# asmuth-archive/libsmatrix

Hardware: AMD Instinct MI355X
Metric: mixed incr+get ops/s (higher is better)
Workload: dtype u32; 1 GPU; config-2: 1xMI355X, 100M-nnz / 1M-row Zipf(1.1) stream (scrambled ids, seed 12345), batched incr+get, 2^24 ops per batch, step = incr batch + get batch; ids_per_axis=1000000, batch_ops=16777216, parallelism=single GPU

## Files before the change

include/smatrix_batch.h:

```cpp
#ifndef SMATRIX_BATCH_H
#define SMATRIX_BATCH_H

#include "smatrix.h"

#ifdef __cplusplus
extern "C" {
#endif

enum { SMATRIX_OP_GET = 0, SMATRIX_OP_SET = 1, SMATRIX_OP_INCR = 2, SMATRIX_OP_DECR = 3 };

int smatrix_apply_batch(smatrix_t* self, int op, size_t n, const uint32_t* x,
                        const uint32_t* y, const uint32_t* v, uint32_t* out);
int smatrix_get_batch(smatrix_t* self, size_t n, const uint32_t* x, const uint32_t* y, uint32_t* out);
int smatrix_set_batch(smatrix_t* self, size_t n, const uint32_t* x, const uint32_t* y,
                      const uint32_t* v, uint32_t* out);
int smatrix_incr_batch(smatrix_t* self, size_t n, const uint32_t* x, const uint32_t* y,
                       const uint32_t* v, uint32_t* out);
int smatrix_decr_batch(smatrix_t* self, size_t n, const uint32_t* x, const uint32_t* y,
                       const uint32_t* v, uint32_t* out);
int smatrix_rowlen_batch(smatrix_t* self, size_t n, const uint32_t* x, uint32_t* out);
int smatrix_getrow_batch(smatrix_t* self, size_t n, const uint32_t* x, const uint64_t* offsets,
                         uint32_t* ret, uint32_t* counts);

int smatrix_apply_batch_dev(smatrix_t* self, int op, size_t n, const uint32_t* d_x,
                            const uint32_t* d_y, const uint32_t* d_v, uint32_t* d_out,
                            void* hip_stream);

int smatrix_apply_packed_dev(smatrix_t* self, int op, size_t n, const uint32_t* d_records, uint32_t width,
                             uint32_t* d_out, void* hip_stream);
int smatrix_rowlen_batch_dev(smatrix_t* self, size_t n, const uint32_t* d_x, uint32_t* d_out,
                             void* hip_stream);
int smatrix_getrow_batch_dev(smatrix_t* self, size_t n, const uint32_t* d_x,
                             const uint64_t* d_offsets, uint32_t* d_ret, uint32_t* d_counts,
                             void* hip_stream);

int smatrix_cf_neighbors_batch(smatrix_t* self, size_t n, const uint32_t* items, const uint64_t* offsets,
                               uint32_t* ids, double* scores, uint32_t* counts);
int smatrix_cf_neighbors_batch_dev(smatrix_t* self, size_t n, const uint32_t* d_items,
                                   const uint64_t* d_offsets, uint32_t* d_ids, double* d_scores,
                                   uint32_t* d_counts, void* hip_stream);

int smatrix_cf_topk_batch(smatrix_t* self, size_t n, const uint32_t* items, uint32_t k, uint32_t* ids, double* scores,
                          uint32_t* counts);
int smatrix_cf_topk_batch_dev(smatrix_t* self, size_t n, const uint32_t* d_items, uint32_t k, uint32_t* d_ids,
                              double* d_scores, uint32_t* d_counts, void* hip_stream);

int smatrix_cf_recommend_batch(smatrix_t* self, size_t n_sessions, const uint64_t* offsets, const uint32_t* items,
                               uint32_t k, uint32_t* ids, double* scores, uint32_t* counts);
int smatrix_cf_recommend_batch_dev(smatrix_t* self, size_t n_sessions, const uint64_t* d_offsets, const uint32_t* d_items,
                                   uint32_t k, uint32_t* d_ids, double* d_scores, uint32_t* d_counts, void* hip_stream);

int smatrix_cf_import_sessions(smatrix_t* self, size_t n_sessions, const uint64_t* offsets, const uint32_t* ids);
int smatrix_cf_import_sessions_dev(smatrix_t* self, size_t n_sessions, const uint64_t* d_offsets, const uint32_t* d_ids,
                                   const uint64_t* d_op_offsets, uint64_t total_ops, void* hip_stream);

enum { SMATRIX_EXPORT_TABLE = 0, SMATRIX_EXPORT_SORTED = 1 };

int smatrix_export(smatrix_t* self, int order, uint64_t cap_rows, uint64_t cap_nnz,
                   uint32_t* rows, uint64_t* row_ptr, uint32_t* pairs, uint64_t* n_rows, uint64_t* nnz);
int smatrix_export_dev(smatrix_t* self, int order, uint64_t cap_rows, uint64_t cap_nnz,
                       uint32_t* d_rows, uint64_t* d_row_ptr, uint32_t* d_pairs,
                       uint64_t* n_rows, uint64_t* nnz, void* hip_stream);

int smatrix_merge(smatrix_t* dst, smatrix_t* src, int op, uint64_t max_batch, uint64_t* n_ops);

int smatrix_merge_scaled(smatrix_t* dst, smatrix_t* src, int op, uint32_t num, uint32_t den, uint32_t min_value,
                         uint64_t max_batch, uint64_t* n_ops, uint64_t* n_dropped);

int smatrix_merge_topk(smatrix_t* dst, smatrix_t* src, int op, uint32_t m, uint32_t min_value, uint64_t max_batch,
                       uint64_t* n_ops, uint64_t* n_dropped);
int smatrix_import_csr(smatrix_t* self, int op, uint64_t n_rows, const uint32_t* rows, const uint64_t* row_ptr,
                       const uint32_t* pairs, uint64_t max_batch, uint64_t* n_ops);
int smatrix_import_csr_dev(smatrix_t* self, int op, uint64_t n_rows, const uint32_t* d_rows,
                           const uint64_t* d_row_ptr, const uint32_t* d_pairs, uint64_t max_batch,
                           uint64_t* n_ops, void* hip_stream);

int smatrix_reserve(smatrix_t* self, uint64_t bytes);

void smatrix_release_cached_memory(void);

typedef struct {
  uint64_t rows;
  uint64_t dir_slots;
  uint64_t arena_units;
  uint64_t arena_mapped;
  uint64_t arena_free_units;
  uint64_t batches;
  uint64_t rounds;
  uint64_t deferred_ops;
  uint64_t rows_grown;
  uint64_t dir_grown;
  uint64_t rows_rebalanced;
  uint64_t long_probe_rounds;
  uint64_t scalar_cache_hits;
  uint64_t scalar_cache_flushes;
  uint64_t scalar_cache_flushed_cells;
  uint64_t bulk_rounds;
  uint64_t bulk_ops;
  uint64_t file_flushes;
  uint64_t file_rows_written;
  uint64_t file_leaked_bytes;
  uint64_t file_compactions;
  uint64_t spec_chains;
  uint64_t spec_refused;
  uint64_t file_bg_flushes;
  uint64_t cold_starts;
  uint64_t cold_keys;
  uint64_t clustered_mode;
  uint64_t set_located_by_fold;
  uint64_t flush_snapshots_refused;
  double   kernel_ms[4];
  uint64_t kernel_launches[4];
  uint64_t kernel_ops[4];
  double   write_call_ms, write_wait_ms, write_alloc_ms;
  double   last_write_call_ms, last_write_wait_ms, last_write_alloc_ms;
} smatrix_stats_t;

void smatrix_stats(smatrix_t* self, smatrix_stats_t* out);
void smatrix_stats_sz(smatrix_t* self, smatrix_stats_t* out, size_t size);
int smatrix_flush(smatrix_t* self);
#ifdef SMATRIX_EXPERIMENTAL
int smatrix_compact(smatrix_t* self);
#endif
void smatrix_profile(smatrix_t* self, int on);
int smatrix_row_info(smatrix_t* self, uint32_t x, uint32_t* size, uint32_t* used);
uint32_t smatrix_row_slots(smatrix_t* self, uint32_t x, uint32_t* kv, uint32_t cap_slots);
int smatrix_device_available(void);

#ifdef __cplusplus
}
#endif
#endif
```

libsmatrix_amd/_lib.py:

```python
import ctypes as C
import os

HERE = os.path.dirname(os.path.abspath(__file__))
LIB_PATH = os.path.join(HERE, "lib", "smatrix.so")
CSRC = os.path.join(HERE, "csrc")

u32p = C.POINTER(C.c_uint32)
u64p = C.POINTER(C.c_uint64)


class Stats(C.Structure):
    _fields_ = [(n, C.c_uint64) for n in (
        "rows", "dir_slots", "arena_units", "arena_mapped", "arena_free_units", "batches", "rounds",
        "deferred_ops", "rows_grown", "dir_grown", "rows_rebalanced", "long_probe_rounds", "scalar_cache_hits", "scalar_cache_flushes",
        "scalar_cache_flushed_cells", "bulk_rounds", "bulk_ops", "file_flushes", "file_rows_written", "file_leaked_bytes",
        "file_compactions", "spec_chains", "spec_refused", "file_bg_flushes", "cold_starts", "cold_keys", "clustered_mode", "set_located_by_fold", "flush_snapshots_refused")] + [
        ("kernel_ms", C.c_double * 4), ("kernel_launches", C.c_uint64 * 4), ("kernel_ops", C.c_uint64 * 4)] + [
        (n, C.c_double) for n in ("write_call_ms", "write_wait_ms", "write_alloc_ms", "last_write_call_ms", "last_write_wait_ms", "last_write_alloc_ms")]


class Handle(C.Structure):
    _fields_ = [("fd", C.c_int), ("shutdown", C.c_int), ("fpos", C.c_uint64),
                ("mem", C.c_uint64), ("impl", C.c_void_p)]


_lib = None


def load():
    global _lib
    if _lib is not None:
        return _lib
    if not os.path.exists(LIB_PATH):
        raise ImportError(
            "libsmatrix_amd: %s is missing -- build it with `make -C %s` "
            "(or python -c 'import __graft_entry__ as g; g.build()').  "
            "This package has no CPU fallback." % (LIB_PATH, CSRC))
    lib = C.CDLL(LIB_PATH)
    H = C.POINTER(Handle)
    V = C.c_void_p
    sig = {
        "smatrix_open": (H, [C.c_char_p]),
        "smatrix_close": (None, [H]),
        "smatrix_get": (C.c_uint32, [H, C.c_uint32, C.c_uint32]),
        "smatrix_set": (C.c_uint32, [H, C.c_uint32, C.c_uint32, C.c_uint32]),
        "smatrix_incr": (C.c_uint32, [H, C.c_uint32, C.c_uint32, C.c_uint32]),
        "smatrix_decr": (C.c_uint32, [H, C.c_uint32, C.c_uint32, C.c_uint32]),
        "smatrix_rowlen": (C.c_uint32, [H, C.c_uint32]),
        "smatrix_getrow": (C.c_uint32, [H, C.c_uint32, u32p, C.c_size_t]),
        "smatrix_apply_batch": (C.c_int, [H, C.c_int, C.c_size_t, u32p, u32p, u32p, u32p]),
        "smatrix_get_batch": (C.c_int, [H, C.c_size_t, u32p, u32p, u32p]),
        "smatrix_set_batch": (C.c_int, [H, C.c_size_t, u32p, u32p, u32p, u32p]),
        "smatrix_incr_batch": (C.c_int, [H, C.c_size_t, u32p, u32p, u32p, u32p]),
        "smatrix_decr_batch": (C.c_int, [H, C.c_size_t, u32p, u32p, u32p, u32p]),
        "smatrix_rowlen_batch": (C.c_int, [H, C.c_size_t, u32p, u32p]),
        "smatrix_getrow_batch": (C.c_int, [H, C.c_size_t, u32p, u64p, u32p, u32p]),
        "smatrix_apply_batch_dev": (C.c_int, [H, C.c_int, C.c_size_t, V, V, V, V, V]),
        "smatrix_apply_packed_dev": (C.c_int, [V, C.c_int, C.c_size_t, V, C.c_uint32, V, V]),
        "smatrix_rowlen_batch_dev": (C.c_int, [H, C.c_size_t, V, V, V]),
        "smatrix_getrow_batch_dev": (C.c_int, [H, C.c_size_t, V, V, V, V, V]),
        "smatrix_cf_neighbors_batch": (C.c_int, [H, C.c_size_t, u32p, u64p, u32p, C.POINTER(C.c_double), u32p]),
        "smatrix_cf_neighbors_batch_dev": (C.c_int, [H, C.c_size_t, V, V, V, V, V, V]),
        "smatrix_release_cached_memory": (None, []),
        "smatrix_reserve": (C.c_int, [H, C.c_uint64]),
        "smatrix_cf_topk_batch": (C.c_int, [H, C.c_size_t, u32p, C.c_uint32, u32p, C.POINTER(C.c_double), u32p]),
        "smatrix_cf_topk_batch_dev": (C.c_int, [H, C.c_size_t, V, C.c_uint32, V, V, V, V]),
        "smatrix_cf_recommend_batch": (C.c_int, [H, C.c_size_t, u64p, u32p, C.c_uint32, u32p, C.POINTER(C.c_double), u32p]),
        "smatrix_cf_recommend_batch_dev": (C.c_int, [H, C.c_size_t, V, V, C.c_uint32, V, V, V, V]),
        "smatrix_cf_import_sessions": (C.c_int, [H, C.c_size_t, u64p, u32p]),
        "smatrix_cf_import_sessions_dev": (C.c_int, [H, C.c_size_t, V, V, V, C.c_uint64, V]),
        "smatrix_export": (C.c_int, [H, C.c_int, C.c_uint64, C.c_uint64, u32p, u64p, u32p, u64p, u64p]),
        "smatrix_export_dev": (C.c_int, [H, C.c_int, C.c_uint64, C.c_uint64, V, V, V, u64p, u64p, V]),
        "smatrix_merge": (C.c_int, [H, H, C.c_int, C.c_uint64, u64p]),
        "smatrix_merge_scaled": (C.c_int, [H, H, C.c_int, C.c_uint32, C.c_uint32, C.c_uint32, C.c_uint64, u64p, u64p]),
        "smatrix_merge_topk": (C.c_int, [H, H, C.c_int, C.c_uint32, C.c_uint32, C.c_uint64, u64p, u64p]),
        "smatrix_import_csr": (C.c_int, [H, C.c_int, C.c_uint64, u32p, u64p, u32p, C.c_uint64, u64p]),
        "smatrix_import_csr_dev": (C.c_int, [H, C.c_int, C.c_uint64, V, V, V, C.c_uint64, u64p, V]),
        "smatrix_stats": (None, [H, C.POINTER(Stats)]),
        "smatrix_stats_sz": (None, [H, C.POINTER(Stats), C.c_size_t]),
        "smatrix_profile": (None, [H, C.c_int]),
        "smatrix_flush": (C.c_int, [H]),
        "smatrix_compact": (C.c_int, [H]),
        "smatrix_row_info": (C.c_int, [H, C.c_uint32, u32p, u32p]),
        "smatrix_row_slots": (C.c_uint32, [H, C.c_uint32, u32p, C.c_uint32]),
        "smatrix_device_available": (C.c_int, []),
        "smatrix_shard_of": (C.c_uint32, [C.c_uint32, C.c_uint32]),
        "smatrix_partition_dev": (C.c_int, [C.c_size_t, V, V, V, C.c_uint32, u64p, V, V, V, V, V, V, C.c_uint32, V, V]),
        "smatrix_partition_packed_dev": (C.c_int, [C.c_size_t, V, V, V, C.c_uint32, u64p, V, V, V, V, C.c_uint32, V, V]),
        "smatrix_shard_mix": (C.c_uint32, [C.c_uint32]),
        "smatrix_place_slot": (C.c_uint32, [C.c_uint32, C.c_uint32]),
        "smatrix_displaced_rows": (C.c_size_t, [V, C.c_uint32, C.c_uint32, V, C.c_size_t]),
        "smatrix_unpack_dev": (C.c_int, [C.c_size_t, C.c_uint32, V, V, V, V, V]),
        "smatrix_gather_dev": (C.c_int, [C.c_size_t, V, V, V, V]),
        "smatrix_shard_unique_id": (C.c_int, [V]),
        "smatrix_shard_open": (V, [C.c_char_p, C.c_int, C.c_int, V]),
        "smatrix_shard_close": (None, [V]),
        "smatrix_shard_local": (H, [V]),
        "smatrix_shard_rank": (C.c_int, [V]),
        "smatrix_shard_nranks": (C.c_int, [V]),
        "smatrix_shard_ops_applied": (C.c_uint64, [V]),
        "smatrix_shard_set_placement": (C.c_int, [V, V, V, C.c_uint32]),
        "smatrix_shard_apply_dev": (C.c_int, [V, C.c_int, C.c_size_t, V, V, V, V, V]),
        "smatrix_shard_apply_then_get_dev": (C.c_int, [V, C.c_int, C.c_size_t, V, V, V, V, V, V]),
        "smatrix_shard_transport": (C.c_char_p, [V]),
        "smatrix_shard_plan_json": (C.c_int, [V, V, C.c_size_t, C.c_uint64, C.c_int, C.c_int, V, C.c_size_t]),
        "smatrix_shard_get_placement": (C.c_int, [V, V, V, V, C.c_uint32, V]),
        "smatrix_shard_route_dev": (V, [V, C.c_int, C.c_size_t, V, V, V, C.c_int, V]),
        "smatrix_shard_apply_routed": (C.c_int, [V, V, C.c_int, V]),
        "smatrix_shard_finish": (C.c_int, [V, V, V, V]),
        "smatrix_shard_wait": (C.c_int, [V, V, V]),
        "smatrix_shard_rowlen_dev": (C.c_int, [V, C.c_size_t, V, V, V]),
        "smatrix_shard_getrow_dev": (C.c_int, [V, C.c_size_t, V, V, V, V, V]),
        "smx_probe_random_dev": (C.c_int, [V, C.c_size_t, C.c_size_t, C.c_int, C.c_uint64, V, V]),
        "smx_stream_new": (V, [C.c_int, C.c_uint64, C.c_uint32, C.c_double, C.c_int]),
        "smx_stream_free": (None, [V]),
        "smx_stream_fill": (None, [V, C.c_uint64, C.c_size_t, u32p, u32p]),
        "smx_stream_fill_device": (C.c_int, [V, C.c_uint64, C.c_size_t, V, V, V]),
        "smx_splitmix64_at": (C.c_uint64, [C.c_uint64, C.c_uint64]),
        "smx_fmix32": (C.c_uint32, [C.c_uint32]),
        "smx_stream_cdf": (C.POINTER(C.c_double), [V, u32p]),
    }
    for name, (res, args) in sig.items():
        fn = getattr(lib, name)
        fn.restype, fn.argtypes = res, args
    _lib = lib
    return lib
```

libsmatrix_amd/csrc/kernels/growth.hpp:

```cpp


constexpr uint32_t CHUNK_NONE = 0xFFFFFFFFu;
__device__ __forceinline__ void grow_plan_body(VGrid g, Ctl* ctl, GrowTask* tasks, uint64_t arena_cap_units, FreeLists fl,
                                               uint32_t task_budget, uint32_t chunk_cap, uint32_t* pend_ctl = nullptr, uint32_t pend_cap_keys = 0,
                                               uint32_t* task_of = nullptr) {
  __shared__ uint32_t l_pend, l_pend0, l_pend_ok;
  __shared__ uint32_t l_want[N_CLASSES], l_got[N_CLASSES];
  __shared__ int32_t l_top[N_CLASSES];
  __shared__ uint32_t l_chunks, l_chunk0, l_chunk_ok;
  __shared__ unsigned long long l_units, l_unit0;
  __shared__ uint32_t l_unit_ok;
  const uint32_t n = aload(&ctl->n_tasks);
  for (uint32_t t0 = g.bid * blockDim.x; t0 < n; t0 += g.nb * blockDim.x) {
    if (threadIdx.x < N_CLASSES) l_want[threadIdx.x] = 0;
    if (threadIdx.x == 0) { l_chunks = 0; l_units = 0; l_chunk_ok = 1; l_unit_ok = 1; l_pend = 0; l_pend_ok = 0; }
    __syncthreads();
    const uint32_t t = t0 + threadIdx.x;
    const bool live = t < n;
    uint32_t cls = 0, rank = 0;
    bool refused = live && t >= task_budget;
    const bool chunked = live && !refused && grow_kind(tasks[t].old_lg) == GROW_CHUNKED;
    uint32_t my_chunk = 0;
    if (chunked) my_chunk = atomicAdd(&l_chunks, 1u << (tasks[t].old_lg - 6));
    __syncthreads();
// ... 1055 lines not shown
  if (k.old_lg + 1 >= HOME_LG) {
    unsigned long long* hb = row_home(arena, k.new_base, k.old_lg + 1);
    for (uint32_t w = 0; w <= (nmask >> 6); w++) {
      unsigned long long m = 0;
      for (uint32_t b = 0; b < 64; b++) {
        const uint64_t c = T[w * 64 + b];
        if (c != 0 && cell_key(c) != 0 && (cell_key(c) & nmask) == w * 64 + b) m |= 1ull << b;
      }
      hb[w] = m;
    }
  }
  if (k.old_lg >= HOME_LG)
    for (uint32_t w = 0; w < (old_size >> 6); w++) row_home(arena, k.old_base, k.old_lg)[w] = 0;
}

__device__ __forceinline__ void grow_zero_body(VGrid g, const Ctl* ctl, const GrowTask* tasks,
                                               const uint32_t* map_old, uint8_t* arena) {
  uint32_t nchunks = aload(&ctl->n_chunks);
  uint32_t wave = (g.bid * blockDim.x + threadIdx.x) >> 6;
  uint32_t lane = threadIdx.x & 63;
  uint32_t nwaves = (g.nb * blockDim.x) >> 6;
  for (uint32_t ch = wave; ch < nchunks; ch += nwaves) {
    const GrowTask k = tasks[map_old[ch]];
    if (k.dup || k.new_base == 0) continue;
    const uint32_t p = (ch - k.chunk0) * 64 + lane;
    if (p < (1u << k.old_lg)) row_cells(arena, k.old_base)[p] = 0;
    if (lane == 0) row_home(arena, k.old_base, k.old_lg)[ch - k.chunk0] = 0;
  }
}
__global__ __launch_bounds__(256) void k_grow_zero(const Ctl* ctl, const GrowTask* tasks,
                                                   const uint32_t* map_old, uint8_t* arena) {
  grow_zero_body(SMX_VG, ctl, tasks, map_old, arena);
}

__device__ __forceinline__ void grow_commit_body(VGrid g, Ctl* ctl, GrowTask* tasks, DirSlot* dir, uint8_t* arena,
                                                 FreeLists fl, uint32_t* big_list = nullptr, uint32_t big_cap = 0) {
  __shared__ uint32_t l_want[N_CLASSES], l_at[N_CLASSES];
  const uint32_t n = aload(&ctl->n_tasks);
  for (uint32_t t0 = g.bid * blockDim.x; t0 < n; t0 += g.nb * blockDim.x) {
    if (threadIdx.x < N_CLASSES) l_want[threadIdx.x] = 0;
    __syncthreads();
    const uint32_t t = t0 + threadIdx.x;
    bool live = t < n;
    GrowTask k = {};
    uint32_t cls = 0, rank = 0;
    if (live && tasks[t].new_base == 0) {
      atomicAnd(&dir[tasks[t].dslot].meta, ~META_GROW);
      live = false;
    }
    if (live) {
      if (tasks[t].dup) grow_fixdup_one(tasks[t], arena);
      k = tasks[t];
      DirSlot& d = dir[k.dslot];
      const uint32_t lg = k.old_lg + 1;
      uint32_t count = k.count;
      if (lg >= BIG_LG && !k.dup) {
        const SubCtr* sc = row_subs(arena, k.new_base, lg);
        for (uint32_t i = 0; i < SUBS; i++) count += sc[i].cnt;
      }
      d.meta = META_USED | META_DIRTY | (lg << META_LG_SHIFT);
      d.base = k.new_base;
      d.used = count;
      if (big_list && lg == FAR_ROW_LG) {
        const uint32_t at = atomicAdd(&big_list[0], 1u);
        if (at < big_cap) big_list[1u + at] = k.dslot;
      }
      if (lg >= BIG_LG) {
        const uint32_t cap = (1u << lg) / 2u + 1u;
        subs_init(row_subs(arena, k.new_base, lg), cap > count ? cap - count : 0u);
      }
      if (k.old_lg >= BIG_LG) {
        uint64_t* z = reinterpret_cast<uint64_t*>(row_subs(arena, k.old_base, k.old_lg));
        for (uint32_t i = 0; i < SUBS * 8; i++) z[i] = 0;
      }
      cls = k.old_lg - ROW_FIRST_LG;
      rank = atomicAdd(&l_want[cls], 1u);
    }
    __syncthreads();
    if (threadIdx.x < N_CLASSES && l_want[threadIdx.x])
      l_at[threadIdx.x] = (uint32_t)atomicAdd(&ctl->free_cnt[threadIdx.x], (int32_t)l_want[threadIdx.x]);
    __syncthreads();
    if (live) {
      fl.list[cls][l_at[cls] + rank] = k.old_base;
    }
    __syncthreads();
  }
}
__global__ __launch_bounds__(256) void k_grow_commit(Ctl* ctl, GrowTask* tasks, DirSlot* dir, uint8_t* arena,
                                                     FreeLists fl, uint32_t* big_list, uint32_t big_cap) {
  grow_commit_body(SMX_VG, ctl, tasks, dir, arena, fl, big_list, big_cap);
}

__global__ __launch_bounds__(256) void k_home_list(const DirSlot* dir, uint32_t dir_size, uint32_t* list, uint32_t* n_list, uint32_t cap) {
  for (uint32_t h = blockIdx.x * blockDim.x + threadIdx.x; h < dir_size; h += gridDim.x * blockDim.x) {
    const DirSlot d = dir[h];
    if ((d.meta & META_USED) && d.base != 0 && meta_lg(d.meta) >= HOME_LG) {
      const uint32_t at = atomicAdd(n_list, 1u);
      if (at < cap) list[at] = h;
    }
  }
}
__global__ __launch_bounds__(256) void k_home_rebuild(const DirSlot* dir, const uint32_t* list, uint32_t first, uint8_t* arena) {
  const DirSlot d = dir[list[first + blockIdx.y]];
  const uint32_t lg = meta_lg(d.meta), nwords = 1u << (lg - 6), mask = (1u << lg) - 1u;
  const uint64_t* cells = row_cells(arena, d.base);
  unsigned long long* hb = row_home(arena, d.base, lg);
  const uint32_t lane = threadIdx.x & 63u;
  for (uint32_t w = blockIdx.x * 4u + (threadIdx.x >> 6); w < nwords; w += gridDim.x * 4u) {
    const uint32_t p = w * 64u + lane;
    const uint64_t c = cells[p];
    const uint64_t m = __ballot(c != 0 && cell_key(c) != 0 && (cell_key(c) & mask) == p);
    if (lane == 0) hb[w] = m;
  }
}

__device__ __forceinline__ void rebal_body(VGrid g, const Ctl* ctl, const uint32_t* rebal, DirSlot* dir, uint8_t* arena) {
  uint32_t n = aload(&ctl->n_rebal);
  for (uint32_t t = g.bid * blockDim.x + threadIdx.x; t < n; t += g.nb * blockDim.x) {
    DirSlot& d = dir[rebal[t]];
    const uint32_t lg = meta_lg(d.meta);
    SubCtr* sc = row_subs(arena, d.base, lg);
    uint32_t used = d.used;
    for (uint32_t k = 0; k < SUBS; k++) used += sc[k].cnt;
    const uint32_t cap = (1u << lg) / 2u + 1u;
    d.used = used;
    d.meta &= ~META_REBAL;
    subs_init(sc, cap > used ? cap - used : 0u);
  }
}
__global__ void k_rebal(const Ctl* ctl, const uint32_t* rebal, DirSlot* dir, uint8_t* arena) {
  rebal_body(SMX_VG, ctl, rebal, dir, arena);
}

__global__ void k_round_advance(Ctl* ctl, const uint32_t* rebal, DirSlot* dir, uint8_t* arena) {
  rebal_body(VGrid{0, 1}, ctl, rebal, dir, arena);
  __syncthreads();
  if (threadIdx.x != 0 || blockIdx.x != 0) return;
  ctl->n_prev = ctl->n_defer;
  ctl->spec_nd0 = ctl->n_defer;
  ctl->spec_nt0 = ctl->n_tasks;
  ctl->spec_gu0 = ctl->grow_units;
  ctl->spec_nrebal0 = ctl->n_rebal;
  ctl->spec_dirfull0 = ctl->dir_full;
  for (int k = 0; k < 4; k++) ctl->spec_nkind0[k] = ctl->n_kind[k];
  const uint32_t keep_long = ctl->n_long, keep_oom = ctl->arena_oom, keep_long_ops = ctl->n_long_ops, n_absent = ctl->n_absent;
  uint64_t* z = reinterpret_cast<uint64_t*>(ctl);
  for (uint32_t i = 0; i < CTL_ROUND_BYTES / 8; i++) z[i] = 0;
  ctl->n_defer = n_absent;
  ctl->n_long = keep_long;
  ctl->n_long_ops = keep_long_ops;
  ctl->arena_oom = keep_oom;
}

__global__ __launch_bounds__(256) void k_dir_rehash(const DirSlot* old, uint32_t old_size,
                                                    DirSlot* dir, uint32_t dmask) {
  uint32_t p = blockIdx.x * blockDim.x + threadIdx.x;
  if (p >= old_size) return;
  DirSlot s = old[p];
  if (!(s.meta & META_USED)) return;
  uint32_t h = fmix32(s.x) & dmask;
  uint64_t want = (uint64_t)s.meta | ((uint64_t)s.x << 32);
  for (;;) {
    uint64_t prev = atomicCAS(reinterpret_cast<unsigned long long*>(&dir[h]), 0ull,
                              (unsigned long long)want);
    if (prev == 0) break;
    h = (h + 1) & dmask;
  }
  dir[h].base = s.base;
  dir[h].used = s.used;
}
```

libsmatrix_amd/csrc/kernels/layout.hpp:

```cpp


struct DirSlot {
  uint32_t meta;
  uint32_t x;
  uint32_t base;
  uint32_t used;
};
static_assert(sizeof(DirSlot) == 16, "DirSlot must be 16 bytes");

constexpr uint32_t META_USED = 1u;
constexpr uint32_t META_GROW = 1u << 16;
constexpr uint32_t META_DIRTY = 1u << 18;
constexpr uint32_t META_LG_SHIFT = 8;
constexpr uint32_t ROW_FIRST_LG = 4;
constexpr uint32_t UNIT_BYTES = 128;

__host__ __device__ inline uint32_t meta_lg(uint32_t meta) { return (meta >> META_LG_SHIFT) & 63u; }
__host__ __device__ inline uint64_t units_of_lg(uint32_t lg) { return 1ull << (lg - ROW_FIRST_LG); }

constexpr uint32_t META_REBAL = 1u << 17;
#ifndef SMX_BIG_LG
#define SMX_BIG_LG 15
#endif
constexpr uint32_t BIG_LG = SMX_BIG_LG;
constexpr uint32_t SUBS = 64;
constexpr uint32_t SUB_UNITS = SUBS * 64 / 128;
struct SubCtr { uint32_t cnt, quota, pad[14]; };
static_assert(sizeof(SubCtr) == 64, "one sub-counter per 64-byte line");

#ifndef SMX_HOME_LG
#define SMX_HOME_LG 12
#endif
constexpr uint32_t HOME_LG = SMX_HOME_LG;
static_assert(HOME_LG >= 10, "the bitmap of the smallest such row fills whole 128-byte units");
__host__ __device__ inline uint64_t home_units(uint32_t lg) { return lg >= HOME_LG ? 1ull << (lg - 10) : 0; }
__host__ __device__ inline uint64_t block_units(uint32_t lg) {
  return units_of_lg(lg) + (lg >= BIG_LG ? SUB_UNITS : 0) + home_units(lg);
}
#ifndef SMX_ENDGAME
#define SMX_ENDGAME 8
#endif
constexpr uint32_t SUBS_ENDGAME = SMX_ENDGAME * SUBS;
__host__ __device__ inline void subs_init(SubCtr* sc, uint32_t room) {
  for (uint32_t k = 0; k < SUBS; k++) {
    sc[k].cnt = 0;
    sc[k].quota = room < SUBS_ENDGAME ? (k == 0 ? room : 0u) : room / SUBS + (k < room % SUBS ? 1u : 0u);
  }
  sc[0].pad[0] = 0;
}

enum Op : int { OP_GET = 0, OP_SET = 1, OP_INCR = 2, OP_DECR = 3 };


constexpr uint32_t N_CLASSES = 28;
struct Ctl {
  uint32_t n_defer;
  uint32_t n_tasks;
  uint32_t dir_full;
  uint32_t arena_oom;
  uint64_t grow_units;
  uint32_t n_chunks;
  uint32_t n_chunks_new;
  uint32_t n_rebal;
  uint32_t n_kind[4];
  uint32_t n_long;
  uint32_t n_long_ops;
  uint32_t n_absent;
  uint32_t dir_used;
  uint32_t pad1;
  uint64_t arena_next;
  int32_t  free_cnt[N_CLASSES];
  uint32_t n_prev;
  uint32_t spec_nd0;
  uint32_t spec_nt0;
  uint32_t spec_failed;
  uint64_t spec_gu0;
  uint32_t spec_nrebal0, spec_dirfull0;
  uint32_t spec_nkind0[4];
  uint32_t n_big, n_units;
  uint32_t far_nd, pad_far;
};
constexpr size_t CTL_ROUND_BYTES = 64;
static_assert(offsetof(Ctl, dir_used) == CTL_ROUND_BYTES, "the per-round part of Ctl is what ctl_reset_round zeroes");

struct FreeLists {
  uint32_t* list[N_CLASSES];
  uint32_t cap[N_CLASSES];
};

struct GrowTask {
  uint32_t dslot;
  uint32_t old_lg;
  uint32_t old_base;
  uint32_t new_base;
  uint32_t count;
  uint32_t chunk0;
  uint32_t chunk0_new;
  uint32_t dup;
  uint32_t wrap_from;
  uint32_t wrap_seen;
  uint32_t n_disp;
  uint32_t pend_off;
  uint32_t pend_cap;
  uint32_t n_pend;
};

constexpr uint32_t GROW_LG0 = 8;
constexpr uint32_t GROW_LG1 = 11;
constexpr uint32_t GROW_LG2 = 13;
constexpr uint32_t GROW_CHUNKED = 3;
__host__ __device__ inline uint32_t grow_kind(uint32_t old_lg) {
  return old_lg <= GROW_LG0 ? 0u : old_lg <= GROW_LG1 ? 1u : old_lg <= GROW_LG2 ? 2u : GROW_CHUNKED;
}

struct VGrid { uint32_t bid, nb; };
#define SMX_VG (VGrid{blockIdx.x, gridDim.x})
__device__ inline uint32_t aload(const uint32_t* p) { return __hip_atomic_load(p, __ATOMIC_RELAXED, __HIP_MEMORY_SCOPE_AGENT); }
__device__ inline uint64_t aload(const uint64_t* p) { return __hip_atomic_load(p, __ATOMIC_RELAXED, __HIP_MEMORY_SCOPE_AGENT); }

__device__ inline uint32_t fmix32(uint32_t h) {
  h ^= h >> 16; h *= 0x85ebca6bU; h ^= h >> 13; h *= 0xc2b2ae35U; h ^= h >> 16;
  return h;
}

__device__ inline uint64_t splitmix_at(uint64_t seed, uint64_t j) {
  uint64_t z = seed + (j + 1) * 0x9e3779b97f4a7c15ULL;
  z = (z ^ (z >> 30)) * 0xbf58476d1ce4e5b9ULL;
  z = (z ^ (z >> 27)) * 0x94d049bb133111ebULL;
  return z ^ (z >> 31);
}

__device__ inline uint64_t pack_cell(uint32_t key, uint32_t value) {
  return (uint64_t)key | ((uint64_t)value << 32);
}
__device__ inline uint32_t cell_key(uint64_t c) { return (uint32_t)c; }
__device__ inline uint32_t cell_val(uint64_t c) { return (uint32_t)(c >> 32); }

__device__ inline uint64_t ld_relaxed(const uint64_t* p) {
  return __hip_atomic_load(p, __ATOMIC_RELAXED, __HIP_MEMORY_SCOPE_AGENT);
}

__device__ inline uint64_t* row_cells(uint8_t* arena, uint32_t base) {
  return reinterpret_cast<uint64_t*>(arena + (uint64_t)base * UNIT_BYTES);
}
__device__ inline SubCtr* row_subs(uint8_t* arena, uint32_t base, uint32_t lg) {
  return reinterpret_cast<SubCtr*>(arena + ((uint64_t)base + units_of_lg(lg)) * UNIT_BYTES);
}
__device__ inline unsigned long long* row_home(uint8_t* arena, uint32_t base, uint32_t lg) {
  return reinterpret_cast<unsigned long long*>(arena + ((uint64_t)base + units_of_lg(lg) + (lg >= BIG_LG ? SUB_UNITS : 0)) * UNIT_BYTES);
}
__device__ inline const unsigned long long* cells_home(const uint64_t* cells, uint32_t mask) {
  return reinterpret_cast<const unsigned long long*>(cells + (uint64_t)mask + 1u) + (mask + 1u >= (1u << BIG_LG) ? SUBS * 8u : 0u);
}
__device__ inline uint32_t subs_sum(const SubCtr* sc) {
  uint32_t t = 0;
  for (uint32_t k = 0; k < SUBS; k++) t += __hip_atomic_load(&sc[k].cnt, __ATOMIC_RELAXED, __HIP_MEMORY_SCOPE_AGENT);
  return t;
}

__device__ inline DirSlot* dir_find(DirSlot* dir, uint32_t dmask, uint32_t x, uint4* snap) {
  uint32_t h = fmix32(x) & dmask;
  for (;;) {
    uint4 s = *reinterpret_cast<const uint4*>(&dir[h]);
    if (!(s.x & META_USED)) return nullptr;
    if (s.y == x) { *snap = s; return &dir[h]; }
    h = (h + 1) & dmask;
  }
}
```

libsmatrix_amd/csrc/smx_runtime.hip:

```cpp
#include "smx_kernels.hpp"

#include <fcntl.h>
#include <sys/stat.h>
#include <time.h>
#include <unistd.h>

#include <linux/falloc.h>
#include <sys/uio.h>

#include <algorithm>
#include <atomic>
#include <chrono>
#include <thread>
#include <cstdio>
#include <cstdlib>
#include <cstring>
#include <deque>
#include <condition_variable>
#include <mutex>
#include <string>
#include <map>
#include <vector>

#define SMATRIX_EXPERIMENTAL 1
// ... 369 lines not shown
      count_hit();
      return true;
    }
    for (;;) {
      if (w_state(w) == 3) return false;
      const uint32_t nv = op == OP_SET ? v : op == OP_INCR ? w_val(w) + v : w_val(w) - v;
      const uint64_t nw = (w & 0xFFFFFFFC00000000ull) | ((uint64_t)2 << 32) | nv;
      if (e->word.compare_exchange_weak(w, nw)) {
        if (w_state(w) == 1) s.dirty.fetch_add(1, std::memory_order_relaxed);
        *res = nv;
        count_hit();
        return true;
      }
      if (w_state(w) == 0 || ((w ^ nw) >> 34) != 0 || e->key.load(std::memory_order_relaxed) != key) return false;
    }
  }
  void wipe_locked(Shard& s) {
    for (uint32_t i : s.occ) s.tab[i].word.store(0);
    s.occ.clear();
    s.dirty.store(0, std::memory_order_relaxed);
    s.gen = (s.gen + 1) & 0x3FFFFFFFu;
    if (s.gen == 0) s.gen = 1;
  }
  void put(uint32_t x, uint32_t y, uint32_t val) {
    if (!enabled || y == 0) return;
    const uint64_t h = mix(x, y), key = (uint64_t)x << 32 | y;
    Shard& s = sh[h & (SHARDS - 1)];
    std::lock_guard<std::mutex> g(s.mu);
    if (!s.tab) {
      s.tab = static_cast<Ent*>(calloc(SLOTS, sizeof(Ent)));
      if (!s.tab) smx_die("malloc() failed");
    }
    uint64_t w;
    if (Ent* e = find(s, h, key, &w)) {
      if (w_state(w) == 1) e->word.compare_exchange_strong(w, (w & 0xFFFFFFFF00000000ull) | val);
      return;
    }
    if (s.occ.size() >= shard_cap) {
      size_t frozen = 0;
      bool dirty_found = false;
      for (; frozen < s.occ.size() && !dirty_found; frozen++) {
        Ent& e = s.tab[s.occ[frozen]];
        uint64_t w = e.word.load();
        for (;;) {
          if (w_state(w) == 2) { dirty_found = true; break; }
          if (e.word.compare_exchange_weak(w, w | ((uint64_t)3 << 32))) break;
        }
        if (dirty_found) break;
      }
      if (dirty_found) {
        for (size_t k = 0; k < frozen; k++) {
          Ent& e = s.tab[s.occ[k]];
          e.word.store(e.word.load() & ~((uint64_t)2 << 32));
        }
        return;
      }
      wipe_locked(s);
    }
    size_t i = (h >> 4) & (SLOTS - 1);
    while (w_state(s.tab[i].word.load(std::memory_order_relaxed))) i = (i + 1) & (SLOTS - 1);
    s.tab[i].key.store(key, std::memory_order_relaxed);
    s.tab[i].word.store(w_make(val, s.gen, 1));
    s.occ.push_back((uint32_t)i);
  }
  void drain(std::vector<uint32_t>& xs, std::vector<uint32_t>& ys, std::vector<uint32_t>& vs, bool clear) {
    for (Shard& s : sh) {
      if (!s.tab || s.occ.empty()) continue;
      std::lock_guard<std::mutex> g(s.mu);
      if (!clear && !s.dirty.load(std::memory_order_acquire)) continue;
      s.dirty.store(0, std::memory_order_release);
      for (uint32_t i : s.occ) {
        Ent& e = s.tab[i];
        uint64_t w = e.word.load();
        for (;;) {
          if (!clear && w_state(w) != 2) break;
          const uint64_t nw = clear ? 0ull : (w & 0xFFFFFFFC00000000ull) | ((uint64_t)1 << 32) | w_val(w);
          if (e.word.compare_exchange_weak(w, nw)) {
            if (w_state(w) == 2) {
              const uint64_t k = e.key.load(std::memory_order_relaxed);
              xs.push_back((uint32_t)(k >> 32)); ys.push_back((uint32_t)k); vs.push_back(w_val(w));
            }
            break;
          }
        }
      }
      if (clear) {
        s.occ.clear();
        s.gen = (s.gen + 1) & 0x3FFFFFFFu;
        if (s.gen == 0) s.gen = 1;
      }
    }
  }
};

struct Matrix {
  int device = 0;
  hipStream_t stream = nullptr;
  std::mutex mu;
  std::mutex qmu;
  std::condition_variable qcv;
  std::vector<ScalarReq*> queue;
  bool combining = false;

  Ctl* d_ctl = nullptr;
  Ctl* h_ctl = nullptr;
  DirSlot* d_dir = nullptr;
  uint32_t dir_size = 0;
  Arena arena;
  uint64_t arena_next = 1;
  uint32_t dir_used = 0;

  DevBuf<uint32_t> defer[2];
  DevBuf<GrowTask> tasks;
  uint64_t io_window = 256ull << 20;
  uint32_t in_stride = 1;
  uint32_t prep_blocks = 512;
  unsigned io_threads = 16;
  DevBuf<uint32_t> klist;
  uint32_t klist_cap = 0;
  DevBuf<uint32_t> rebal;
  FreeLists fl = {};
  int32_t free_cnt[N_CLASSES] = {0};
  DevBuf<uint32_t> map_old, map_new;
  DevBuf<unsigned long long> disp_mask;
  DevBuf<uint32_t> rest_tab;
  uint32_t rest_slice_cells = REST_SLICE_CELLS;
  static constexpr uint32_t rest_grid = 768;
  DevBuf<uint64_t> cellp;
  DevBuf<uint32_t> sx, sy, sv, so;
  DevBuf<uint64_t> soff;
  bool no_ret = false;
  uint32_t set_entries = 0;
  bool set_always_locate = false;
  DevBuf<uint32_t> ent_idx;
  DevBuf<uint32_t> big;
  DevBuf<uint32_t> seg;
  uint32_t* d_small = nullptr;
  uint32_t* h_small = nullptr;

  smatrix_stats_t st = {};
  uint32_t agg_min = 1024;
  uint32_t agg_min_retry = 1u << 20;
  bool retry_may_repeat = false;
  bool profile = false;
  bool trace_rounds = false;
  bool trace_sync = false;
  hipEvent_t ev0 = nullptr, ev1 = nullptr;
  struct TimedLaunch { hipEvent_t e0, e1; uint32_t n; };
  std::deque<TimedLaunch> get_pending;
  std::vector<hipEvent_t> ev_free;
  static constexpr bool grow_fork = true;
  hipStream_t helper = nullptr;
  hipEvent_t ev_fork = nullptr, ev_join = nullptr;

  std::string fname;
  std::atomic<bool> dirty{false};
  bool in_cache_sync = false;
  uint64_t flush_ms = 100;
  std::mutex file_mu;
  std::atomic<bool> ckpt_due{false};
  uint64_t flush_snapshot = 2048ull << 20;
  hipStream_t flush_stream = nullptr;
  std::atomic<uint64_t> file_flushes_done{0}, file_rows_written_done{0}, file_bg_flushes_done{0};
  std::thread flusher;
  std::mutex fl_mu;
  std::condition_variable fl_cv;
  bool fl_stop = false;
  CellCache cache;
  DevBuf<uint64_t> row_ret;
  uint32_t* h_row = nullptr;
  void* file_index = nullptr;
  bool compact_at_close = false;
  bool file_fsync = false;
  uint64_t flush_every = 0;
  uint64_t dbg_after = 0;
  bool bulk_enabled = true;
  bool expect_bulk = true;
  uint32_t fix_share = 4;
  uint32_t fix_presize_min = 1u << 18;
  uint32_t fix_min = 1u << 14;
  DevBuf<uint32_t> fx_cnt, fx_cur, fx_pos, fx_touched, fx_where, fx_grouped, fx_rank;
  std::vector<void*> put_aside;
  uint32_t fx_dir_size = 0;
  DevBuf<uint64_t> fx_excl, fx_tiles;
  bool spec_enabled = true;
  bool spec_ready = false;
  bool spec_tiny = false;
  uint32_t last_nd0 = 1;
  uint32_t spec_nd_prev = 0, spec_nt_prev = 0, spec_nk_prev[4] = {0, 0, 0, 0};
  uint64_t spec_gu_prev = 0;
  bool long_probes = false;
  bool clustered = false, clustered_forced = false;
  uint32_t clustered_quiet = 0;
  uint4* d_hints = nullptr;
  uint32_t hint_lg = 24;
  static constexpr uint32_t wpo_max = 1u << 22;
  uint32_t* absent_list_dev = nullptr;
  static constexpr bool retry_far = true;
  static constexpr bool small_first = true;
  static constexpr bool retry_split = true;
  static constexpr bool absent_split = true;
  unsigned long long* rest_dbg = nullptr; uint32_t rest_dbg_mode = 0; uint64_t rest_dbg_from = 0;
  static constexpr bool get_split = true;
  bool rest_lds = true;
  void* host_pipe = nullptr;
  bool far_join = true;
  DevBuf<uint4> far_tab;
  DevBuf<uint32_t> far_unit_row, far_zeros;
  DevBuf<unsigned long long> far_occ, far_occ0;
  DevBuf<uint32_t> far_clm;
  DevBuf<uint2> pend_rec;
  DevBuf<uint32_t> pend_keys, task_of, pend_ctl;
  DevBuf<unsigned long long> pend_hash;
  double w_call_s = 0, w_wait_s = 0, w_alloc_s = 0;
  bool pend_on = true;
  uint32_t pend_est = 0;
  DevBuf<uint32_t> big_list;
  bool big_list_valid = false;
  DevBuf<uint2> far_unit_info;
  DevBuf<uint32_t> far_bloom;
  DevBuf<uint32_t> far_rcnt, far_bucket, far_prows;
  bool far_place = true;
  uint32_t far_tab_lg = 0;
  uint32_t far_nd_seen = 0;
  uint32_t far_rows_seen = 0, far_units_seen = 0;
  bool home_on = false;
  uint32_t cold_min = 1u << 20;
  uint32_t cold_share = 64;
  DevBuf<unsigned long long> cold_set;
  DevBuf<uint32_t> cold_idx[2], cold_zero;
  static constexpr uint32_t cold_far_max = 1u << 20;
  static constexpr bool cold_all_far = true;
  static constexpr bool cold_far = true;
  DevBuf<unsigned long long> cold_keys[3];
  void* ex = nullptr;
  void* rec = nullptr;
  void* mg = nullptr;
};

void set_device(Matrix* m) { HIP_OK(hipSetDevice(m->device)); }

#define DBG_STEP(m, s, what)                                                          \
  do {                                                                                \
    if ((m)->trace_sync) {                                                            \
      fprintf(stderr, "[smatrix]     %s ...", what); fflush(stderr);                  \
      HIP_OK(hipStreamSynchronize(s));                                                \
      if ((m)->helper) HIP_OK(hipStreamSynchronize((m)->helper));                     \
      fprintf(stderr, " done\n");                                                    \
    }                                                                                 \
  } while (0)

void ctl_reset_round(Matrix* m, hipStream_t s) {
  HIP_OK(hipMemsetAsync(m->d_ctl, 0, CTL_ROUND_BYTES, s));
}

void ctl_push_persistent(Matrix* m, hipStream_t s) {
  Ctl c = {};
  c.dir_used = m->dir_used;
  c.arena_next = m->arena_next;
  memcpy(c.free_cnt, m->free_cnt, sizeof c.free_cnt);
  *m->h_ctl = c;
  HIP_OK(hipMemcpyAsync(m->d_ctl, m->h_ctl, sizeof(Ctl), hipMemcpyHostToDevice, s));
  HIP_OK(hipStreamSynchronize(s));
}

void sync_counted(Matrix* m, hipStream_t s) {
  const double t0 = mono_s();
  HIP_OK(hipStreamSynchronize(s));
  m->w_wait_s += mono_s() - t0;
}
void ctl_read(Matrix* m, hipStream_t s) {
  HIP_OK(hipMemcpyAsync(m->h_ctl, m->d_ctl, sizeof(Ctl), hipMemcpyDeviceToHost, s));
  sync_counted(m, s);
  m->dir_used = m->h_ctl->dir_used;
  m->arena_next = m->h_ctl->arena_next;
  memcpy(m->free_cnt, m->h_ctl->free_cnt, sizeof m->free_cnt);
}

void ensure_free_cap(Matrix* m, uint32_t c, uint64_t extra, hipStream_t s) {
  const uint64_t have = m->free_cnt[c] > 0 ? (uint64_t)m->free_cnt[c] : 0;
  const uint64_t need = have + extra;
  if (need <= m->fl.cap[c]) return;
  const uint64_t ncap = std::max<uint64_t>(need + std::max<uint64_t>(need / 4, 65536), (uint64_t)m->fl.cap[c] * 5 / 4);
  uint32_t* np = nullptr;
  dev_malloc(&np, ncap * sizeof(uint32_t));
  if (have) HIP_OK(hipMemcpyAsync(np, m->fl.list[c], have * sizeof(uint32_t), hipMemcpyDeviceToDevice, s));
  HIP_OK(hipStreamSynchronize(s));
  if (m->fl.list[c]) HIP_OK(dev_free(m->fl.list[c]));
  m->fl.list[c] = np;
  m->fl.cap[c] = (uint32_t)std::min<uint64_t>(ncap, 0x7fffffffu);
}

void ensure_arena_free(Matrix* m, uint64_t units, hipStream_t s) {
  uint64_t need = (m->arena_next + units) * UNIT_BYTES;
  if (need <= m->arena.mapped) return;
  struct timespec t0, t1;
  clock_gettime(CLOCK_MONOTONIC, &t0);
  struct Report {
    Matrix* m; struct timespec* t0; struct timespec* t1; hipStream_t s;
    ~Report() {
      if (!m->trace_rounds) return;
      (void)hipStreamSynchronize(s);
      clock_gettime(CLOCK_MONOTONIC, t1);
      fprintf(stderr, "[smatrix]   arena grown to %.2f GB in %.3f ms\n", m->arena.mapped / 1e9,
              (t1->tv_sec - t0->tv_sec) * 1e3 + (t1->tv_nsec - t0->tv_nsec) * 1e-6);
    }
  } report{m, &t0, &t1, s};
  uint64_t target = std::max<uint64_t>(need, m->arena.mapped + m->arena.mapped / 2);
  if (m->arena.vmm) target = std::min<uint64_t>(std::max<uint64_t>(need, target), m->arena.reserved);
  m->arena.grow_to(target, m->arena_next * UNIT_BYTES, s);
}

constexpr uint32_t BIG_LIST_CAP = 1u << 20;
void grow_directory(Matrix* m, uint32_t factor, hipStream_t s) {
  m->big_list_valid = false;
  uint64_t ns64 = (uint64_t)m->dir_size * factor;
  if (ns64 > (1ull << 31)) smx_die("directory too large");
  uint32_t ns = (uint32_t)ns64;
  DirSlot* nd = nullptr;
  dev_malloc(&nd, (size_t)ns * sizeof(DirSlot));
  zero_async(nd, (size_t)ns * sizeof(DirSlot), s);
  hipLaunchKernelGGL(k_dir_rehash, dim3(blocks_for(m->dir_size)), dim3(256), 0, s, m->d_dir,
                     m->dir_size, nd, ns - 1);
  HIP_OK(hipGetLastError());
  HIP_OK(hipStreamSynchronize(s));
  HIP_OK(dev_free(m->d_dir));
  m->d_dir = nd;
  if (m->trace_rounds)
    fprintf(stderr, "[smatrix] batch %llu directory grown: %u -> %u slots (rows=%u)\n", (unsigned long long)m->st.batches, m->dir_size, ns, m->dir_used);
  m->dir_size = ns;
  m->st.dir_grown++;
}

void ensure_hints(Matrix* m, hipStream_t s) {
  if (m->d_hints || m->hint_lg == 0) return;
  const size_t bytes = (size_t)16 << m->hint_lg;
  dev_malloc(&m->d_hints, bytes);
  zero_async(m->d_hints, bytes, s);
  struct { uint32_t mask; uint4* p; } __attribute__((packed)) w = {(1u << m->hint_lg) - 1u, m->d_hints};
  static_assert(sizeof(w) == 12 && offsetof(ArenaHead, hint_mask) == 4 && offsetof(ArenaHead, hints) == 8, "ArenaHead layout");
  HIP_OK(hipMemcpyAsync(m->arena.base + offsetof(ArenaHead, hint_mask), &w, sizeof(w), hipMemcpyHostToDevice, s));
  HIP_OK(hipStreamSynchronize(s));
  if (m->trace_rounds) fprintf(stderr, "[smatrix] clustered tables: hint table of 2^%u entries\n", m->hint_lg);
// ... 73 lines not shown
  }
  const uint32_t tmask = (1u << lg) - 1u;
  HIP_OK(hipMemsetAsync(m->far_tab.p, 0, (size_t)16 << lg, s));
  arena_head_set(m, offsetof(ArenaHead, far_overflow), 0u, s);
  HIP_OK(hipMemsetAsync(&m->d_ctl->n_big, 0, 8, s));
  m->big_list.need(BIG_LIST_CAP + 1);
  const bool by_list = m->big_list_valid;
  if (!by_list) HIP_OK(hipMemsetAsync(m->big_list.p, 0, 4, s));
  hipLaunchKernelGGL(k_far_rows, dim3(std::min<uint32_t>(blocks_for(by_list ? std::max<uint32_t>(m->far_rows_seen * 2u, 4096u) : m->dir_size), 4096)), dim3(256), 0, s, m->d_ctl,
                     m->d_dir, m->dir_size, m->far_unit_row.p, cap_units, m->far_tab.p, tmask, m->far_unit_info.p, m->big_list.p, BIG_LIST_CAP, by_list ? 1u : 0u);
  m->big_list_valid = true;
  DBG_STEP(m, s, "k_far_rows");
  m->far_bloom.need((size_t)1 << (FAR_BLOOM_LG - 5));
  HIP_OK(hipMemsetAsync(m->far_bloom.p, 0, (size_t)4 << (FAR_BLOOM_LG - 5), s));
  hipLaunchKernelGGL(k_far_keys, dim3(std::min<uint32_t>(blocks_for(est_nd), 4096)), dim3(256), 0, s, m->d_ctl, m->d_dir, m->dir_size - 1, m->arena.base, dl, x, y,
                     m->in_stride, m->far_tab.p, tmask, (1u << lg) / 4u, all_far ? 1u : 0u, m->far_bloom.p);
  DBG_STEP(m, s, "k_far_keys");
  const bool place = m->far_place;
  if (place) { m->far_rcnt.need((size_t)cap_units + 1); m->far_bucket.need((size_t)cap_units * FAR_BUCKET_PER_UNIT); m->far_prows.need(cap_rows); }
  hipLaunchKernelGGL(k_far_scan, dim3(std::min<uint32_t>(blocks_for((uint64_t)cap_units * 64), 32768)), dim3(256), 0, s, m->d_ctl, m->d_dir, m->far_unit_row.p, cap_units,
                     m->arena.base, m->far_tab.p, tmask, m->far_occ.p, m->far_zeros.p, m->far_occ0.p, m->far_clm.p, place ? m->far_rcnt.p : nullptr, m->far_bloom.p, m->far_unit_info.p);
  DBG_STEP(m, s, "k_far_scan");
  if (place) {
    hipLaunchKernelGGL(k_far_absent, dim3(std::min<uint32_t>(blocks_for((uint64_t)1 << lg), 2048)), dim3(256), 0, s, m->d_dir, m->far_unit_row.p, m->arena.base, m->far_tab.p, tmask,
                       m->far_rcnt.p, cap_units, m->far_bucket.p, m->far_prows.p, cap_rows);
    hipLaunchKernelGGL((k_far_place<64, FAR_ROW_LG, FAR_PLACE_SMALL_LG>), dim3(2048), dim3(64), far_place_lds_bytes(FAR_PLACE_SMALL_LG), s, m->d_dir, m->far_unit_row.p, m->arena.base,
                       m->far_tab.p, m->far_rcnt.p, cap_units, m->far_bucket.p, m->far_prows.p, cap_rows, m->far_occ.p, m->far_zeros.p, m->far_occ0.p);
    hipLaunchKernelGGL((k_far_place<512, FAR_PLACE_SMALL_LG + 1, REST_LDS_MAX_LG>), dim3(256), dim3(512), far_place_lds_bytes(REST_LDS_MAX_LG), s, m->d_dir, m->far_unit_row.p, m->arena.base,
                       m->far_tab.p, m->far_rcnt.p, cap_units, m->far_bucket.p, m->far_prows.p, cap_rows, m->far_occ.p, m->far_zeros.p, m->far_occ0.p);
    DBG_STEP(m, s, "k_far_place");
  }
  HIP_OK(hipGetLastError());
  arena_head_set(m, offsetof(ArenaHead, far_on), 1u, s);
  return true;
}

template <int OP>
void launch_apply(Matrix* m, hipStream_t s, uint32_t n, const uint32_t* idx, const uint32_t* x,
                  const uint32_t* y, const uint32_t* v, uint32_t* out, uint32_t* defer) {
  if ((OP == OP_INCR || OP == OP_DECR) && idx && m->clustered && m->retry_far && n >= (1u << 15) && n <= (1u << 21) && m->in_stride != 3) {
    HIP_OK(hipMemsetD32Async(reinterpret_cast<hipDeviceptr_t>(&m->d_ctl->n_prev), (int)n, 1, s));
    if (far_join_enqueue(m, s, idx, x, y, n)) {
      hipLaunchKernelGGL((k_apply_wpo_far<OP == OP_DECR ? OP_DECR : OP_INCR>), dim3(65536), dim3(256), 0, s, m->d_ctl, m->d_dir, m->dir_size - 1, m->arena.base, n,
                         idx, x, y, v, out, defer, m->in_stride);
      HIP_OK(hipGetLastError());
      arena_head_set(m, offsetof(ArenaHead, far_on), 0u, s);
      return;
    }
  }
  if (OP != OP_GET && idx && m->clustered && n <= m->wpo_max) {
    hipLaunchKernelGGL((k_apply_wpo<OP>), dim3(std::min<uint32_t>(blocks_for((uint64_t)n * (64 / SMX_WPO_OPS)), 65536)), dim3(256), 0, s, m->d_ctl, m->d_dir,
                       m->dir_size - 1, m->arena.base, n, idx, x, y, v, out, defer, m->in_stride);
    HIP_OK(hipGetLastError());
    return;
  }
  if (OP == OP_GET && m->d_hints && m->clustered && !idx && m->get_split)
    hipLaunchKernelGGL(k_get_clu, dim3(blocks_for(n)), dim3(256), 0, s, m->d_dir, m->dir_size - 1, m->arena.base, n, x, y, out, m->in_stride);
  else if (m->d_hints)
    hipLaunchKernelGGL((k_apply<OP, true>), dim3(blocks_for(n)), dim3(256), 0, s, m->d_ctl, m->d_dir,
                       m->dir_size - 1, m->arena.base, n, idx, x, y, v, out, defer, m->in_stride);
  else
  hipLaunchKernelGGL((k_apply<OP>), dim3(blocks_for(n)), dim3(256), 0, s, m->d_ctl, m->d_dir,
                     m->dir_size - 1, m->arena.base, n, idx, x, y, v, out, defer, m->in_stride);
  HIP_OK(hipGetLastError());
}

template <int OP>
void launch_apply_agg(Matrix* m, hipStream_t s, uint32_t n, const uint32_t* idx, const uint32_t* x,
                      const uint32_t* y, const uint32_t* v, uint32_t* out, uint32_t* defer) {
  const dim3 grid(blocks_for(n, AGG_TILE)), block(AGG_THREADS);
  if (m->no_ret) {
    if (m->in_stride == 3)
      hipLaunchKernelGGL((k_apply_agg<OP, 3, false>), grid, block, 0, s, m->d_ctl, m->d_dir, m->dir_size - 1, m->arena.base, n, idx, x, y, v, out, defer);
    else
      hipLaunchKernelGGL((k_apply_agg<OP, 1, false>), grid, block, 0, s, m->d_ctl, m->d_dir, m->dir_size - 1, m->arena.base, n, idx, x, y, v, out, defer);
  } else if (m->in_stride == 3) {
    hipLaunchKernelGGL((k_apply_agg<OP, 3>), grid, block, 0, s, m->d_ctl, m->d_dir, m->dir_size - 1, m->arena.base, n, idx, x, y, v, out, defer);
  } else if (m->d_hints && m->clustered) {
    hipLaunchKernelGGL((k_apply_agg_clu<OP>), grid, block, 0, s, m->d_ctl, m->d_dir, m->dir_size - 1, m->arena.base, n, idx, x, y, v, out, defer);
  } else {
    hipLaunchKernelGGL((k_apply_agg<OP>), grid, block, 0, s, m->d_ctl, m->d_dir, m->dir_size - 1, m->arena.base, n, idx, x, y, v, out, defer);
  }
  HIP_OK(hipGetLastError());
}

void launch_apply_op(Matrix* m, int op, hipStream_t s, uint32_t n, const uint32_t* idx,
                     const uint32_t* x, const uint32_t* y, const uint32_t* v, uint32_t* out,
                     uint32_t* defer) {
  bool timed = m->profile && idx == nullptr;
  if (timed) HIP_OK(hipEventRecord(m->ev0, s));
  switch (op) {
    case OP_GET:  launch_apply<OP_GET>(m, s, n, idx, x, y, v, out, defer); break;
    case OP_SET:
      if (idx == nullptr && !m->long_probes && n >= m->agg_min) {
        const uint32_t tiles = blocks_for(n, AGG_TILE);
        m->set_entries = tiles * AGG_TILE;
        m->ent_idx.need(m->set_entries);
        if (m->in_stride == 3)
          hipLaunchKernelGGL((k_set_fold<3>), dim3(tiles), dim3(AGG_THREADS), 0, s, m->d_ctl, m->d_dir, m->dir_size - 1, m->arena.base, n, x, y, v, out, defer, m->ent_idx.p, m->cellp.p);
        else
          hipLaunchKernelGGL((k_set_fold<1>), dim3(tiles), dim3(AGG_THREADS), 0, s, m->d_ctl, m->d_dir, m->dir_size - 1, m->arena.base, n, x, y, v, out, defer, m->ent_idx.p, m->cellp.p);
        HIP_OK(hipGetLastError());
      } else {
        launch_apply<OP_SET>(m, s, n, idx, x, y, v, out, defer);
      }
      break;
    case OP_INCR:
      if (!m->long_probes && n >= (idx && !m->retry_may_repeat ? m->agg_min_retry : m->agg_min)) launch_apply_agg<OP_INCR>(m, s, n, idx, x, y, v, out, defer);
      else launch_apply<OP_INCR>(m, s, n, idx, x, y, v, out, defer);
      break;
    case OP_DECR:
      if (!m->long_probes && n >= (idx && !m->retry_may_repeat ? m->agg_min_retry : m->agg_min)) launch_apply_agg<OP_DECR>(m, s, n, idx, x, y, v, out, defer);
      else launch_apply<OP_DECR>(m, s, n, idx, x, y, v, out, defer);
      break;
    default: smx_die("bad op code");
  }
  if (timed) HIP_OK(hipEventRecord(m->ev1, s));
}

void account_kernel_time(Matrix* m, int op, uint32_t n) {
  float ms = 0;
  HIP_OK(hipEventSynchronize(m->ev1));
  HIP_OK(hipEventElapsedTime(&ms, m->ev0, m->ev1));
  m->st.kernel_ms[op] += ms;
  m->st.kernel_launches[op]++;
  m->st.kernel_ops[op] += n;
}

void get_timing_resolve(Matrix* m, size_t keep) {
  while (m->get_pending.size() > keep) {
    Matrix::TimedLaunch t = m->get_pending.front();
    m->get_pending.pop_front();
    float ms = 0;
    HIP_OK(hipEventSynchronize(t.e1));
    HIP_OK(hipEventElapsedTime(&ms, t.e0, t.e1));
    m->st.kernel_ms[OP_GET] += ms;
    m->st.kernel_launches[OP_GET]++;
    m->st.kernel_ops[OP_GET] += t.n;
    m->ev_free.push_back(t.e0);
    m->ev_free.push_back(t.e1);
  }
}
hipEvent_t get_timing_event(Matrix* m) {
  if (m->ev_free.empty()) {
    hipEvent_t e;
    HIP_OK(hipEventCreate(&e));
    return e;
  }
  hipEvent_t e = m->ev_free.back();
  m->ev_free.pop_back();
  return e;
}

void grow_rows(Matrix* m, hipStream_t s, uint32_t nt, uint64_t gu, const uint32_t* nk, bool spec, bool pend_prep) {
  ensure_arena_free(m, gu, s);
  m->map_new.need((size_t)nt + gu / 4 + 1);
  m->map_old.need((size_t)nt + gu / 8 + 1);
  if (m->clustered && m->home_on && m->rest_lds) {
    m->disp_mask.need(m->map_old.cap);
    m->rest_tab.need(2 + 2 * ((size_t)m->map_old.cap * 64 / m->rest_slice_cells + m->tasks.cap + 1));
  }
  uint64_t cap_units = m->arena.mapped / UNIT_BYTES;
  if (spec && m->spec_tiny) cap_units = std::min<uint64_t>(cap_units, m->arena_next + gu);
  for (uint32_t c = 0; c < N_CLASSES; c++) ensure_free_cap(m, c, nt, s);
  const bool pend = pend_prep && m->clustered && m->home_on;
  uint32_t pend_hash_lg = 16;
  if (pend) {
    m->pend_keys.need(std::min<uint64_t>(8ull * nt + 4ull * gu + 1024, 0x7FFFFFFFull));
    m->task_of.need(m->dir_size);
    while (pend_hash_lg < 24 && (1ull << pend_hash_lg) < 2ull * m->pend_est) pend_hash_lg++;
    m->pend_hash.need((size_t)1 << pend_hash_lg);
  }
  hipLaunchKernelGGL(k_grow_plan, dim3(std::min<uint32_t>(blocks_for(nt), 1024)), dim3(256), 0, s,
                     m->d_ctl, m->tasks.p, cap_units, m->fl, spec ? nt : 0xFFFFFFFFu,
                     spec ? (uint32_t)std::min<uint64_t>(m->map_old.cap, m->map_new.cap / 2) : 0xFFFFFFFFu,
                     pend ? m->pend_ctl.p : nullptr, (uint32_t)m->pend_keys.cap, m->task_of.p);
  DBG_STEP(m, s, "k_grow_plan");
  if (pend) {
    HIP_OK(hipMemsetAsync(m->pend_hash.p, 0, (size_t)8 << pend_hash_lg, s));
    hipLaunchKernelGGL(k_pend_group, dim3(std::min<uint32_t>(blocks_for(std::max<uint32_t>(m->pend_est, 1)), 2048)), dim3(256), 0, s, m->d_ctl, m->tasks.p, m->task_of.p,
                       m->pend_rec.p, (uint32_t)m->pend_rec.cap, m->pend_ctl.p, m->pend_hash.p, (1u << pend_hash_lg) - 1u, m->pend_keys.p);
    DBG_STEP(m, s, "k_pend_group");
  }
  const uint32_t* pend_keys = pend ? m->pend_keys.p : nullptr;
  const uint32_t n_chunked = nk[GROW_CHUNKED];
  const bool fork = m->grow_fork && n_chunked && (nk[0] || nk[1] || nk[2]);
  if (fork) HIP_OK(hipEventRecord(m->ev_fork, s));
  auto lds_kinds = [&](auto pend_c) {
    constexpr bool P = decltype(pend_c)::value;
    if (nk[0])
      hipLaunchKernelGGL((k_grow_lds<64, GROW_LG0, P>), dim3(std::min<uint32_t>(nk[0], 32768)), dim3(64), grow_lds_bytes(GROW_LG0), s,
                         m->d_ctl, m->tasks.p, m->klist.p, 0u, m->arena.base, pend_keys);
    if (nk[1])
      hipLaunchKernelGGL((k_grow_lds<256, GROW_LG1, P>), dim3(std::min<uint32_t>(nk[1], 4096)), dim3(256), grow_lds_bytes(GROW_LG1), s,
                         m->d_ctl, m->tasks.p, m->klist.p + m->klist_cap, 1u, m->arena.base, pend_keys);
    if (nk[2])
      hipLaunchKernelGGL((k_grow_lds<1024, GROW_LG2, P>), dim3(std::min<uint32_t>(nk[2], 1024)), dim3(1024), grow_lds_bytes(GROW_LG2), s,
                         m->d_ctl, m->tasks.p, m->klist.p + 2 * (size_t)m->klist_cap, 2u, m->arena.base, pend_keys);
  };
  if (pend_keys) lds_kinds(std::true_type{}); else lds_kinds(std::false_type{});
  DBG_STEP(m, s, "k_grow_lds x3");
  const uint64_t oc_bound = (uint64_t)n_chunked + gu / 8, nc_bound = (uint64_t)n_chunked + gu / 4;
  hipStream_t sc = s;
  if (fork) {
    HIP_OK(hipStreamWaitEvent(m->helper, m->ev_fork, 0));
    sc = m->helper;
  }
  if (n_chunked) {
    const bool two_pass = m->clustered && m->home_on;
    if (two_pass)
      hipLaunchKernelGGL(k_grow_map<true>, dim3(std::min<uint32_t>(std::max<uint32_t>(n_chunked, 1), 2048)),
                         dim3(256), 0, sc, m->d_ctl, m->tasks.p, m->klist.p + 3 * (size_t)m->klist_cap, m->map_old.p, m->map_new.p, m->arena.base);
    else
      hipLaunchKernelGGL(k_grow_map<false>, dim3(std::min<uint32_t>(std::max<uint32_t>(n_chunked, 1), 2048)),
                         dim3(256), 0, sc, m->d_ctl, m->tasks.p, m->klist.p + 3 * (size_t)m->klist_cap, m->map_old.p, m->map_new.p, nullptr);
    if (two_pass) {
      hipLaunchKernelGGL(k_grow_move_home, dim3(std::min<uint32_t>(blocks_for(oc_bound * 64), 16384)),
                         dim3(256), 0, sc, m->d_ctl, m->tasks.p, m->map_old.p, m->arena.base, m->rest_lds ? m->disp_mask.p : nullptr);
      if (m->rest_lds) {
        hipLaunchKernelGGL(k_grow_rest_count, dim3(std::min<uint32_t>(blocks_for(oc_bound), 1024)), dim3(256), 0, sc, m->d_ctl, m->tasks.p, m->map_old.p, m->disp_mask.p);
        hipLaunchKernelGGL(k_grow_rest_plan, dim3(1), dim3(1024), 0, sc, m->d_ctl, m->tasks.p, m->klist.p + 3 * (size_t)m->klist_cap, m->rest_tab.p,
                           (uint32_t)std::min<size_t>((m->rest_tab.cap - 2) / 2, 0x7FFFFFFFu), m->rest_slice_cells);
        hipLaunchKernelGGL(k_grow_rest_lds, dim3(m->rest_grid), dim3(REST_THREADS), rest_lds_bytes(), sc,
                           m->d_ctl, m->tasks.p, m->rest_tab.p, m->disp_mask.p, m->arena.base, m->st.batches >= m->rest_dbg_from ? m->rest_dbg : nullptr, m->rest_dbg_mode | ((uint32_t)(m->st.batches & 31u) << 8), pend_keys);
      }
      hipLaunchKernelGGL(k_grow_move_rest, dim3(std::min<uint32_t>(blocks_for(oc_bound * 64), 16384)),
                         dim3(256), 0, sc, m->d_ctl, m->tasks.p, m->map_old.p, m->arena.base, m->rest_lds);
    } else {
      hipLaunchKernelGGL(k_grow_move, dim3(std::min<uint32_t>(blocks_for(oc_bound * 64), 16384)),
                         dim3(256), 0, sc, m->d_ctl, m->tasks.p, m->map_old.p, m->arena.base);
    }
    hipLaunchKernelGGL(k_grow_finish, dim3(std::min<uint32_t>(blocks_for(nc_bound * 64), 16384)),
                       dim3(256), 0, sc, m->d_ctl, m->tasks.p, m->map_new.p, m->arena.base, two_pass);
    hipLaunchKernelGGL(k_grow_zero, dim3(std::min<uint32_t>(blocks_for(oc_bound * 64), 16384)),
                       dim3(256), 0, sc, m->d_ctl, m->tasks.p, m->map_old.p, m->arena.base);
  }
  DBG_STEP(m, s, "chunked passes");
  if (fork) {
    HIP_OK(hipEventRecord(m->ev_join, sc));
    HIP_OK(hipStreamWaitEvent(s, m->ev_join, 0));
  }
  hipLaunchKernelGGL(k_grow_commit, dim3(std::min<uint32_t>(blocks_for(nt), 1024)), dim3(256), 0, s,
                     m->d_ctl, m->tasks.p, m->d_dir, m->arena.base, m->fl, m->big_list_valid ? m->big_list.p : nullptr, BIG_LIST_CAP);
  HIP_OK(hipGetLastError());
  DBG_STEP(m, s, "k_grow_commit");
  if (m->trace_rounds && nt > 1000 && !spec) {
    std::vector<GrowTask> ht(nt);
    HIP_OK(hipMemcpyAsync(ht.data(), m->tasks.p, (size_t)nt * sizeof(GrowTask), hipMemcpyDeviceToHost, s));
    sync_counted(m, s);
    uint64_t cnt[32] = {0};
    for (const GrowTask& k : ht) cnt[k.old_lg & 31]++;
    fprintf(stderr, "[smatrix]   growth by old size:");
    for (int lg = 4; lg < 32; lg++)
      if (cnt[lg]) fprintf(stderr, " 2^%d x%llu (%.1fM cells)", lg, (unsigned long long)cnt[lg], cnt[lg] * (double)(1ull << lg) / 1e6);
    fprintf(stderr, "\n");
  }
  m->arena_next += gu;
  if (!spec) m->st.rows_grown += nt;
}

template <int OP>
uint32_t run_bulk_t(Matrix* m, uint32_t nd, const uint32_t* dl, uint32_t* dl_out, const uint32_t* x, const uint32_t* y,
                    const uint32_t* v, uint32_t* out, hipStream_t s) {
  bool created_from_set = false;
  if (nd >= m->fix_presize_min && nd / 16 >= m->dir_size && nd <= (1u << 27)) {
    uint64_t slots = 1u << 16;
    while (slots < 2ull * std::min<uint64_t>(nd, 1ull << 27)) slots <<= 1;
    m->cold_set.need_on(slots, s);
    zero_async(m->cold_set.p, slots * 8, s);
    HIP_OK(hipMemsetAsync(m->d_small + 12, 0, 8, s));
    hipLaunchKernelGGL(k_fix_count_rows, dim3(std::min<uint32_t>(blocks_for(nd, 256 * FIXR_OPT), 4096)), dim3(256), 0, s, m->d_dir, m->dir_size - 1, nd, dl,
                       x, m->in_stride, m->cold_set.p, slots - 1, m->d_small + 12);
    HIP_OK(hipGetLastError());
    HIP_OK(hipMemcpyAsync(m->h_small + 12, m->d_small + 12, 8, hipMemcpyDeviceToHost, s));
    sync_counted(m, s);
    const uint64_t need = (uint64_t)m->dir_used + m->h_small[12] + m->h_small[13];
    uint64_t size = m->dir_size;
    while (need > size / 2) size *= 4;
    if (need * 2 >= size) size *= 2;
    if (m->trace_rounds)
      fprintf(stderr, "[smatrix] batch %llu bulk path: %u ops name %u rows the directory lacks; directory %u -> %llu slots\n",
              (unsigned long long)m->st.batches, nd, m->h_small[12] + m->h_small[13], m->dir_size, (unsigned long long)size);
    if (size > m->dir_size) grow_directory(m, (uint32_t)(size / m->dir_size), s);
    if (need > m->dir_used && need <= m->dir_size / 2) {
      ensure_arena_free(m, need - m->dir_used, s);
      hipLaunchKernelGGL(k_fix_create_set, dim3((uint32_t)std::min<uint64_t>(blocks_for(slots, 256 * FIXS_OPT), 1024)), dim3(256), 0, s, m->d_ctl, m->d_dir,
                         m->dir_size - 1, m->cold_set.p, slots, (uint64_t)(m->arena.mapped / UNIT_BYTES), m->fl);
      HIP_OK(hipGetLastError());
      created_from_set = true;
      m->fx_where.need(nd); m->fx_grouped.need(nd); m->fx_rank.need(nd);
      const uint32_t rows_guess = (uint32_t)std::min<uint64_t>(nd, need);
      m->fx_touched.need(std::max<uint32_t>(rows_guess, 1)); m->fx_excl.need(std::max<uint32_t>(rows_guess, 1));
      m->fx_tiles.need((rows_guess + SCAN_TILE - 1) / SCAN_TILE + 2);
      if (m->fx_dir_size != m->dir_size) { m->fx_cnt.need(m->dir_size); m->fx_cur.need(m->dir_size); m->fx_pos.need(m->dir_size); }
      ctl_read(m, s);
      if (m->h_ctl->arena_oom) smx_die("internal: arena reservation too small");
    }
  }
  for (int tries = 0; !created_from_set; tries++) {
    if (tries > 40) smx_die("bulk path: the directory does not take the batch's rows");
    const uint32_t dir_limit = m->dir_size / 2;
    const uint32_t room = dir_limit > m->dir_used ? dir_limit - m->dir_used : 0;
    ensure_arena_free(m, std::min<uint64_t>(nd, room), s);
    ctl_reset_round(m, s);
    hipLaunchKernelGGL(k_fix_create, dim3(std::min<uint32_t>(blocks_for(nd, 256 * FIXR_OPT), 4096)), dim3(256), 0, s, m->d_ctl, m->d_dir,
                       m->dir_size - 1, dir_limit, nd, dl, x, m->in_stride, (uint64_t)(m->arena.mapped / UNIT_BYTES), m->fl);
    HIP_OK(hipGetLastError());
    if (tries == 0) {
      m->fx_where.need(nd); m->fx_grouped.need(nd); m->fx_rank.need(nd);
      const uint32_t rows_guess = (uint32_t)std::min<uint64_t>(nd, (uint64_t)m->dir_size / 2);
      m->fx_touched.need(std::max<uint32_t>(rows_guess, 1)); m->fx_excl.need(std::max<uint32_t>(rows_guess, 1));
      m->fx_tiles.need((rows_guess + SCAN_TILE - 1) / SCAN_TILE + 2);
      if (m->fx_dir_size != m->dir_size) { m->fx_cnt.need(m->dir_size); m->fx_cur.need(m->dir_size); m->fx_pos.need(m->dir_size); }
    }
    ctl_read(m, s);
    if (m->h_ctl->arena_oom) smx_die("internal: arena reservation too small");
    const bool full = m->h_ctl->dir_full != 0;
    if (full) grow_directory(m, 4, s);
    else if ((uint64_t)m->dir_used * 2 >= m->dir_size) grow_directory(m, 2, s);
    if (!full) break;
  }
  const uint32_t ds = m->dir_size;
  if (m->fx_dir_size != ds) {
    m->fx_cnt.need(ds); m->fx_cur.need(ds); m->fx_pos.need(ds);
    HIP_OK(hipMemsetAsync(m->fx_cnt.p, 0, (size_t)ds * 4, s));
    HIP_OK(hipMemsetAsync(m->fx_cur.p, 0, (size_t)ds * 4, s));
    m->fx_dir_size = ds;
  }
  const uint32_t rows_max = (uint32_t)std::min<uint64_t>(nd, m->dir_used);
  const uint32_t ntiles = (rows_max + SCAN_TILE - 1) / SCAN_TILE;
  for (uint32_t c = 0; c <= FIX_MAX_LG - ROW_FIRST_LG; c++) ensure_free_cap(m, c, rows_max, s);
  m->fx_touched.need(std::max<uint32_t>(rows_max, 1)); m->fx_excl.need(std::max<uint32_t>(rows_max, 1)); m->fx_tiles.need(ntiles + 2);
  m->fx_where.need(nd); m->fx_grouped.need(nd); m->fx_rank.need(nd);
  ctl_reset_round(m, s);
  hipLaunchKernelGGL(k_fix_count, dim3(std::min<uint32_t>(blocks_for(nd, 256 * FIXC_OPT), 8192)), dim3(256), 0, s, m->d_ctl, m->d_dir, ds - 1, nd,
                     dl, x, y, m->in_stride, m->fx_cnt.p, m->fx_where.p, dl_out, m->fx_touched.p, m->fx_pos.p, m->fx_rank.p);
  HIP_OK(hipMemsetAsync(m->fx_tiles.p + ntiles, 0, 16, s));
  hipLaunchKernelGGL(k_fix_scan_tiles, dim3(std::max(ntiles, 1u)), dim3(256), 0, s, m->d_ctl, m->d_dir, m->fx_cnt.p, m->fx_touched.p,
                     m->fx_excl.p, m->fx_tiles.p, m->fx_tiles.p + ntiles + 1);
  hipLaunchKernelGGL(k_fix_scan_tops, dim3(1), dim3(1024), 0, s, m->fx_tiles.p, ntiles, m->fx_tiles.p + ntiles);
  hipLaunchKernelGGL(k_fix_scan_add, dim3(blocks_for(std::max<uint32_t>(rows_max, 1))), dim3(256), 0, s, m->d_ctl, m->fx_excl.p, m->fx_tiles.p);
  hipLaunchKernelGGL(k_fix_scatter, dim3(std::min<uint32_t>(blocks_for(nd, 256 * FIXC_OPT), 8192)), dim3(256), 0, s, m->d_ctl, m->d_dir, m->fx_cnt.p, nd, dl, m->fx_where.p, m->fx_excl.p,
                     m->fx_pos.p, m->fx_rank.p, m->fx_grouped.p, dl_out);
  HIP_OK(hipGetLastError());
  uint64_t tw[2] = {0, 0};
  HIP_OK(hipMemcpyAsync(tw, m->fx_tiles.p + ntiles, 16, hipMemcpyDeviceToHost, s));
  sync_counted(m, s);
  const uint64_t units = tw[0] >> 32;
  ensure_arena_free(m, units, s);
  if (m->arena_next + units >= (1ull << 32)) smx_die("row arena exhausted");
  const uint64_t new_base0 = m->arena_next;
  const dim3 fgrid(std::max<uint32_t>(1, std::min<uint32_t>((rows_max + FIX_WAVES - 1) / FIX_WAVES, 8192)));
  hipLaunchKernelGGL((k_fix_rows<OP, FIX_MAX_LG - 1>), fgrid, dim3(64 * FIX_WAVES), 0, s,
                     m->d_ctl, m->d_dir, m->fx_touched.p, m->arena.base, m->fx_cnt.p, m->fx_cur.p, m->fx_excl.p, m->fx_grouped.p, y, v,
                     m->in_stride, out, dl_out, new_base0, m->fl);
  if (tw[1])
    hipLaunchKernelGGL((k_fix_rows<OP, FIX_MAX_LG>), fgrid, dim3(64 * FIX_WAVES), 0, s,
                     m->d_ctl, m->d_dir, m->fx_touched.p, m->arena.base, m->fx_cnt.p, m->fx_cur.p, m->fx_excl.p, m->fx_grouped.p, y, v,
                     m->in_stride, out, dl_out, new_base0, m->fl);
  HIP_OK(hipGetLastError());
  const uint64_t next = new_base0 + units;
  HIP_OK(hipMemcpyAsync(&m->d_ctl->arena_next, &next, 8, hipMemcpyHostToDevice, s));
  std::vector<void*> put_aside;
  {
    const uint64_t bound = std::min<uint64_t>(nd, m->dir_size);
    const auto grow = [&](auto& buf, size_t n) {
      if (n <= buf.cap) return;
      if (buf.p) put_aside.push_back(buf.p);
      buf.p = nullptr; buf.cap = 0;
      buf.need(n);
    };
    grow(m->tasks, bound); grow(m->klist, 4 * bound); grow(m->rebal, bound);
    if (m->cold_min && nd >= m->cold_min) {
      uint64_t slots = 1;
      while (slots < 2ull * nd) slots <<= 1;
      m->cold_set.need_on(slots, s);
      m->cold_keys[0].need_on(nd, s);
      m->cold_keys[1].need_on(nd / 4 + nd / 8, s);
      if (m->small_first) m->cold_keys[2].need_on(nd / 4 + nd / 8, s);
      if (m->small_first && m->cold_far && m->far_join) {
        m->cold_idx[0].need_on(m->cold_far_max, s); m->cold_idx[1].need_on(m->cold_far_max, s); m->cold_zero.need_on(3 * (size_t)m->cold_far_max, s);
      }
    }
  }
  ctl_read(m, s);
  m->put_aside.insert(m->put_aside.end(), put_aside.begin(), put_aside.end());
  m->st.bulk_rounds++;
  m->st.bulk_ops += nd - m->h_ctl->n_defer;
  return m->h_ctl->n_defer;
}

bool insert_pending_keys(Matrix* m, const uint32_t* list, uint32_t n_list, const uint32_t* x, const uint32_t* y, hipStream_t s) {
  uint64_t slots = 1;
// ... 3 lines not shown
  zero_async(m->cold_set.p, slots * 8, s);
  HIP_OK(hipMemsetAsync(m->d_small + 12, 0, 8, s));
  hipLaunchKernelGGL(k_dedup_keys, dim3(std::min<uint32_t>(blocks_for(n_list, DEDUP_THREADS * DEDUP_TRIPS), 4096)), dim3(DEDUP_THREADS), 0, s,
                     n_list, list, x, y, m->in_stride, m->cold_set.p, slots - 1, m->cold_keys[0].p, m->d_small + 12);
  HIP_OK(hipGetLastError());
  HIP_OK(hipMemcpyAsync(m->h_small + 12, m->d_small + 12, 8, hipMemcpyDeviceToHost, s));
  sync_counted(m, s);
  uint32_t cur_n = m->h_small[12];
  const bool dense_keys = (uint64_t)m->h_small[13] * 4 >= cur_n;
  if (m->trace_rounds)
    fprintf(stderr, "[smatrix] batch %llu cold start: %u pending ops name %u distinct keys, %u of them below %u%s\n", (unsigned long long)m->st.batches, n_list, cur_n,
            m->h_small[13], n_list, dense_keys && m->small_first ? ": the rounds take the keys below their row's size first" : "");
  if ((uint64_t)cur_n * 4 > (uint64_t)n_list * 3) return false;
  m->st.cold_starts++;
  m->st.cold_keys += cur_n;
  const bool was_clustered = m->clustered;
  if (dense_keys && m->small_first && !m->clustered_forced && !m->clustered) {
    m->clustered = true; m->clustered_quiet = 0;
    clustered_sync(m, s);
    if (m->trace_rounds) fprintf(stderr, "[smatrix]   dense ids: clustered tables from here on\n");
  }
  uint32_t cur_buf = 0;
  if (was_clustered && m->dir_used) {
    m->cold_keys[1].need_on(cur_n, s);
    ctl_reset_round(m, s);
    const uint32_t wpo = cur_n <= (1u << 21) ? 1u : 0u;
    hipLaunchKernelGGL(k_insert_keys, dim3(wpo ? std::min<uint32_t>(blocks_for((uint64_t)cur_n * 64, INS_THREADS), 16384) : blocks_for(cur_n, INS_THREADS)), dim3(INS_THREADS), 0, s,
                       m->d_ctl, m->d_dir, m->dir_size - 1, m->arena.base, cur_n, m->cold_keys[0].p, m->cold_keys[1].p, wpo, INS_DROP_EXISTING, (unsigned long long*)nullptr);
    HIP_OK(hipGetLastError());
    ctl_read(m, s);
    if (m->trace_rounds) fprintf(stderr, "[smatrix]   %u of the %u keys exist already (left by the pass in front of prep): dropped from the list\n", cur_n - m->h_ctl->n_defer, cur_n);
    cur_n = m->h_ctl->n_defer;
    cur_buf = 1;
    if (cur_n == 0) return true;
  }
  const unsigned long long* kin = m->cold_keys[cur_buf].p;
  uint32_t stalled = 0, rows_before = m->dir_used;
  for (uint32_t round = 0; cur_n; round++) {
    if (stalled > 8) smx_die("write batch did not converge (corrupt row table?)");
    const uint32_t dir_limit = m->dir_size / 2;
    const uint32_t room = dir_limit > m->dir_used ? dir_limit - m->dir_used : 0;
    m->tasks.need(std::min<uint64_t>(cur_n, m->dir_size));
    m->klist_cap = (uint32_t)std::min<uint64_t>(cur_n, m->dir_size);
    m->klist.need(4 * (size_t)m->klist_cap);
    m->rebal.need(std::min<uint64_t>(cur_n, m->dir_size));
    unsigned long long* other = cur_buf ? m->cold_keys[0].p : (m->cold_keys[1].need_on(cur_n, s), m->cold_keys[1].p);
    ensure_arena_free(m, std::min<uint64_t>(cur_n, room), s);
    ctl_reset_round(m, s);
    const uint32_t ins_wpo = m->clustered && cur_n <= (1u << 21) ? 1u : 0u;
    unsigned long long* kout = other;
    if ((m->clustered || dense_keys) && m->small_first) {
      unsigned long long* mine = const_cast<unsigned long long*>(kin);
      m->cold_keys[2].need_on(cur_n, s);
      unsigned long long* walk = m->cold_keys[2].p;
      hipLaunchKernelGGL(k_insert_keys, dim3(blocks_for(cur_n, INS_THREADS)), dim3(INS_THREADS), 0, s,
                         m->d_ctl, m->d_dir, m->dir_size - 1, m->arena.base, cur_n, kin, other, 0u, INS_SMALL_ONLY, (unsigned long long*)nullptr);
      hipLaunchKernelGGL(k_list_advance, dim3(1), dim3(1), 0, s, m->d_ctl);
      hipLaunchKernelGGL(k_insert_keys, dim3(blocks_for(cur_n, INS_THREADS)), dim3(INS_THREADS), 0, s,
                         m->d_ctl, m->d_dir, m->dir_size - 1, m->arena.base, cur_n, other, mine, 0u, INS_HOME_ONLY | INS_FROM_PREV, walk);
      hipLaunchKernelGGL(k_walk_advance, dim3(1), dim3(1), 0, s, m->d_ctl);
      kout = mine;
      bool far_joined = false;
      if (m->clustered && m->home_on && m->far_join && m->cold_far && cur_n <= m->cold_far_max) {
        m->cold_idx[0].need_on(cur_n, s); m->cold_idx[1].need_on(cur_n, s); m->cold_zero.need_on(3 * (size_t)cur_n, s);
        zero_async(m->cold_zero.p, 8 * (size_t)cur_n, s);
        hipLaunchKernelGGL(k_iota, dim3(std::min<uint32_t>(blocks_for(cur_n), 4096)), dim3(256), 0, s, m->cold_idx[0].p, cur_n);
        const uint32_t* xk = reinterpret_cast<const uint32_t*>(walk) + 1, * yk = reinterpret_cast<const uint32_t*>(walk);
        const uint32_t stride_was = m->in_stride;
        m->in_stride = 2;
        far_joined = far_join_enqueue(m, s, m->cold_idx[0].p, xk, yk, cur_n, m->cold_all_far);
        if (far_joined) {
          hipLaunchKernelGGL((k_apply_wpo_far<OP_INCR>), dim3(65536), dim3(256), 0, s, m->d_ctl, m->d_dir, m->dir_size - 1, m->arena.base, 0xFFFFFFFFu,
                             m->cold_idx[0].p, xk, yk, m->cold_zero.p, m->cold_zero.p + 2 * (size_t)cur_n, m->cold_idx[1].p, 2u);
          arena_head_set(m, offsetof(ArenaHead, far_on), 0u, s);
          hipLaunchKernelGGL(k_gather_keys, dim3(std::min<uint32_t>(blocks_for(cur_n), 4096)), dim3(256), 0, s, m->d_ctl, m->cold_idx[1].p, walk, kout, cur_n);
        }
        m->in_stride = stride_was;
      }
      if (!far_joined)
        hipLaunchKernelGGL(k_insert_keys, dim3(ins_wpo ? std::min<uint32_t>(blocks_for((uint64_t)cur_n * 64, INS_THREADS), 16384) : blocks_for(cur_n, INS_THREADS)), dim3(INS_THREADS), 0, s,
                           m->d_ctl, m->d_dir, m->dir_size - 1, m->arena.base, cur_n, walk, kout, ins_wpo, INS_FROM_PREV, (unsigned long long*)nullptr);
    } else {
      hipLaunchKernelGGL(k_insert_keys, dim3(ins_wpo ? std::min<uint32_t>(blocks_for((uint64_t)cur_n * 64, INS_THREADS), 16384) : blocks_for(cur_n, INS_THREADS)), dim3(INS_THREADS), 0, s,
                         m->d_ctl, m->d_dir, m->dir_size - 1, m->arena.base, cur_n, kin, kout, ins_wpo, 0u, (unsigned long long*)nullptr);
      cur_buf ^= 1u;
    }
    hipLaunchKernelGGL(k_prep, dim3(std::min<uint32_t>(blocks_for(cur_n, PREP_THREADS), m->prep_blocks)), dim3(PREP_THREADS), 0, s,
                       m->d_ctl, m->d_dir, m->dir_size - 1, dir_limit, m->arena.base,
                       (uint64_t)(m->arena.mapped / UNIT_BYTES), (const uint32_t*)nullptr, reinterpret_cast<const uint32_t*>(kout) + 1,
                       reinterpret_cast<const uint32_t*>(kout), m->tasks.p, m->klist.p, m->klist_cap, m->rebal.p, m->fl, 2u, 2u, 0u, (uint2*)nullptr, 0u, (uint32_t*)nullptr);
    HIP_OK(hipGetLastError());
    ctl_read(m, s);
    m->st.rounds++;
    const Ctl& c = *m->h_ctl;
    if (m->trace_rounds) {
      static thread_local double t_prev = 0;
      struct timespec ts;
      clock_gettime(CLOCK_MONOTONIC, &ts);
      const double now = ts.tv_sec * 1e3 + ts.tv_nsec * 1e-6;
      fprintf(stderr, "[smatrix] batch %llu cold round %u (+%.3f ms): keys=%u deferred=%u grow=%u (%llu units) rebal=%u dir_full=%u rows=%u\n",
              (unsigned long long)m->st.batches, round, t_prev ? now - t_prev : 0.0, cur_n, c.n_defer, c.n_tasks, (unsigned long long)c.grow_units,
              c.n_rebal, c.dir_full, c.dir_used);
      t_prev = now;
    }
    if (c.arena_oom) smx_die("internal: arena reservation too small");
    const uint32_t nd = c.n_defer;
    if (nd == 0) break;
    if (!m->clustered_forced && !m->clustered && (uint64_t)c.n_long_ops * 64 >= cur_n) {
      m->clustered = true; m->clustered_quiet = 0;
      clustered_sync(m, s);
      if (m->trace_rounds) fprintf(stderr, "[smatrix]   %u of %u keys needed the wave-cooperative probe: clustered tables from here on\n", c.n_long_ops, cur_n);
    }
    const bool progress = nd < cur_n || c.n_tasks || c.n_rebal || c.dir_full || m->dir_used != rows_before || (uint64_t)m->dir_used * 2 >= m->dir_size;
    stalled = progress ? 0 : stalled + 1;
    rows_before = m->dir_used;
    m->st.deferred_ops += nd;
    if (c.n_tasks) grow_rows(m, s, c.n_tasks, c.grow_units, c.n_kind, false, false);
    if (c.n_rebal) {
      hipLaunchKernelGGL(k_rebal, dim3(std::min<uint32_t>(blocks_for(c.n_rebal, 64), 1024)), dim3(64), 0, s, m->d_ctl, m->rebal.p, m->d_dir, m->arena.base);
      HIP_OK(hipGetLastError());
      m->st.rows_rebalanced += c.n_rebal;
    }
    if (c.dir_full) grow_directory(m, 4, s);
    else if ((uint64_t)m->dir_used * 2 >= m->dir_size) grow_directory(m, 2, s);
    kin = kout;
    cur_n = nd;
  }
  return true;
}

void run_write(Matrix* m, int op, uint32_t n, const uint32_t* x, const uint32_t* y,
               const uint32_t* v, uint32_t* out, hipStream_t s) {
  if (n == 0) return;
  if (!m->in_cache_sync) m->dirty = true;
  m->defer[0].need(n);
  m->defer[1].need(n);
  if (op == OP_SET) m->cellp.need((size_t)n + AGG_TILE);
  m->set_entries = 0;
  m->st.batches++;
  if (m->dbg_after && m->st.batches == m->dbg_after) {
    const uint32_t one = 1;
    HIP_OK(hipMemcpyAsync(&m->d_ctl->pad1, &one, 4, hipMemcpyHostToDevice, s));
  }

  uint32_t cur_n = n;
  const uint32_t* idx = nullptr;
  bool timed0 = m->profile;
  uint32_t stalled = 0, rows_before = m->dir_used;
  m->long_probes = false;
  m->retry_may_repeat = false;
  uint32_t rounds_this_batch = 0;
  bool cold_tried = false;
  bool structure_stable = false;
  bool chain = m->spec_enabled && m->spec_ready && !m->expect_bulk && n >= m->agg_min && m->dbg_after == 0 &&
               (m->last_nd0 != 0 || m->spec_tiny);
  for (uint32_t round = 0;; round++) {
    if (stalled > 8) smx_die("write batch did not converge (corrupt row table?)");
    const uint32_t dir_limit = m->dir_size / 2;
    const uint32_t room = dir_limit > m->dir_used ? dir_limit - m->dir_used : 0;
    m->tasks.need(std::min<uint64_t>(cur_n, m->dir_size));
    m->klist_cap = (uint32_t)std::min<uint64_t>(cur_n, m->dir_size);
    m->klist.need(4 * (size_t)m->klist_cap);
    m->rebal.need(std::min<uint64_t>(cur_n, m->dir_size));
    if (round >= 1 && idx && !cold_tried && m->cold_min && cur_n >= m->cold_min && (uint64_t)cur_n * m->cold_share >= n &&
        op != OP_GET) {
      cold_tried = true;
      if (insert_pending_keys(m, idx, cur_n, x, y, s)) rounds_this_batch += 4;
    }
    uint32_t* dl = m->defer[round & 1].p;
    const bool chained = chain && round == 0;
    const uint32_t est_nt = m->spec_tiny ? 5u : (uint32_t)std::min<uint64_t>(std::max<uint64_t>(2ull * m->spec_nt_prev, 1u << 16), std::min<uint64_t>(cur_n, m->dir_size));
    const uint64_t est_gu = m->spec_tiny ? 24u : std::max<uint64_t>(2 * m->spec_gu_prev, 1ull << 20);
    ensure_arena_free(m, std::min<uint64_t>(cur_n, room) + (chained ? est_gu : 0), s);
    ctl_reset_round(m, s);
    const bool all_new = round == 0 && !chained && m->dir_used == 0 && m->bulk_enabled && m->expect_bulk && n >= m->fix_min &&
                         n >= m->agg_min && m->dbg_after == 0 && (op == OP_INCR || op == OP_DECR);
    if (all_new) {
      hipLaunchKernelGGL(k_iota, dim3(std::min<uint32_t>(blocks_for(n), 4096)), dim3(256), 0, s, dl, n);
      HIP_OK(hipGetLastError());
      HIP_OK(hipMemcpyAsync(&m->d_ctl->n_defer, &n, 4, hipMemcpyHostToDevice, s));
      timed0 = false;
    } else {
      if (op == OP_INCR || op == OP_DECR) {
        const bool pass_follows = (chained || (round == 0 && idx == nullptr && m->home_on && m->far_join && n >= (1u << 16))) && m->clustered;
        absent_list_set(m, pass_follows && m->absent_split && m->dbg_after == 0 ? m->defer[1].p : nullptr, s);
      }
      launch_apply_op(m, op, s, cur_n, idx, x, y, v, out, dl);
    }
    DBG_STEP(m, s, m->long_probes ? "op kernel (lane per op)" : "op kernel");
#if defined(SMX_AGG_DBG) && SMX_AGG_DBG == 5
    if (m->dbg_after && m->st.batches >= m->dbg_after) {
      ctl_read(m, s);
      if (timed0) { account_kernel_time(m, op, n); timed0 = false; }
      break;
    }
#endif
    if (round == 0 && !chained && m->bulk_enabled && m->expect_bulk && op != OP_GET && n >= m->fix_min) {
      if (!all_new) ctl_read(m, s);
      if (timed0) { account_kernel_time(m, op, n); timed0 = false; }
      const uint32_t nd0 = all_new ? n : m->h_ctl->n_defer + m->h_ctl->n_absent;
      m->expect_bulk = (uint64_t)nd0 * 8 >= n;
      if (nd0 >= m->fix_min && nd0 < 0x80000000u && (uint64_t)nd0 * m->fix_share >= n) {
        m->st.rounds++;
        rounds_this_batch++;
        m->st.deferred_ops += nd0;
        m->tasks.need(std::min<uint64_t>(cur_n, m->dir_size));
        if (!all_new && m->h_ctl->n_absent) {
          HIP_OK(hipMemcpyAsync(dl + m->h_ctl->n_defer, m->defer[1].p, (size_t)m->h_ctl->n_absent * 4, hipMemcpyDeviceToDevice, s));
          HIP_OK(hipMemsetD32Async(reinterpret_cast<hipDeviceptr_t>(&m->d_ctl->n_defer), (int)nd0, 1, s));
          HIP_OK(hipMemsetD32Async(reinterpret_cast<hipDeviceptr_t>(&m->d_ctl->n_absent), 0, 1, s));
        }
        uint32_t* dl2 = m->defer[1].p;
        const uint32_t nd2 = op == OP_INCR   ? run_bulk_t<OP_INCR>(m, nd0, dl, dl2, x, y, v, out, s)
                             : op == OP_DECR ? run_bulk_t<OP_DECR>(m, nd0, dl, dl2, x, y, v, out, s)
                                             : run_bulk_t<OP_SET>(m, nd0, dl, dl2, x, y, v, out, s);
        if (m->trace_rounds)
          fprintf(stderr, "[smatrix] batch %llu bulk path: %u deferred ops grouped by row, %u handed back, rows=%u\n",
                  (unsigned long long)m->st.batches, nd0, nd2, m->dir_used);
        if (nd2 == 0) break;
        m->retry_may_repeat = true;
        idx = dl2;
        cur_n = nd2;
        round++;
        rounds_this_batch += 2;
        continue;
      }
    }
    bool prep_pend = false;
    const auto launch_prep = [&](const uint32_t* list) {
      const uint32_t pgrid = m->clustered && cur_n <= 8192u ? blocks_for((uint64_t)cur_n * 64, PREP_THREADS) : blocks_for(cur_n, PREP_THREADS);
      const bool pend = m->clustered && m->home_on && m->pend_on && m->in_stride != 3;
      if (pend) {
        m->pend_rec.need(std::min<size_t>(n, (size_t)1 << 22));
        m->pend_ctl.need(16);
        HIP_OK(hipMemsetAsync(m->pend_ctl.p, 0, 16, s));
        m->pend_est = (uint32_t)std::min<uint64_t>(chained ? std::max<uint64_t>(2ull * m->spec_nd_prev, 1u << 16) : cur_n, m->pend_rec.cap);
      }
      prep_pend = pend;
      hipLaunchKernelGGL(k_prep, dim3(std::min<uint32_t>(pgrid, m->prep_blocks)), dim3(PREP_THREADS), 0, s,
                         m->d_ctl, m->d_dir, m->dir_size - 1, dir_limit, m->arena.base,
                         (uint64_t)(m->arena.mapped / UNIT_BYTES), list, x, y, m->tasks.p, m->klist.p, m->klist_cap,
                         m->rebal.p, m->fl, m->in_stride, 0u, m->clustered ? 8192u : 0u, pend ? m->pend_rec.p : nullptr, (uint32_t)m->pend_rec.cap, m->pend_ctl.p);
    };
    const bool pre_pass = (chained || (round == 0 && idx == nullptr && !all_new && m->home_on && m->far_join && n >= (1u << 16))) && m->clustered &&
                          (op == OP_INCR || op == OP_DECR);
    bool far_joined = false;
    if (pre_pass) {
      uint32_t* dlp = m->defer[1].p;
      hipLaunchKernelGGL(k_round_advance, dim3(1), dim3(64), 0, s, m->d_ctl, m->rebal.p, m->d_dir, m->arena.base);
      uint64_t est_far = std::max<uint64_t>({2ull * m->spec_nd_prev, 3ull * m->far_nd_seen / 2, 1ull << 16});
      if (!chained && m->far_join && m->home_on) {
        uint32_t nd_now = 0;
        HIP_OK(hipMemcpyAsync(&nd_now, &m->d_ctl->n_prev, 4, hipMemcpyDeviceToHost, s));
        sync_counted(m, s);
        est_far = (uint64_t)nd_now + nd_now / 8 + 1024;
        if (m->trace_rounds) fprintf(stderr, "[smatrix] batch %llu: the folding kernel deferred %u ops\n", (unsigned long long)m->st.batches, nd_now);
      }
      far_joined = far_join_enqueue(m, s, dl, x, y, (uint32_t)std::min<uint64_t>(est_far, cur_n));
      if (far_joined) {
        const dim3 wgrid(65536);
        if (op == OP_INCR) hipLaunchKernelGGL((k_apply_wpo_far<OP_INCR>), wgrid, dim3(256), 0, s, m->d_ctl, m->d_dir, m->dir_size - 1, m->arena.base, 0xFFFFFFFFu, dl, x, y, v, out, dlp, m->in_stride);
        else hipLaunchKernelGGL((k_apply_wpo_far<OP_DECR>), wgrid, dim3(256), 0, s, m->d_ctl, m->d_dir, m->dir_size - 1, m->arena.base, 0xFFFFFFFFu, dl, x, y, v, out, dlp, m->in_stride);
      } else {
      const dim3 wgrid(65536);
      if (op == OP_INCR) hipLaunchKernelGGL((k_apply_wpo<OP_INCR>), wgrid, dim3(256), 0, s, m->d_ctl, m->d_dir, m->dir_size - 1, m->arena.base, 0xFFFFFFFFu, dl, x, y, v, out, dlp, m->in_stride);
      else hipLaunchKernelGGL((k_apply_wpo<OP_DECR>), wgrid, dim3(256), 0, s, m->d_ctl, m->d_dir, m->dir_size - 1, m->arena.base, 0xFFFFFFFFu, dl, x, y, v, out, dlp, m->in_stride);
      }
      HIP_OK(hipGetLastError());
      DBG_STEP(m, s, "the pass in front of prep");
      dl = dlp;
    }
    launch_prep(dl);
    HIP_OK(hipGetLastError());
    if (far_joined) arena_head_set(m, offsetof(ArenaHead, far_on), 0u, s);
    DBG_STEP(m, s, "k_prep");
    uint32_t nd_chain0 = 0;
    bool retry_halves = false;
    if (chained) {
      const uint32_t est_nk[4] = {std::max<uint32_t>(2 * m->spec_nk_prev[0], 4096), std::max<uint32_t>(2 * m->spec_nk_prev[1], 1024),
                                  std::max<uint32_t>(2 * m->spec_nk_prev[2], 256), std::max<uint32_t>(2 * m->spec_nk_prev[3], 64)};
      const uint64_t host_next = m->arena_next;
      grow_rows(m, s, est_nt, est_gu, est_nk, true, prep_pend);
      m->arena_next = host_next;
      hipLaunchKernelGGL(k_round_advance, dim3(1), dim3(64), 0, s, m->d_ctl, m->rebal.p, m->d_dir, m->arena.base);
      const uint32_t est_nd = (uint32_t)std::min<uint64_t>(std::max<uint64_t>(2ull * m->spec_nd_prev, 1u << 16), cur_n);
      uint32_t* dl1 = pre_pass ? m->defer[0].p : m->defer[1].p;
      const dim3 rgrid(std::min<uint32_t>(blocks_for(est_nd), 16384));
      if (m->clustered && est_nd <= m->wpo_max && m->retry_split && m->d_hints) {
        uint32_t* dl0 = dl;
        const dim3 wgrid(std::min<uint32_t>(blocks_for((uint64_t)est_nd * (64 / SMX_WPO_OPS)), 65536));
        switch (op) {
          case OP_SET:  hipLaunchKernelGGL((k_apply_short<OP_SET>), rgrid, dim3(256), 0, s, m->d_ctl, m->d_dir, m->dir_size - 1, m->arena.base, 0xFFFFFFFFu, dl, x, y, v, out, dl1, m->in_stride); break;
          case OP_INCR: hipLaunchKernelGGL((k_apply_short<OP_INCR>), rgrid, dim3(256), 0, s, m->d_ctl, m->d_dir, m->dir_size - 1, m->arena.base, 0xFFFFFFFFu, dl, x, y, v, out, dl1, m->in_stride); break;
          default:      hipLaunchKernelGGL((k_apply_short<OP_DECR>), rgrid, dim3(256), 0, s, m->d_ctl, m->d_dir, m->dir_size - 1, m->arena.base, 0xFFFFFFFFu, dl, x, y, v, out, dl1, m->in_stride); break;
        }
        hipLaunchKernelGGL(k_list_advance, dim3(1), dim3(64), 0, s, m->d_ctl);
        switch (op) {
          case OP_SET:  hipLaunchKernelGGL((k_apply_wpo<OP_SET>), wgrid, dim3(256), 0, s, m->d_ctl, m->d_dir, m->dir_size - 1, m->arena.base, 0xFFFFFFFFu, dl1, x, y, v, out, dl0, m->in_stride); break;
          case OP_INCR: hipLaunchKernelGGL((k_apply_wpo<OP_INCR>), wgrid, dim3(256), 0, s, m->d_ctl, m->d_dir, m->dir_size - 1, m->arena.base, 0xFFFFFFFFu, dl1, x, y, v, out, dl0, m->in_stride); break;
          default:      hipLaunchKernelGGL((k_apply_wpo<OP_DECR>), wgrid, dim3(256), 0, s, m->d_ctl, m->d_dir, m->dir_size - 1, m->arena.base, 0xFFFFFFFFu, dl1, x, y, v, out, dl0, m->in_stride); break;
        }
        dl1 = dl0;
        retry_halves = true;
      } else if (m->clustered && est_nd <= m->wpo_max) {
        const dim3 wgrid(std::min<uint32_t>(blocks_for((uint64_t)est_nd * 64), 65536));
        switch (op) {
          case OP_SET:  hipLaunchKernelGGL((k_apply_wpo<OP_SET>), wgrid, dim3(256), 0, s, m->d_ctl, m->d_dir, m->dir_size - 1, m->arena.base, 0xFFFFFFFFu, dl, x, y, v, out, dl1, m->in_stride); break;
          case OP_INCR: hipLaunchKernelGGL((k_apply_wpo<OP_INCR>), wgrid, dim3(256), 0, s, m->d_ctl, m->d_dir, m->dir_size - 1, m->arena.base, 0xFFFFFFFFu, dl, x, y, v, out, dl1, m->in_stride); break;
          default:      hipLaunchKernelGGL((k_apply_wpo<OP_DECR>), wgrid, dim3(256), 0, s, m->d_ctl, m->d_dir, m->dir_size - 1, m->arena.base, 0xFFFFFFFFu, dl, x, y, v, out, dl1, m->in_stride); break;
        }
      } else
      switch (op) {
        case OP_SET:  hipLaunchKernelGGL((k_apply<OP_SET>), rgrid, dim3(256), 0, s, m->d_ctl, m->d_dir, m->dir_size - 1, m->arena.base, 0xFFFFFFFFu, dl, x, y, v, out, dl1, m->in_stride); break;
        case OP_INCR: hipLaunchKernelGGL((k_apply<OP_INCR>), rgrid, dim3(256), 0, s, m->d_ctl, m->d_dir, m->dir_size - 1, m->arena.base, 0xFFFFFFFFu, dl, x, y, v, out, dl1, m->in_stride); break;
        default:      hipLaunchKernelGGL((k_apply<OP_DECR>), rgrid, dim3(256), 0, s, m->d_ctl, m->d_dir, m->dir_size - 1, m->arena.base, 0xFFFFFFFFu, dl, x, y, v, out, dl1, m->in_stride); break;
      }
      launch_prep(dl1);
      HIP_OK(hipGetLastError());
      dl = dl1;
    }
    ctl_read(m, s);
    if (timed0 && round == 0) account_kernel_time(m, op, n);
    m->st.rounds++;
    rounds_this_batch++;
    if (chained) {
      const Ctl& c = *m->h_ctl;
      nd_chain0 = c.spec_nd0;
      if (far_joined) { m->far_rows_seen = c.n_big; m->far_units_seen = c.n_units; m->far_nd_seen = c.far_nd; }
      if (!m->in_cache_sync) m->last_nd0 = nd_chain0;
      m->expect_bulk = (uint64_t)nd_chain0 * 8 >= n;
      m->st.spec_chains++;
      if (nd_chain0) {
        m->st.rounds++;
        rounds_this_batch++;
        m->st.deferred_ops += nd_chain0;
        m->st.rows_grown += c.spec_nt0;
        m->st.rows_rebalanced += c.spec_nrebal0;
        m->spec_nd_prev = nd_chain0; m->spec_nt_prev = c.spec_nt0; m->spec_gu_prev = c.spec_gu0;
        for (int k = 0; k < 4; k++) m->spec_nk_prev[k] = c.spec_nkind0[k];
      }
      if (c.spec_failed) {
        m->st.spec_refused++;
        const uint32_t zero = 0;
        HIP_OK(hipMemcpyAsync(&m->d_ctl->spec_failed, &zero, 4, hipMemcpyHostToDevice, s));
      }
      if (m->trace_rounds && m->rest_dbg) {
        static thread_local unsigned long long last[3] = {0, 0, 0};
        unsigned long long now[3];
        HIP_OK(hipMemcpy(now, m->rest_dbg + 16, 24, hipMemcpyDeviceToHost));
        fprintf(stderr, "[smatrix]   far join: big rows %u (%u units); long probes of the pass: not in the table %llu, cell known %llu, absent %llu\n",
                c.n_big, c.n_units, now[0] - last[0], now[1] - last[1], now[2] - last[2]);
        memcpy(last, now, sizeof last);
      }
      if (m->trace_rounds)
        fprintf(stderr, "[smatrix] batch %llu chain: ops=%u (the pass in front of prep took %u) deferred=%u grow=%u (%llu units) rebal=%u refused=%u | after the retry: deferred=%u grow=%u rows=%u | long probes %u%s\n",
                (unsigned long long)m->st.batches, cur_n, far_joined ? c.far_nd : 0u, nd_chain0, c.spec_nt0, (unsigned long long)c.spec_gu0, c.spec_nrebal0,
                c.spec_failed, c.n_defer, c.n_tasks, c.dir_used, c.n_long_ops, m->clustered ? " (clustered)" : "");
      if (!m->clustered_forced && m->clustered) {
        m->clustered_quiet = (uint64_t)c.n_long_ops * (m->d_hints ? 4096 : 256) < n ? m->clustered_quiet + 1 : 0;
        if (m->clustered_quiet >= 8) { m->clustered = false; clustered_sync(m, s); }
      }
      if (nd_chain0 == 0) { structure_stable = true; break; }
      cur_n = nd_chain0;
      round = (pre_pass ? 2 : 1) + (retry_halves ? 1 : 0);
    } else if (pre_pass) {
      if (far_joined) { m->far_rows_seen = m->h_ctl->n_big; m->far_units_seen = m->h_ctl->n_units; m->far_nd_seen = m->h_ctl->far_nd; }
      if (m->trace_rounds) {
        uint32_t ovf = 0;
        HIP_OK(hipMemcpy(&ovf, m->arena.base + offsetof(ArenaHead, far_overflow), 4, hipMemcpyDeviceToHost));
        fprintf(stderr, "[smatrix] batch %llu round 0 with the pass in front of prep (it took %u ops; join table 2^%u%s): ops=%u deferred=%u grow=%u rows=%u\n", (unsigned long long)m->st.batches,
                far_joined ? m->h_ctl->far_nd : 0u, m->far_tab_lg, ovf ? ", OVERFLOWED" : "", cur_n, m->h_ctl->n_defer, m->h_ctl->n_tasks, m->h_ctl->dir_used);
      }
    } else if (m->trace_rounds) {
      static thread_local double t_prev = 0;
      struct timespec ts;
      clock_gettime(CLOCK_MONOTONIC, &ts);
      const double now = ts.tv_sec * 1e3 + ts.tv_nsec * 1e-6;
      fprintf(stderr, "[smatrix] batch %llu round %u (+%.3f ms): ops=%u deferred=%u grow=%u (%llu units) rebal=%u dir_full=%u rows=%u\n",
              (unsigned long long)m->st.batches, round, t_prev ? now - t_prev : 0.0, cur_n, m->h_ctl->n_defer,
              m->h_ctl->n_tasks, (unsigned long long)m->h_ctl->grow_units, m->h_ctl->n_rebal, m->h_ctl->dir_full,
              m->h_ctl->dir_used);
      t_prev = now;
    }
    if (m->h_ctl->arena_oom) smx_die("internal: arena reservation too small");
    const uint32_t nd = m->h_ctl->n_defer;
    if (round == 0) m->expect_bulk = (uint64_t)nd * 8 >= n;
    if (round == 0 && !chained && !m->in_cache_sync) m->last_nd0 = nd;
    if (round == 1 && !chained && nd == 0) {
      m->spec_nd_prev = cur_n;
    }
    if (nd == 0) { structure_stable = round == 0 && !chained; break; }
    if (m->h_ctl->n_long) { m->long_probes = true; m->st.long_probe_rounds++; }
    if (!m->clustered_forced && !m->clustered && (uint64_t)m->h_ctl->n_long_ops * 64 >= n) { m->clustered = true; m->clustered_quiet = 0; }
    clustered_sync(m, s);

    const bool progress = nd < cur_n || m->h_ctl->n_long || m->h_ctl->n_tasks || m->h_ctl->n_rebal || m->h_ctl->dir_full ||
                          m->dir_used != rows_before || (uint64_t)m->dir_used * 2 >= m->dir_size;
    stalled = progress ? 0 : stalled + 1;
    m->retry_may_repeat = m->dir_used != rows_before;
    rows_before = m->dir_used;
    m->st.deferred_ops += nd;
    if (round == 0) {
      m->spec_nt_prev = m->h_ctl->n_tasks; m->spec_gu_prev = m->h_ctl->grow_units;
      for (int k = 0; k < 4; k++) m->spec_nk_prev[k] = m->h_ctl->n_kind[k];
    }
    if (m->h_ctl->n_tasks) grow_rows(m, s, m->h_ctl->n_tasks, m->h_ctl->grow_units, m->h_ctl->n_kind, false, prep_pend);
    if (m->h_ctl->n_rebal) {
      hipLaunchKernelGGL(k_rebal, dim3(std::min<uint32_t>(blocks_for(m->h_ctl->n_rebal, 64), 1024)), dim3(64), 0, s,
                         m->d_ctl, m->rebal.p, m->d_dir, m->arena.base);
      HIP_OK(hipGetLastError());
      m->st.rows_rebalanced += m->h_ctl->n_rebal;
    }
    if (m->h_ctl->dir_full) grow_directory(m, 4, s);
    else if ((uint64_t)m->dir_used * 2 >= m->dir_size) grow_directory(m, 2, s);
    idx = dl;
    cur_n = nd;
    if (pre_pass && !chained) round++;
  }
  m->spec_ready = rounds_this_batch <= 4;
  for (void* q : m->put_aside) (void)dev_free(q);
  m->put_aside.clear();
  if (m->spec_ready || !cold_tried) {
    m->cold_set.release_on(s); m->cold_keys[0].release_on(s); m->cold_keys[1].release_on(s); m->cold_keys[2].release_on(s);
    m->cold_idx[0].release_on(s); m->cold_idx[1].release_on(s); m->cold_zero.release_on(s);
  }
  if (m->trace_rounds) {
    AllocClock& ac = alloc_clock();
    if (ac.n_alloc + ac.n_free)
      fprintf(stderr, "[smatrix] batch %llu: %llu device allocations %.3f ms, %llu frees %.3f ms\n", (unsigned long long)m->st.batches,
              (unsigned long long)ac.n_alloc, ac.s_alloc * 1e3, (unsigned long long)ac.n_free, ac.s_free * 1e3);
    ac = AllocClock();
  }

  if (op == OP_SET && m->set_entries) {
    const uint32_t ne = m->set_entries;
    dim3 g(blocks_for(ne)), b(256);
    if (!structure_stable || m->set_always_locate)
      hipLaunchKernelGGL(k_set_locate_e, g, b, 0, s, m->d_dir, m->dir_size - 1, m->arena.base, ne, x, y, m->ent_idx.p, m->cellp.p, m->in_stride);
    else m->st.set_located_by_fold++;
    hipLaunchKernelGGL(k_set_rank_e, g, b, 0, s, ne, m->ent_idx.p, m->cellp.p, m->arena.base);
    hipLaunchKernelGGL(k_set_pick_e, g, b, 0, s, ne, m->ent_idx.p, m->cellp.p, m->arena.base);
    hipLaunchKernelGGL(k_set_store_e, g, b, 0, s, ne, m->ent_idx.p, m->cellp.p, v, m->arena.base, m->in_stride);
    HIP_OK(hipGetLastError());
    sync_counted(m, s);
  } else if (op == OP_SET) {
    dim3 g(blocks_for(n)), b(256);
    hipLaunchKernelGGL(k_set_locate, g, b, 0, s, m->d_dir, m->dir_size - 1, m->arena.base, n, x, y,
                       m->cellp.p, m->in_stride);
    hipLaunchKernelGGL(k_set_clear, g, b, 0, s, n, m->cellp.p, m->arena.base);
    hipLaunchKernelGGL(k_set_rank, g, b, 0, s, n, m->cellp.p, m->arena.base);
    hipLaunchKernelGGL(k_set_pick, g, b, 0, s, n, m->cellp.p, m->arena.base);
    hipLaunchKernelGGL(k_set_store, g, b, 0, s, n, m->cellp.p, v, m->arena.base, m->in_stride);
    HIP_OK(hipGetLastError());
    sync_counted(m, s);
  }
}

void run_get(Matrix* m, uint32_t n, const uint32_t* x, const uint32_t* y, uint32_t* out,
             hipStream_t s) {
  if (n == 0) return;
  if (!m->profile) {
    launch_apply_op(m, OP_GET, s, n, nullptr, x, y, nullptr, out, nullptr);
    return;
  }
  get_timing_resolve(m, 15);
  Matrix::TimedLaunch t{get_timing_event(m), get_timing_event(m), n};
  HIP_OK(hipEventRecord(t.e0, s));
  m->profile = false;
  launch_apply_op(m, OP_GET, s, n, nullptr, x, y, nullptr, out, nullptr);
  m->profile = true;
  HIP_OK(hipEventRecord(t.e1, s));
  m->get_pending.push_back(t);
}

Matrix* M(smatrix_t* self) { return static_cast<Matrix*>(self->impl); }

void refresh_public(smatrix_t* self) {
  Matrix* m = M(self);
  uint64_t free_units = 0;
  for (uint32_t c = 0; c < N_CLASSES; c++)
    if (m->free_cnt[c] > 0) free_units += (uint64_t)m->free_cnt[c] * block_units(c + ROW_FIRST_LG);
  const uint64_t live_units = m->arena_next > free_units ? m->arena_next - free_units : 0;
  self->mem = (uint64_t)m->dir_size * sizeof(DirSlot) + live_units * UNIT_BYTES;
}

bool file_flush(smatrix_t* self, Matrix* m, bool all, std::unique_lock<std::mutex>* unlock);
void cache_sync(Matrix* m, bool drop);
void export_release(Matrix* m);
void recommend_release(Matrix* m);
void merge_release(Matrix* m);

void apply_dev_locked(smatrix_t* self, int op, size_t n, const uint32_t* x, const uint32_t* y,
                      const uint32_t* v, uint32_t* out, hipStream_t s) {
  Matrix* m = M(self);
  if (n >= (1ull << 32)) smx_die("batch too large (n must be < 2^32)");
  if (op == OP_GET) run_get(m, (uint32_t)n, x, y, out, s);
  else {
    const double t0 = mono_s(), w0 = m->w_wait_s;
    const AllocClock a0 = alloc_clock();
    run_write(m, op, (uint32_t)n, x, y, v, out, s);
    const AllocClock a1 = alloc_clock();
    const double call = mono_s() - t0, wait = m->w_wait_s - w0, al = std::max(0.0, (a1.s_alloc + a1.s_free) - (a0.s_alloc + a0.s_free));
    m->w_call_s += call; m->w_alloc_s += al;
    m->st.write_call_ms = m->w_call_s * 1e3; m->st.write_wait_ms = m->w_wait_s * 1e3; m->st.write_alloc_ms = m->w_alloc_s * 1e3;
    m->st.last_write_call_ms = call * 1e3; m->st.last_write_wait_ms = wait * 1e3; m->st.last_write_alloc_ms = al * 1e3;
  }
  refresh_public(self);
  if (op != OP_GET && m->flush_every && self->fd && !m->in_cache_sync && m->st.batches % m->flush_every == 0) m->ckpt_due = true;
}

void checkpoint(smatrix_t* self) {
  Matrix* m = M(self);
  set_device(m);
  std::unique_lock<std::mutex> fg(m->file_mu);
  std::unique_lock<std::mutex> g(m->mu);
  if (!self->fd || !m->dirty.exchange(false)) return;
  cache_sync(m, false);
  if (file_flush(self, m, false, &g)) m->dirty = true;
}
struct CkptAfter {
  smatrix_t* self;
  explicit CkptAfter(smatrix_t* s) : self(s) {}
  ~CkptAfter() { if (M(self)->ckpt_due.exchange(false)) checkpoint(self); }
};

void cache_sync(Matrix* m, bool drop) {
  if (!m->cache.enabled) return;
  std::vector<uint32_t> xs, ys, vs;
  m->cache.drain(xs, ys, vs, drop);
  const size_t k = xs.size();
  if (!k) return;
  hipStream_t s = m->stream;
  m->sx.need(k); m->sy.need(k); m->sv.need(k); m->so.need(k);
  HIP_OK(hipMemcpyAsync(m->sx.p, xs.data(), k * 4, hipMemcpyHostToDevice, s));
  HIP_OK(hipMemcpyAsync(m->sy.p, ys.data(), k * 4, hipMemcpyHostToDevice, s));
  HIP_OK(hipMemcpyAsync(m->sv.p, vs.data(), k * 4, hipMemcpyHostToDevice, s));
  const uint32_t keep = m->in_stride;
  m->in_stride = 1;
  const uint64_t batches = m->st.batches;
  const bool k_ready = m->spec_ready, k_bulk = m->expect_bulk, k_long = m->long_probes, k_clu = m->clustered;
  const uint32_t k_nd = m->spec_nd_prev, k_nt = m->spec_nt_prev, k_quiet = m->clustered_quiet;
  const uint64_t k_gu = m->spec_gu_prev;
  uint32_t k_nk[4];
  memcpy(k_nk, m->spec_nk_prev, sizeof k_nk);
  m->in_cache_sync = true;
  run_write(m, OP_SET, (uint32_t)k, m->sx.p, m->sy.p, m->sv.p, m->so.p, s);
  m->in_cache_sync = false;
  m->spec_ready = k_ready; m->expect_bulk = k_bulk; m->long_probes = k_long; m->clustered = k_clu;
  clustered_sync(m, s);
  m->spec_nd_prev = k_nd; m->spec_nt_prev = k_nt; m->clustered_quiet = k_quiet; m->spec_gu_prev = k_gu;
  memcpy(m->spec_nk_prev, k_nk, sizeof k_nk);
  m->st.batches = batches;
  m->in_stride = keep;
  m->cache.flushes++;
  m->cache.flushed_cells += k;
}

}

#include "smx_file.inc"

namespace {
void flusher_main(smatrix_t* self, Matrix* m) {
  using clock = std::chrono::steady_clock;
  const auto period = std::chrono::milliseconds(m->flush_ms);
  std::unique_lock<std::mutex> l(m->fl_mu);
  auto next = clock::now() + period;
  while (!m->fl_stop) {
    m->fl_cv.wait_until(l, next, [&] { return m->fl_stop; });
    if (m->fl_stop) break;
    l.unlock();
    auto pause = period;
    if (m->dirty.load()) {
      const auto t0 = clock::now();
      bool more = false;
      {
        set_device(m);
        std::lock_guard<std::mutex> fg(m->file_mu);
        std::unique_lock<std::mutex> g(m->mu);
        if (m->dirty.exchange(false)) {
          cache_sync(m, false);
          more = file_flush(self, m, false, &g);
          m->file_bg_flushes_done.fetch_add(1);
          if (more) m->dirty = true;
        }
      }
      const auto took = std::chrono::duration_cast<std::chrono::milliseconds>(clock::now() - t0);
      pause = more ? std::chrono::milliseconds(1) : std::max(period, took * 10);
    }
    l.lock();
    next = clock::now() + pause;
  }
}
}

struct CopyPool {
  struct Slice { unsigned char* dst; const unsigned char* src; size_t len; std::atomic<uint32_t>* bad = nullptr; uint32_t want = 0; };
  std::vector<std::thread> th;
  std::mutex mu, run_mu;
  std::condition_variable cv, done_cv;
  std::vector<Slice> slices;
  size_t next = 0, left = 0;
  bool stop = false;
  void start(unsigned n) {
    for (unsigned t = 0; t < n; t++)
      th.emplace_back([this] {
        std::unique_lock<std::mutex> l(mu);
        for (;;) {
          cv.wait(l, [&] { return stop || next < slices.size(); });
          if (stop) return;
          const Slice sl = slices[next++];
          l.unlock();
          if (!sl.bad) memcpy(sl.dst, sl.src, sl.len);
          else if (!sl.bad->load(std::memory_order_relaxed)) {
            const uint32_t* p = reinterpret_cast<const uint32_t*>(sl.src);
            const size_t nw = sl.len / 4;
            uint32_t diff = 0;
            for (size_t i = 0; i < nw && !diff; i += 1024) {
              const size_t e = std::min(nw, i + 1024);
              for (size_t q = i; q < e; q++) diff |= p[q] ^ sl.want;
            }
            if (diff) sl.bad->store(1, std::memory_order_relaxed);
          }
          l.lock();
          if (--left == 0) done_cv.notify_all();
        }
      });
  }
  void add(std::vector<Slice>& v, void* dst, const void* src, size_t len) {
    for (size_t o = 0; o < len; o += (size_t)1 << 20) v.push_back({static_cast<unsigned char*>(dst) + o, static_cast<const unsigned char*>(src) + o, std::min<size_t>((size_t)1 << 20, len - o)});
  }
  void add_check(std::vector<Slice>& v, const void* src, size_t len, uint32_t want, std::atomic<uint32_t>* bad) {
    for (size_t o = 0; o < len; o += (size_t)1 << 20) v.push_back({nullptr, static_cast<const unsigned char*>(src) + o, std::min<size_t>((size_t)1 << 20, len - o), bad, want});
  }
  void run(std::vector<Slice>&& v) {
    if (v.empty()) return;
    std::lock_guard<std::mutex> one(run_mu);
    std::unique_lock<std::mutex> l(mu);
    slices = std::move(v); next = 0; left = slices.size();
    cv.notify_all();
    done_cv.wait(l, [&] { return left == 0; });
    slices.clear(); next = 0;
  }
  ~CopyPool() {
    { std::lock_guard<std::mutex> l(mu); stop = true; }
    cv.notify_all();
    for (auto& t : th) t.join();
  }
};

struct HostPipe {
  static constexpr int NB = 3;
  size_t chunk = 0;
  uint32_t* h_in[NB] = {nullptr, nullptr, nullptr};
  uint32_t* h_out[NB] = {nullptr, nullptr, nullptr};
  uint32_t* d_in[NB] = {nullptr, nullptr, nullptr};
  uint32_t* d_out[NB] = {nullptr, nullptr, nullptr};
  hipStream_t s_in = nullptr, s_out = nullptr;
  hipEvent_t ev_in[NB], ev_k[NB];
  CopyPool pool_in, pool_out;
  bool ok = true;
  HostPipe(size_t chunk_ops, unsigned t_in, unsigned t_out) : chunk(chunk_ops) {
    for (int b = 0; b < NB; b++) { ev_in[b] = nullptr; ev_k[b] = nullptr; }
    for (int b = 0; b < NB && ok; b++) {
      ok = ok && hipHostMalloc(reinterpret_cast<void**>(&h_in[b]), chunk * 12) == hipSuccess;
      ok = ok && hipHostMalloc(reinterpret_cast<void**>(&h_out[b]), chunk * 4) == hipSuccess;
      ok = ok && hipMalloc(reinterpret_cast<void**>(&d_in[b]), chunk * 12) == hipSuccess;
      ok = ok && hipMalloc(reinterpret_cast<void**>(&d_out[b]), chunk * 4) == hipSuccess;
      ok = ok && hipEventCreateWithFlags(&ev_in[b], hipEventDisableTiming) == hipSuccess;
      ok = ok && hipEventCreateWithFlags(&ev_k[b], hipEventDisableTiming) == hipSuccess;
    }
    ok = ok && hipStreamCreateWithFlags(&s_in, hipStreamNonBlocking) == hipSuccess;
    ok = ok && hipStreamCreateWithFlags(&s_out, hipStreamNonBlocking) == hipSuccess;
    if (!ok) { (void)hipGetLastError(); return; }
    pool_in.start(t_in);
    pool_out.start(t_out);
  }
  ~HostPipe() {
    for (int b = 0; b < NB; b++) {
      if (h_in[b]) (void)hipHostFree(h_in[b]);
      if (h_out[b]) (void)hipHostFree(h_out[b]);
      if (d_in[b]) (void)hipFree(d_in[b]);
      if (d_out[b]) (void)hipFree(d_out[b]);
      if (ev_in[b]) (void)hipEventDestroy(ev_in[b]);
      if (ev_k[b]) (void)hipEventDestroy(ev_k[b]);
    }
    if (s_in) (void)hipStreamDestroy(s_in);
    if (s_out) (void)hipStreamDestroy(s_out);
  }
};

size_t host_chunk_ops() {
  const char* a = getenv("SMATRIX_HOST_CHUNK_LG");
  const unsigned lg = a ? (unsigned)std::min(26ul, std::max(12ul, strtoul(a, nullptr, 10))) : 21u;
  return (size_t)1 << lg;
}

bool host_pipe_ready(Matrix* m) {
  if (m->host_pipe && static_cast<HostPipe*>(m->host_pipe)->chunk != host_chunk_ops()) {
    delete static_cast<HostPipe*>(m->host_pipe);
    m->host_pipe = nullptr;
  }
  if (!m->host_pipe) {
    const unsigned hw = std::max(2u, std::thread::hardware_concurrency());
    HostPipe* hp = new HostPipe(host_chunk_ops(), std::min(12u, hw / 2), std::min(8u, std::max(1u, hw / 4)));
    if (!hp->ok) { delete hp; return false; }
    m->host_pipe = hp;
  }
  return true;
}
template <typename F>
void host_pipeline(Matrix* m, size_t n, const uint32_t* const in[3], uint32_t* out, F compute) {
  HostPipe& hp = *static_cast<HostPipe*>(m->host_pipe);
  const size_t C = hp.chunk, nc = (n + C - 1) / C;
  const int dev = m->device;
  std::mutex mu;
  std::condition_variable cv;
  size_t fed = 0, computed = 0, drained = 0;
  double t_feed_copy = 0, t_feed_wait = 0, t_drain_copy = 0, t_drain_dma = 0, t_main_wait = 0, t_main_compute = 0;
  const double t_call = mono_s();
  std::thread feeder([&] {
    HIP_OK(hipSetDevice(dev));
    for (size_t k = 0; k < nc; k++) {
      const int b = (int)(k % HostPipe::NB);
      const size_t cnt = std::min(C, n - k * C);
      const double tf0 = mono_s();
      if (k >= (size_t)HostPipe::NB) {
        { std::unique_lock<std::mutex> l(mu); cv.wait(l, [&] { return computed >= k - HostPipe::NB + 1; }); }
        HIP_OK(hipEventSynchronize(hp.ev_k[b]));
      }
      const double tf1 = mono_s();
      std::atomic<uint32_t> v_differs{1};
      uint32_t v0 = 0;
      std::vector<CopyPool::Slice> v;
      for (int q = 0; q < 2; q++)
        if (in[q]) hp.pool_in.add(v, hp.h_in[b] + (size_t)q * C, in[q] + k * C, cnt * 4);
      if (in[2]) {
        const uint32_t* a = in[2] + k * C;
        v0 = a[0];
        if (a[cnt - 1] == v0 && a[cnt / 2] == v0 && a[cnt / 3] == v0) {
          v_differs.store(0);
          hp.pool_in.add_check(v, a, cnt * 4, v0, &v_differs);
        }
      }
      hp.pool_in.run(std::move(v));
      if (in[2] && v_differs.load()) {
        std::vector<CopyPool::Slice> v2;
        hp.pool_in.add(v2, hp.h_in[b] + 2 * C, in[2] + k * C, cnt * 4);
        hp.pool_in.run(std::move(v2));
      }
      t_feed_wait += tf1 - tf0; t_feed_copy += mono_s() - tf1;
      for (int q = 0; q < 2; q++)
        if (in[q]) HIP_OK(hipMemcpyAsync(hp.d_in[b] + (size_t)q * C, hp.h_in[b] + (size_t)q * C, cnt * 4, hipMemcpyHostToDevice, hp.s_in));
      if (in[2]) {
        if (v_differs.load()) HIP_OK(hipMemcpyAsync(hp.d_in[b] + 2 * C, hp.h_in[b] + 2 * C, cnt * 4, hipMemcpyHostToDevice, hp.s_in));
        else HIP_OK(hipMemsetD32Async(reinterpret_cast<hipDeviceptr_t>(hp.d_in[b] + 2 * C), (int)v0, cnt, hp.s_in));
      }
      HIP_OK(hipEventRecord(hp.ev_in[b], hp.s_in));
      { std::lock_guard<std::mutex> l(mu); fed = k + 1; }
      cv.notify_all();
    }
  });
  std::thread drain;
  if (out)
    drain = std::thread([&] {
      HIP_OK(hipSetDevice(dev));
      for (size_t k = 0; k < nc; k++) {
        const int b = (int)(k % HostPipe::NB);
        const size_t cnt = std::min(C, n - k * C);
        { std::unique_lock<std::mutex> l(mu); cv.wait(l, [&] { return computed >= k + 1; }); }
        const double td0 = mono_s();
        HIP_OK(hipStreamWaitEvent(hp.s_out, hp.ev_k[b], 0));
        HIP_OK(hipMemcpyAsync(hp.h_out[b], hp.d_out[b], cnt * 4, hipMemcpyDeviceToHost, hp.s_out));
        HIP_OK(hipStreamSynchronize(hp.s_out));
        const double td1 = mono_s();
        { std::lock_guard<std::mutex> l(mu); drained = k + 1; }
        cv.notify_all();
        std::vector<CopyPool::Slice> v;
        hp.pool_out.add(v, out + k * C, hp.h_out[b], cnt * 4);
        hp.pool_out.run(std::move(v));
        t_drain_dma += td1 - td0; t_drain_copy += mono_s() - td1;
      }
    });
  for (size_t k = 0; k < nc; k++) {
    const int b = (int)(k % HostPipe::NB);
    const size_t cnt = std::min(C, n - k * C);
    const double tm0 = mono_s();
    {
      std::unique_lock<std::mutex> l(mu);
      cv.wait(l, [&] { return fed >= k + 1 && (!out || k < (size_t)HostPipe::NB || drained >= k - HostPipe::NB + 1); });
    }
    const double tm1 = mono_s();
    HIP_OK(hipStreamWaitEvent(m->stream, hp.ev_in[b], 0));
    compute(cnt, hp.d_in[b], hp.d_in[b] + C, hp.d_in[b] + 2 * C, hp.d_out[b]);
    HIP_OK(hipEventRecord(hp.ev_k[b], m->stream));
    t_main_wait += tm1 - tm0; t_main_compute += mono_s() - tm1;
    { std::lock_guard<std::mutex> l(mu); computed = k + 1; }
    cv.notify_all();
  }
  feeder.join();
  if (drain.joinable()) drain.join();
  HIP_OK(hipStreamSynchronize(m->stream));
  if (m->trace_rounds)
    fprintf(stderr, "[smatrix] host pipeline: %zu ops in %zu chunks, %.2f ms | feeder: copies %.2f, waits %.2f | caller: waits %.2f, kernels %.2f | drain: device-to-host + waits %.2f, copies %.2f\n",
            n, nc, (mono_s() - t_call) * 1e3, t_feed_copy * 1e3, t_feed_wait * 1e3, t_main_wait * 1e3, t_main_compute * 1e3, t_drain_dma * 1e3, t_drain_copy * 1e3);
}

extern "C" {

int smatrix_flush(smatrix_t* self) {
  Matrix* m = M(self);
  if (m->fname.empty() || !self->fd) return 0;
  set_device(m);
  for (;;) {
    std::unique_lock<std::mutex> fg(m->file_mu);
    std::unique_lock<std::mutex> g(m->mu);
    if (!m->dirty.exchange(false)) break;
    cache_sync(m, false);
    if (!file_flush(self, m, false, &g)) break;
    m->dirty = true;
  }
  return 0;
}

int smatrix_compact(smatrix_t* self) {
  Matrix* m = M(self);
  const char* ex = getenv("SMATRIX_EXPERIMENTAL");
  if (!ex || *ex != '1') {
    fprintf(stderr, "libsmatrix: smatrix_compact is experimental; set SMATRIX_EXPERIMENTAL=1 to use it (nothing done)\n");
    return -1;
  }
  if (m->fname.empty() || !self->fd) return 0;
  set_device(m);
  std::lock_guard<std::mutex> fg(m->file_mu);
  std::lock_guard<std::mutex> g(m->mu);
  cache_sync(m, false);
  file_compact(self, m);
  return 0;
}

int smatrix_device_available(void) {
  int n = 0;
  if (hipGetDeviceCount(&n) != hipSuccess) { (void)hipGetLastError(); return 0; }
  return n > 0;
}

static const char* const KNOWN_SWITCHES[] = {
    "SMATRIX_BULK", "SMATRIX_BULK_MIN", "SMATRIX_BULK_PRESIZE_MIN", "SMATRIX_BULK_SHARE", "SMATRIX_CHUNK_POOL_GB", "SMATRIX_CLUSTERED", "SMATRIX_COLD_MIN",
    "SMATRIX_COLD_SHARE", "SMATRIX_COMPACT_AT_CLOSE", "SMATRIX_DEVICE", "SMATRIX_EXPERIMENTAL", "SMATRIX_FAR_JOIN", "SMATRIX_FAR_PLACE", "SMATRIX_FLUSH_EVERY",
    "SMATRIX_FLUSH_MS", "SMATRIX_FLUSH_SNAPSHOT_MB", "SMATRIX_FLUSH_SNAPSHOT_REFUSE", "SMATRIX_FSYNC", "SMATRIX_HINT_LG", "SMATRIX_HIP_LIB", "SMATRIX_HOST_CHUNK_LG",
    "SMATRIX_IO_THREADS", "SMATRIX_IO_WINDOW_MB", "SMATRIX_NO_VMM", "SMATRIX_PEND", "SMATRIX_RCCL_LIB", "SMATRIX_REST_LDS", "SMATRIX_REST_SLICE", "SMATRIX_SCALAR_CACHE",
    "SMATRIX_SCALAR_CACHE_CAP", "SMATRIX_SCRATCH_POOL", "SMATRIX_SET_LOCATE", "SMATRIX_SHARD_FORCE_RCCL", "SMATRIX_SHARD_PLACE", "SMATRIX_SHARD_SHM_MB",
    "SMATRIX_SHARD_TRANSPORT", "SMATRIX_SPEC", "SMATRIX_SPEC_TINY", "SMATRIX_TRACE_ROUNDS",
    "SMATRIX_SHARD_HOST_STAGED",
#ifdef SMX_MEASURE
    "SMATRIX_DBG_AFTER", "SMATRIX_REST_DBG", "SMATRIX_REST_DBG_FROM",
#endif
};
extern "C" char** environ;
static void warn_unknown_switches() {
  static std::once_flag once;
  std::call_once(once, [] {
    for (char** e = environ; e && *e; e++) {
      if (strncmp(*e, "SMATRIX_", 8) != 0) continue;
      const char* eq = strchr(*e, '=');
      const size_t len = eq ? (size_t)(eq - *e) : strlen(*e);
      bool known = false;
      for (const char* k : KNOWN_SWITCHES) known |= strlen(k) == len && strncmp(k, *e, len) == 0;
      if (!known) fprintf(stderr, "libsmatrix: the environment sets %.*s, which this library does not read (INTEGRATION.md lists its switches)\n", (int)len, *e);
    }
  });
}

smatrix_t* smatrix_open(const char* fname) {
  warn_unknown_switches();
  if (!smatrix_device_available()) {
    fprintf(stderr, "libsmatrix: no HIP device available (this build has no CPU fallback)\n");
    return nullptr;
  }
  smatrix_t* self = static_cast<smatrix_t*>(calloc(1, sizeof(smatrix_t)));
  if (!self) return nullptr;
  Matrix* m = new Matrix();
  self->impl = m;

  int dev = 0;
  const char* env = getenv("SMATRIX_DEVICE");
  if (env && *env) dev = atoi(env);
  else HIP_OK(hipGetDevice(&dev));
  m->device = dev;
  set_device(m);
  HIP_OK(hipStreamCreate(&m->stream));
  dev_malloc(&m->d_ctl, sizeof(Ctl));
  HIP_OK(hipHostMalloc(&m->h_ctl, sizeof(Ctl)));
  dev_malloc(&m->d_small, 64);
  HIP_OK(hipHostMalloc(&m->h_small, 64));
  HIP_OK(hipHostMalloc(&m->h_row, 32 + (size_t)SCALAR_ROW_PAIRS_ALLOC * 8));
  if (const char* a = getenv("SMATRIX_SET_LOCATE")) m->set_always_locate = *a == '1';
  if (const char* a = getenv("SMATRIX_BULK_PRESIZE_MIN")) m->fix_presize_min = (uint32_t)strtoul(a, nullptr, 10);
  if (const char* a = getenv("SMATRIX_FLUSH_SNAPSHOT_MB")) m->flush_snapshot = std::max<uint64_t>(1, strtoull(a, nullptr, 10)) << 20;
  if (const char* a = getenv("SMATRIX_SCALAR_CACHE")) m->cache.enabled = *a != '0';
  if (const char* a = getenv("SMATRIX_SCALAR_CACHE_CAP")) m->cache.shard_cap = std::max<size_t>(4, std::min<size_t>(strtoull(a, nullptr, 10), CellCache::SLOTS / 2));
  HIP_OK(hipEventCreate(&m->ev0));
  HIP_OK(hipEventCreate(&m->ev1));
  if (m->grow_fork) {
    HIP_OK(hipStreamCreateWithFlags(&m->helper, hipStreamNonBlocking));
    HIP_OK(hipEventCreateWithFlags(&m->ev_fork, hipEventDisableTiming));
    HIP_OK(hipEventCreateWithFlags(&m->ev_join, hipEventDisableTiming));
  }
  m->dir_size = 65536;
  dev_malloc(&m->d_dir, (size_t)m->dir_size * sizeof(DirSlot));
  zero_async(m->d_dir, (size_t)m->dir_size * sizeof(DirSlot), m->stream);
  m->arena.init(dev, 4u << 20, m->stream);
  m->map_old.need((size_t)1 << 20);
  m->map_new.need((size_t)1 << 21);
  for (uint32_t c = 0; c < N_CLASSES; c++) ensure_free_cap(m, c, c < 12 ? 1u << 18 : 1u << 12, m->stream);
  {
    if (hipMemPool_t pool = scratch_pool()) {
      void* warm = nullptr;
      if (hipMallocFromPoolAsync(&warm, 4096, pool, m->stream) == hipSuccess) (void)hipFreeAsync(warm, m->stream);
    }
    (void)hipGetLastError();
  }
  HIP_OK(hipStreamSynchronize(m->stream));
  ctl_push_persistent(m, m->stream);
  HIP_OK(hipFuncSetAttribute(reinterpret_cast<const void*>(&k_grow_lds<1024, GROW_LG2, false>),
                             hipFuncAttributeMaxDynamicSharedMemorySize, (int)grow_lds_bytes(GROW_LG2)));
  HIP_OK(hipFuncSetAttribute(reinterpret_cast<const void*>(&k_grow_lds<1024, GROW_LG2, true>),
                             hipFuncAttributeMaxDynamicSharedMemorySize, (int)grow_lds_bytes(GROW_LG2)));
  HIP_OK(hipFuncSetAttribute(reinterpret_cast<const void*>(&k_grow_rest_lds), hipFuncAttributeMaxDynamicSharedMemorySize, (int)rest_lds_bytes()));
  if (const char* a = getenv("SMATRIX_REST_LDS")) m->rest_lds = *a != '0';
  if (const char* a = getenv("SMATRIX_FAR_PLACE")) m->far_place = *a != '0';
  if (const char* a = getenv("SMATRIX_PEND")) m->pend_on = *a != '0';
  HIP_OK(hipFuncSetAttribute(reinterpret_cast<const void*>(&k_far_place<512, FAR_PLACE_SMALL_LG + 1, REST_LDS_MAX_LG>), hipFuncAttributeMaxDynamicSharedMemorySize,
                             (int)far_place_lds_bytes(REST_LDS_MAX_LG)));
  if (const char* a = getenv("SMATRIX_REST_SLICE")) m->rest_slice_cells = std::max<uint32_t>(64, (uint32_t)strtoul(a, nullptr, 10));
  if (const char* a = getenv("SMATRIX_FAR_JOIN")) m->far_join = *a != '0';
#ifdef SMX_MEASURE
  if (const char* a = getenv("SMATRIX_REST_DBG_FROM")) m->rest_dbg_from = strtoull(a, nullptr, 10);
  if (const char* a = getenv("SMATRIX_REST_DBG")) {
    m->rest_dbg_mode = (uint32_t)strtoul(a, nullptr, 10);
    dev_malloc(&m->rest_dbg, 1024);
    HIP_OK(hipMemset(m->rest_dbg, 0, 1024));
    HIP_OK(hipMemcpy(m->arena.base + offsetof(ArenaHead, dbg), &m->rest_dbg, 8, hipMemcpyHostToDevice));
  }
  if (const char* a = getenv("SMATRIX_DBG_AFTER")) m->dbg_after = strtoull(a, nullptr, 10);
#endif
  m->io_threads = std::min(16u, std::max(1u, std::thread::hardware_concurrency()));
  if (const char* a = getenv("SMATRIX_BULK")) m->bulk_enabled = *a != '0';
  if (const char* a = getenv("SMATRIX_SPEC")) m->spec_enabled = *a != '0';
  if (const char* a = getenv("SMATRIX_COLD_MIN")) m->cold_min = (uint32_t)strtoul(a, nullptr, 10);
  if (const char* a = getenv("SMATRIX_COLD_SHARE")) m->cold_share = std::max(1u, (uint32_t)strtoul(a, nullptr, 10));
  if (const char* a = getenv("SMATRIX_CLUSTERED")) { m->clustered = *a != '0'; m->clustered_forced = true; }
  if (const char* a = getenv("SMATRIX_HINT_LG")) m->hint_lg = std::min(28u, (uint32_t)strtoul(a, nullptr, 10));
  clustered_sync(m, m->stream);
  if (const char* a = getenv("SMATRIX_SPEC_TINY")) m->spec_tiny = *a == '1';
  if (const char* a = getenv("SMATRIX_BULK_MIN")) m->fix_min = (uint32_t)strtoul(a, nullptr, 10);
  if (const char* a = getenv("SMATRIX_BULK_SHARE")) m->fix_share = std::max(1u, (uint32_t)strtoul(a, nullptr, 10));
  if (const char* a = getenv("SMATRIX_FSYNC")) m->file_fsync = *a == '1';
  if (const char* a = getenv("SMATRIX_COMPACT_AT_CLOSE")) m->compact_at_close = *a == '1' && getenv("SMATRIX_EXPERIMENTAL") && *getenv("SMATRIX_EXPERIMENTAL") == '1';
  if (const char* a = getenv("SMATRIX_FLUSH_EVERY")) m->flush_every = strtoull(a, nullptr, 10);
  if (const char* a = getenv("SMATRIX_FLUSH_MS")) m->flush_ms = strtoull(a, nullptr, 10);
  if (const char* a = getenv("SMATRIX_IO_WINDOW_MB")) m->io_window = std::max<uint64_t>(1, strtoull(a, nullptr, 10)) << 20;
  if (const char* a = getenv("SMATRIX_IO_THREADS")) m->io_threads = std::max(1u, (unsigned)strtoul(a, nullptr, 10));
  if (const char* t = getenv("SMATRIX_TRACE_ROUNDS")) { m->trace_rounds = *t == '1' || *t == '2' || *t == '3'; m->trace_sync = *t == '2'; }
  m->profile = false;

  if (fname) {
    m->fname = fname;
    if (!file_open_or_create(self, m)) {
      smatrix_close(self);
      return nullptr;
    }
    if (m->clustered) { m->home_on = false; clustered_sync(m, m->stream); }
    if (m->flush_ms) m->flusher = std::thread(flusher_main, self, m);
  }
  refresh_public(self);
  return self;
}

void smatrix_close(smatrix_t* self) {
  if (!self) return;
  Matrix* m = M(self);
  if (m) {
    set_device(m);
    if (m->rest_dbg) {
      unsigned long long c[128];
      HIP_OK(hipMemcpy(c, m->rest_dbg, 1024, hipMemcpyDeviceToHost));
      fprintf(stderr, "[smatrix] far join, long probes of the wave-per-op pass: not in the table %llu, cell known %llu, absent at the scan %llu\n", c[16], c[17], c[18]);
      if (c[24]) fprintf(stderr, "[smatrix] wave-per-op pass with the join, cycles per op: directory + lane probe %.0f, join look-up %.0f, cooperative probes %.0f, apply / insert %.0f  (%llu ops)\n",
                         c[20] / (double)c[24], c[21] / (double)c[24], c[22] / (double)c[24], c[23] / (double)c[24], 64 * c[24]);
      if (c[28]) fprintf(stderr, "[smatrix] wave-per-op pass with the join: %llu trips of more than 10^5 cycles (%.0f on average, the longest %llu, longest cooperative probe %llu); by row size 2^(4k..): %llu %llu %llu %llu %llu %llu; finished %llu, deferred %llu\n",
                         c[28], c[30] / (double)c[28], c[29], c[31], c[32], c[33], c[34], c[35], c[36], c[37], c[38], c[39]);
      if (c[28]) fprintf(stderr, "[smatrix]   ... their cycles: directory + lane probe %.0f, join look-up %.0f, cooperative probes %.0f, apply / insert %.0f\n",
                                          c[40] / (double)c[28], c[41] / (double)c[28], c[42] / (double)c[28], c[43] / (double)c[28]);
      if (c[98] || c[113]) fprintf(stderr, "[smatrix] claimed inserts: %llu (placed %llu, none left %llu), ticks per insert: ticket %.0f (max %llu), claim %.0f (max %llu); words %.1f (max %llu), tries %.2f | above 10^5 ticks: %llu, ticket %.0f, claim %.0f, words %.1f, tries %.1f | no ticket: %llu, %.0f ticks (max %llu)\n",
              c[98], c[104], c[105], c[96] / (double)std::max(1ull, c[98]), c[99], c[97] / (double)std::max(1ull, c[98]), c[100], c[101] / (double)std::max(1ull, c[98]), c[103], c[102] / (double)std::max(1ull, c[98]),
              c[108], c[109] / (double)std::max(1ull, c[108]), c[110] / (double)std::max(1ull, c[108]), c[111] / (double)std::max(1ull, c[108]), c[112] / (double)std::max(1ull, c[108]),
              c[113], c[114] / (double)std::max(1ull, c[113]), c[115]);
      if (c[116]) fprintf(stderr, "[smatrix] retry's wave-per-op pass: %llu ops, %.0f ticks on average (max %llu); above 10^5 ticks: %llu (%.0f on average) by row size 2^(4k..): %llu %llu %llu %llu %llu %llu; deferred %llu\n",
                          c[116], c[117] / (double)c[116], c[118], c[119], c[120] / (double)std::max(1ull, c[119]), c[121], c[122], c[123], c[124], c[125], c[126], c[127]);
      fprintf(stderr, "[smatrix] k_grow_rest_lds: steps %llu rounds %llu | most steps of a wave %llu, most rounds %llu | trips %llu, most of a wave %llu | per round: losers %.2f blocked %.2f committed %.2f\n",
              c[0], c[1], c[3], c[6], c[4], c[5], c[8] / (double)std::max(1ull, c[1]), c[9] / (double)std::max(1ull, c[1]), c[10] / (double)std::max(1ull, c[1]));
      fprintf(stderr, "[smatrix] k_grow_rest_lds clock ticks, longest of all launches: row %llu = set-up %llu + waves %llu (placing %llu); a wave on average: %.0f (placing %.0f) over %llu waves\n",
              c[50], c[51], c[52], c[53], c[54] / (double)std::max(1ull, c[56]), c[55] / (double)std::max(1ull, c[56]), c[56]);
      fprintf(stderr, "[smatrix] k_grow_rest_lds phases, k ticks max / mean per wave: bitmap %llu / %.0f, cuts %llu / %.0f, cells in front %llu / %.0f, ranges %llu / %.0f, placing (wave) %llu / %.0f\n",
              c[59] >> 10, c[60] / 1024.0 / std::max(1ull, c[56]), c[61] >> 10, c[62] / 1024.0 / std::max(1ull, c[56]), c[57] >> 10, c[58] / 1024.0 / std::max(1ull, c[56]),
              c[63] >> 10, c[49] / 1024.0 / std::max(1ull, c[56]), c[52] >> 10, c[54] / 1024.0 / std::max(1ull, c[56]));
      for (int i = 0; i < 32; i++) if (c[64 + i]) fprintf(stderr, "[smatrix]   batch %%32 == %d: the row wave 0 of which ran longest: %llu k ticks, set-up %llu k, old table 2^%llu\n", i, c[64 + i] >> 40, (c[64 + i] >> 20) & 0xFFFFF, c[64 + i] & 0xFF);
      (void)hipFree(m->rest_dbg);
    }
    if (m->flusher.joinable()) {
      { std::lock_guard<std::mutex> l(m->fl_mu); m->fl_stop = true; }
      m->fl_cv.notify_all();
      m->flusher.join();
    }
    {
      std::lock_guard<std::mutex> fg(m->file_mu);
      std::lock_guard<std::mutex> g(m->mu);
      cache_sync(m, true);
      if (!m->fname.empty() && self->fd && m->compact_at_close) file_compact(self, m);
      else if (!m->fname.empty() && self->fd && m->dirty.exchange(false)) file_flush(self, m, false, nullptr);
      (void)hipStreamSynchronize(m->stream);
      PhaseClock clk(m->trace_rounds, "close");
      m->arena.destroy();
      clk.lap("arena unmapped");
      if (m->d_dir) (void)hipFree(m->d_dir);
      if (m->d_hints) (void)hipFree(m->d_hints);
      if (m->d_ctl) (void)hipFree(m->d_ctl);
      if (m->h_ctl) (void)hipHostFree(m->h_ctl);
      if (m->d_small) (void)hipFree(m->d_small);
      if (m->h_small) (void)hipHostFree(m->h_small);
      if (m->h_row) (void)hipHostFree(m->h_row);
      m->row_ret.release();
      export_release(m);
      recommend_release(m);
      merge_release(m);
      delete static_cast<HostPipe*>(m->host_pipe);
      m->far_tab.release(); m->far_unit_row.release(); m->far_zeros.release(); m->far_occ.release(); m->far_occ0.release(); m->far_clm.release(); m->far_rcnt.release(); m->far_bucket.release(); m->far_prows.release(); m->far_bloom.release(); m->far_unit_info.release(); m->big_list.release(); 
      m->pend_rec.release(); m->pend_keys.release(); m->task_of.release(); m->pend_ctl.release(); m->pend_hash.release();
      for (auto& d : m->defer) d.release();
      for (uint32_t c = 0; c < N_CLASSES; c++)
        if (m->fl.list[c]) (void)hipFree(m->fl.list[c]);
      m->cold_set.release(); m->cold_keys[0].release(); m->cold_keys[1].release(); m->cold_keys[2].release();
      m->cold_idx[0].release(); m->cold_idx[1].release(); m->cold_zero.release();
      m->fx_cnt.release(); m->fx_cur.release(); m->fx_pos.release(); m->fx_touched.release(); m->fx_where.release(); m->fx_grouped.release(); m->fx_rank.release(); m->fx_excl.release(); m->fx_tiles.release();
      graveyard().empty();
      m->tasks.release(); m->klist.release(); m->rebal.release(); m->map_old.release(); m->map_new.release(); m->disp_mask.release(); m->rest_tab.release(); m->cellp.release();
      m->sx.release(); m->sy.release(); m->sv.release(); m->so.release(); m->soff.release(); m->big.release(); m->seg.release(); m->ent_idx.release();
      get_timing_resolve(m, 0);
      for (hipEvent_t e : m->ev_free) (void)hipEventDestroy(e);
      if (m->ev0) (void)hipEventDestroy(m->ev0);
      if (m->ev1) (void)hipEventDestroy(m->ev1);
      if (m->ev_fork) (void)hipEventDestroy(m->ev_fork);
      if (m->ev_join) (void)hipEventDestroy(m->ev_join);
      if (m->helper) (void)hipStreamDestroy(m->helper);
      if (m->flush_stream) (void)hipStreamDestroy(m->flush_stream);
      if (m->stream) (void)hipStreamDestroy(m->stream);
      clk.lap("buffers freed");
    }
    if (self->fd) {
      PhaseClock clk(m->trace_rounds, "close");
      close(self->fd);
      clk.lap("close(fd)");
    }
    file_index_free(m);
    delete m;
  }
  free(self);
}

int smatrix_apply_batch_dev(smatrix_t* self, int op, size_t n, const uint32_t* d_x,
                            const uint32_t* d_y, const uint32_t* d_v, uint32_t* d_out,
                            void* hip_stream) {
  Matrix* m = M(self);
  set_device(m);
  CkptAfter ckpt(self);
  std::lock_guard<std::mutex> g(m->mu);
  cache_sync(m, op != OP_GET);
  hipStream_t s = static_cast<hipStream_t>(hip_stream);
  if (!d_out && n) { m->so.need(n); d_out = m->so.p; m->no_ret = true; }
  apply_dev_locked(self, op, n, d_x, d_y, d_v, d_out, s);
  m->no_ret = false;
  if (!hip_stream) HIP_OK(hipStreamSynchronize(s));
  return 0;
}

int smatrix_apply_packed_dev(smatrix_t* self, int op, size_t n, const uint32_t* d_records, uint32_t width,
                             uint32_t* d_out, void* hip_stream) {
  if (width != 2 && width != 3) return -1;
  if (op != OP_GET && width != 3) return -1;
  Matrix* m = M(self);
  set_device(m);
  CkptAfter ckpt(self);
  std::lock_guard<std::mutex> g(m->mu);
  cache_sync(m, op != OP_GET);
  hipStream_t s = static_cast<hipStream_t>(hip_stream);
  m->in_stride = width;
  if (!d_out && n) { m->so.need(n); d_out = m->so.p; m->no_ret = true; }
  apply_dev_locked(self, op, n, d_records, d_records + 1, d_records + 2, d_out, s);
  m->no_ret = false;
  m->in_stride = 1;
  if (!hip_stream) HIP_OK(hipStreamSynchronize(s));
  return 0;
}

int smatrix_apply_batch(smatrix_t* self, int op, size_t n, const uint32_t* x, const uint32_t* y,
                        const uint32_t* v, uint32_t* out) {
  if (n == 0) return 0;
  if (n >= (1ull << 32)) smx_die("batch too large (n must be < 2^32)");
  Matrix* m = M(self);
  set_device(m);
  CkptAfter ckpt(self);
  std::lock_guard<std::mutex> g(m->mu);
  cache_sync(m, op != OP_GET);
  hipStream_t s = m->stream;
  if (n >= 2 * host_chunk_ops() && (op == OP_GET || v) && host_pipe_ready(m)) {
    const uint32_t* in[3] = {x, y, op != OP_GET ? v : nullptr};
    m->no_ret = out == nullptr;
    const uint64_t batches0 = m->st.batches;
    host_pipeline(m, n, in, out, [&](size_t cnt, uint32_t* dx, uint32_t* dy, uint32_t* dv, uint32_t* dout) {
      apply_dev_locked(self, op, cnt, dx, dy, dv, dout, s);
    });
    m->no_ret = false;
    if (op != OP_GET) {
      m->st.batches = batches0 + 1;
      m->ckpt_due = m->flush_every && self->fd && m->st.batches % m->flush_every == 0;
    }
    return 0;
  }
  m->sx.need(n); m->sy.need(n); m->so.need(n);
  HIP_OK(hipMemcpyAsync(m->sx.p, x, n * 4, hipMemcpyHostToDevice, s));
  HIP_OK(hipMemcpyAsync(m->sy.p, y, n * 4, hipMemcpyHostToDevice, s));
  if (op != OP_GET) {
    m->sv.need(n);
    HIP_OK(hipMemcpyAsync(m->sv.p, v, n * 4, hipMemcpyHostToDevice, s));
  }
  m->no_ret = out == nullptr;
  apply_dev_locked(self, op, n, m->sx.p, m->sy.p, m->sv.p, m->so.p, s);
  m->no_ret = false;
  if (out) HIP_OK(hipMemcpyAsync(out, m->so.p, n * 4, hipMemcpyDeviceToHost, s));
  HIP_OK(hipStreamSynchronize(s));
  return 0;
}

int smatrix_get_batch(smatrix_t* self, size_t n, const uint32_t* x, const uint32_t* y, uint32_t* out) {
  return smatrix_apply_batch(self, OP_GET, n, x, y, nullptr, out);
}
int smatrix_set_batch(smatrix_t* self, size_t n, const uint32_t* x, const uint32_t* y,
                      const uint32_t* v, uint32_t* out) {
  return smatrix_apply_batch(self, OP_SET, n, x, y, v, out);
}
int smatrix_incr_batch(smatrix_t* self, size_t n, const uint32_t* x, const uint32_t* y,
                       const uint32_t* v, uint32_t* out) {
  return smatrix_apply_batch(self, OP_INCR, n, x, y, v, out);
}
int smatrix_decr_batch(smatrix_t* self, size_t n, const uint32_t* x, const uint32_t* y,
                       const uint32_t* v, uint32_t* out) {
  return smatrix_apply_batch(self, OP_DECR, n, x, y, v, out);
}

int smatrix_rowlen_batch_dev(smatrix_t* self, size_t n, const uint32_t* d_x, uint32_t* d_out,
                             void* hip_stream) {
  if (n == 0) return 0;
  Matrix* m = M(self);
  set_device(m);
  std::lock_guard<std::mutex> g(m->mu);
  hipStream_t s = static_cast<hipStream_t>(hip_stream);
  hipLaunchKernelGGL(k_rowlen, dim3(blocks_for(n)), dim3(256), 0, s, m->d_dir, m->dir_size - 1,
                     m->arena.base, (uint32_t)n, d_x, d_out);
  HIP_OK(hipGetLastError());
  if (!hip_stream) HIP_OK(hipStreamSynchronize(s));
  return 0;
}

int smatrix_rowlen_batch(smatrix_t* self, size_t n, const uint32_t* x, uint32_t* out) {
  if (n == 0) return 0;
  Matrix* m = M(self);
  set_device(m);
  std::lock_guard<std::mutex> g(m->mu);
  hipStream_t s = m->stream;
  if (n >= 2 * host_chunk_ops() && host_pipe_ready(m)) {
    const uint32_t* in[3] = {x, nullptr, nullptr};
    host_pipeline(m, n, in, out, [&](size_t cnt, uint32_t* dx, uint32_t*, uint32_t*, uint32_t* dout) {
      hipLaunchKernelGGL(k_rowlen, dim3(blocks_for(cnt)), dim3(256), 0, s, m->d_dir, m->dir_size - 1, m->arena.base, (uint32_t)cnt, dx, dout);
      HIP_OK(hipGetLastError());
    });
    return 0;
  }
  m->sx.need(n); m->so.need(n);
  HIP_OK(hipMemcpyAsync(m->sx.p, x, n * 4, hipMemcpyHostToDevice, s));
  hipLaunchKernelGGL(k_rowlen, dim3(blocks_for(n)), dim3(256), 0, s, m->d_dir, m->dir_size - 1,
                     m->arena.base, (uint32_t)n, m->sx.p, m->so.p);
  HIP_OK(hipGetLastError());
  HIP_OK(hipMemcpyAsync(out, m->so.p, n * 4, hipMemcpyDeviceToHost, s));
  HIP_OK(hipStreamSynchronize(s));
  return 0;
}

namespace {
void launch_getrow_big(Matrix* m, hipStream_t s, uint32_t n, uint32_t grid, const uint32_t* x, const uint64_t* off,
                       uint64_t* ret, uint32_t* counts, const uint32_t* big) {
  const uint32_t budget = (uint32_t)std::min<uint64_t>(m->arena.mapped / 8 / GETROW_SEG + 2, 1u << 24);
  const size_t segs = (size_t)n + budget;
  m->seg.need((size_t)n + 1 + segs);
  uint32_t* seg_start = m->seg.p;
  uint32_t* seg_cnt = m->seg.p + n + 1;
  hipLaunchKernelGGL(k_getrow_plan, dim3(1), dim3(1024), 0, s, m->d_dir, m->dir_size - 1, x, big, seg_start, budget);
// ... 591 lines not shown
```

Before: 19840 Mops/s.

## Chain a second speculative grow-and-retry round without host sync

Extends the speculative write chain so that, when the previous batch needed exactly three plain rounds, a second growth pass and retry are enqueued behind the first, sized from the last batch's second-round counts. This removes one host round-trip (readback plus relaunch) per write batch in steady state. It also lets bulk-expected batches chain when bulk mode is disabled. The cost is a larger up-front arena and task reservation and extra state to track. If the estimates are too small, it falls back to the normal rounds.

Result: no change. 19830 Mops/s (-0.1%).

```diff
diff --git a/include/smatrix_batch.h b/include/smatrix_batch.h
--- a/include/smatrix_batch.h
+++ b/include/smatrix_batch.h
@@ -114,6 +114,7 @@
   uint64_t kernel_ops[4];
   double   write_call_ms, write_wait_ms, write_alloc_ms;
   double   last_write_call_ms, last_write_wait_ms, last_write_alloc_ms;
+  uint64_t spec_chains2;
 } smatrix_stats_t;
 
 void smatrix_stats(smatrix_t* self, smatrix_stats_t* out);
diff --git a/libsmatrix_amd/_lib.py b/libsmatrix_amd/_lib.py
--- a/libsmatrix_amd/_lib.py
+++ b/libsmatrix_amd/_lib.py
@@ -16,7 +16,8 @@
         "scalar_cache_flushed_cells", "bulk_rounds", "bulk_ops", "file_flushes", "file_rows_written", "file_leaked_bytes",
         "file_compactions", "spec_chains", "spec_refused", "file_bg_flushes", "cold_starts", "cold_keys", "clustered_mode", "set_located_by_fold", "flush_snapshots_refused")] + [
         ("kernel_ms", C.c_double * 4), ("kernel_launches", C.c_uint64 * 4), ("kernel_ops", C.c_uint64 * 4)] + [
-        (n, C.c_double) for n in ("write_call_ms", "write_wait_ms", "write_alloc_ms", "last_write_call_ms", "last_write_wait_ms", "last_write_alloc_ms")]
+        (n, C.c_double) for n in ("write_call_ms", "write_wait_ms", "write_alloc_ms", "last_write_call_ms", "last_write_wait_ms", "last_write_alloc_ms")] + [
+        ("spec_chains2", C.c_uint64)]
 
 
 class Handle(C.Structure):
diff --git a/libsmatrix_amd/csrc/kernels/growth.hpp b/libsmatrix_amd/csrc/kernels/growth.hpp
--- a/libsmatrix_amd/csrc/kernels/growth.hpp
+++ b/libsmatrix_amd/csrc/kernels/growth.hpp
@@ -1231,6 +1231,24 @@
   ctl->arena_oom = keep_oom;
 }
 
+__global__ void k_round_advance2(Ctl* ctl, const uint32_t* rebal, DirSlot* dir, uint8_t* arena) {
+  rebal_body(VGrid{0, 1}, ctl, rebal, dir, arena);
+  __syncthreads();
+  if (threadIdx.x != 0 || blockIdx.x != 0) return;
+  ctl->n_prev = ctl->n_defer;
+  ctl->spec_nd1 = ctl->n_defer;
+  ctl->spec_nt1 = ctl->n_tasks;
+  ctl->spec_gu1 = ctl->grow_units;
+  ctl->spec_nrebal1 = ctl->n_rebal;
+  for (int k = 0; k < 4; k++) ctl->spec_nkind1[k] = ctl->n_kind[k];
+  const uint32_t keep_long = ctl->n_long, keep_oom = ctl->arena_oom, keep_long_ops = ctl->n_long_ops;
+  uint64_t* z = reinterpret_cast<uint64_t*>(ctl);
+  for (uint32_t i = 0; i < CTL_ROUND_BYTES / 8; i++) z[i] = 0;
+  ctl->n_long = keep_long;
+  ctl->n_long_ops = keep_long_ops;
+  ctl->arena_oom = keep_oom;
+}
+
 __global__ __launch_bounds__(256) void k_dir_rehash(const DirSlot* old, uint32_t old_size,
                                                     DirSlot* dir, uint32_t dmask) {
   uint32_t p = blockIdx.x * blockDim.x + threadIdx.x;
diff --git a/libsmatrix_amd/csrc/kernels/layout.hpp b/libsmatrix_amd/csrc/kernels/layout.hpp
--- a/libsmatrix_amd/csrc/kernels/layout.hpp
+++ b/libsmatrix_amd/csrc/kernels/layout.hpp
@@ -79,6 +79,11 @@
   uint32_t spec_nkind0[4];
   uint32_t n_big, n_units;
   uint32_t far_nd, pad_far;
+  uint32_t spec_nd1;
+  uint32_t spec_nt1;
+  uint64_t spec_gu1;
+  uint32_t spec_nrebal1, spec_pad1;
+  uint32_t spec_nkind1[4];
 };
 constexpr size_t CTL_ROUND_BYTES = 64;
 static_assert(offsetof(Ctl, dir_used) == CTL_ROUND_BYTES, "the per-round part of Ctl is what ctl_reset_round zeroes");
diff --git a/libsmatrix_amd/csrc/smx_runtime.hip b/libsmatrix_amd/csrc/smx_runtime.hip
--- a/libsmatrix_amd/csrc/smx_runtime.hip
+++ b/libsmatrix_amd/csrc/smx_runtime.hip
@@ -545,6 +545,7 @@
   static constexpr bool grow_fork = true;
   hipStream_t helper = nullptr;
   hipEvent_t ev_fork = nullptr, ev_join = nullptr;
+  hipEvent_t ev_fork2 = nullptr, ev_join2 = nullptr;
 
   std::string fname;
   std::atomic<bool> dirty{false};
@@ -582,6 +583,10 @@
   uint32_t last_nd0 = 1;
   uint32_t spec_nd_prev = 0, spec_nt_prev = 0, spec_nk_prev[4] = {0, 0, 0, 0};
   uint64_t spec_gu_prev = 0;
+  bool spec2_enabled = true;
+  bool spec2_ready = false;
+  uint32_t spec2_nd_prev = 0, spec2_nt_prev = 0, spec2_nk_prev[4] = {0, 0, 0, 0};
+  uint64_t spec2_gu_prev = 0;
   bool long_probes = false;
   bool clustered = false, clustered_forced = false;
   uint32_t clustered_quiet = 0;
@@ -961,7 +966,7 @@
   return e;
 }
 
-void grow_rows(Matrix* m, hipStream_t s, uint32_t nt, uint64_t gu, const uint32_t* nk, bool spec, bool pend_prep) {
+void grow_rows_reserve(Matrix* m, hipStream_t s, uint64_t nt, uint64_t gu, bool pend_prep) {
   ensure_arena_free(m, gu, s);
   m->map_new.need((size_t)nt + gu / 4 + 1);
   m->map_old.need((size_t)nt + gu / 8 + 1);
@@ -969,17 +974,25 @@
     m->disp_mask.need(m->map_old.cap);
     m->rest_tab.need(2 + 2 * ((size_t)m->map_old.cap * 64 / m->rest_slice_cells + m->tasks.cap + 1));
   }
+  for (uint32_t c = 0; c < N_CLASSES; c++) ensure_free_cap(m, c, nt, s);
+  if (pend_prep && m->clustered && m->home_on) {
+    m->pend_keys.need(std::min<uint64_t>(8ull * nt + 4ull * gu + 1024, 0x7FFFFFFFull));
+    m->task_of.need(m->dir_size);
+    uint32_t pend_hash_lg = 16;
+    while (pend_hash_lg < 24 && (1ull << pend_hash_lg) < 2ull * m->pend_est) pend_hash_lg++;
+    m->pend_hash.need((size_t)1 << pend_hash_lg);
+  }
+}
+
+void grow_rows(Matrix* m, hipStream_t s, uint32_t nt, uint64_t gu, const uint32_t* nk, bool spec, bool pend_prep, int half = 0) {
+  grow_rows_reserve(m, s, nt, gu, pend_prep);
   uint64_t cap_units = m->arena.mapped / UNIT_BYTES;
   if (spec && m->spec_tiny) cap_units = std::min<uint64_t>(cap_units, m->arena_next + gu);
-  for (uint32_t c = 0; c < N_CLASSES; c++) ensure_free_cap(m, c, nt, s);
   const bool pend = pend_prep && m->clustered && m->home_on;
   uint32_t pend_hash_lg = 16;
-  if (pend) {
-    m->pend_keys.need(std::min<uint64_t>(8ull * nt + 4ull * gu + 1024, 0x7FFFFFFFull));
-    m->task_of.need(m->dir_size);
+  if (pend)
     while (pend_hash_lg < 24 && (1ull << pend_hash_lg) < 2ull * m->pend_est) pend_hash_lg++;
-    m->pend_hash.need((size_t)1 << pend_hash_lg);
-  }
+  hipEvent_t ev_fork = half ? m->ev_fork2 : m->ev_fork, ev_join = half ? m->ev_join2 : m->ev_join;
   hipLaunchKernelGGL(k_grow_plan, dim3(std::min<uint32_t>(blocks_for(nt), 1024)), dim3(256), 0, s,
                      m->d_ctl, m->tasks.p, cap_units, m->fl, spec ? nt : 0xFFFFFFFFu,
                      spec ? (uint32_t)std::min<uint64_t>(m->map_old.cap, m->map_new.cap / 2) : 0xFFFFFFFFu,
@@ -994,7 +1007,7 @@
   const uint32_t* pend_keys = pend ? m->pend_keys.p : nullptr;
   const uint32_t n_chunked = nk[GROW_CHUNKED];
   const bool fork = m->grow_fork && n_chunked && (nk[0] || nk[1] || nk[2]);
-  if (fork) HIP_OK(hipEventRecord(m->ev_fork, s));
+  if (fork) HIP_OK(hipEventRecord(ev_fork, s));
   auto lds_kinds = [&](auto pend_c) {
     constexpr bool P = decltype(pend_c)::value;
     if (nk[0])
@@ -1012,7 +1025,7 @@
   const uint64_t oc_bound = (uint64_t)n_chunked + gu / 8, nc_bound = (uint64_t)n_chunked + gu / 4;
   hipStream_t sc = s;
   if (fork) {
-    HIP_OK(hipStreamWaitEvent(m->helper, m->ev_fork, 0));
+    HIP_OK(hipStreamWaitEvent(m->helper, ev_fork, 0));
     sc = m->helper;
   }
   if (n_chunked) {
@@ -1046,8 +1059,8 @@
   }
   DBG_STEP(m, s, "chunked passes");
   if (fork) {
-    HIP_OK(hipEventRecord(m->ev_join, sc));
-    HIP_OK(hipStreamWaitEvent(s, m->ev_join, 0));
+    HIP_OK(hipEventRecord(ev_join, sc));
+    HIP_OK(hipStreamWaitEvent(s, ev_join, 0));
   }
   hipLaunchKernelGGL(k_grow_commit, dim3(std::min<uint32_t>(blocks_for(nt), 1024)), dim3(256), 0, s,
                      m->d_ctl, m->tasks.p, m->d_dir, m->arena.base, m->fl, m->big_list_valid ? m->big_list.p : nullptr, BIG_LIST_CAP);
@@ -1357,8 +1370,10 @@
   uint32_t rounds_this_batch = 0;
   bool cold_tried = false;
   bool structure_stable = false;
-  bool chain = m->spec_enabled && m->spec_ready && !m->expect_bulk && n >= m->agg_min && m->dbg_after == 0 &&
+  bool chain = m->spec_enabled && m->spec_ready && !(m->expect_bulk && m->bulk_enabled) && n >= m->agg_min && m->dbg_after == 0 &&
                (m->last_nd0 != 0 || m->spec_tiny);
+  const bool chain2 = chain && m->spec2_enabled && m->spec2_ready;
+  bool plain_rounds = true;
   for (uint32_t round = 0;; round++) {
     if (stalled > 8) smx_die("write batch did not converge (corrupt row table?)");
     const uint32_t dir_limit = m->dir_size / 2;
@@ -1370,13 +1385,16 @@
     if (round >= 1 && idx && !cold_tried && m->cold_min && cur_n >= m->cold_min && (uint64_t)cur_n * m->cold_share >= n &&
         op != OP_GET) {
       cold_tried = true;
-      if (insert_pending_keys(m, idx, cur_n, x, y, s)) rounds_this_batch += 4;
+      if (insert_pending_keys(m, idx, cur_n, x, y, s)) { rounds_this_batch += 4; plain_rounds = false; }
     }
     uint32_t* dl = m->defer[round & 1].p;
     const bool chained = chain && round == 0;
     const uint32_t est_nt = m->spec_tiny ? 5u : (uint32_t)std::min<uint64_t>(std::max<uint64_t>(2ull * m->spec_nt_prev, 1u << 16), std::min<uint64_t>(cur_n, m->dir_size));
     const uint64_t est_gu = m->spec_tiny ? 24u : std::max<uint64_t>(2 * m->spec_gu_prev, 1ull << 20);
-    ensure_arena_free(m, std::min<uint64_t>(cur_n, room) + (chained ? est_gu : 0), s);
+    const bool chained2 = chained && chain2;
+    const uint32_t est_nt2 = m->spec_tiny ? 5u : (uint32_t)std::min<uint64_t>(std::max<uint64_t>(2ull * m->spec2_nt_prev, 1u << 16), std::min<uint64_t>(cur_n, m->dir_size));
+    const uint64_t est_gu2 = m->spec_tiny ? 24u : std::max<uint64_t>(2 * m->spec2_gu_prev, 1ull << 20);
+    ensure_arena_free(m, std::min<uint64_t>(cur_n, room) + (chained ? est_gu : 0) + (chained2 ? est_gu2 : 0), s);
     ctl_reset_round(m, s);
     const bool all_new = round == 0 && !chained && m->dir_used == 0 && m->bulk_enabled && m->expect_bulk && n >= m->fix_min &&
                          n >= m->agg_min && m->dbg_after == 0 && (op == OP_INCR || op == OP_DECR);
@@ -1428,6 +1446,7 @@
         cur_n = nd2;
         round++;
         rounds_this_batch += 2;
+        plain_rounds = false;
         continue;
       }
     }
@@ -1485,40 +1504,56 @@
       const uint32_t est_nk[4] = {std::max<uint32_t>(2 * m->spec_nk_prev[0], 4096), std::max<uint32_t>(2 * m->spec_nk_prev[1], 1024),
                                   std::max<uint32_t>(2 * m->spec_nk_prev[2], 256), std::max<uint32_t>(2 * m->spec_nk_prev[3], 64)};
       const uint64_t host_next = m->arena_next;
+      if (chained2) grow_rows_reserve(m, s, (uint64_t)est_nt + est_nt2, est_gu + est_gu2, prep_pend);
       grow_rows(m, s, est_nt, est_gu, est_nk, true, prep_pend);
       m->arena_next = host_next;
       hipLaunchKernelGGL(k_round_advance, dim3(1), dim3(64), 0, s, m->d_ctl, m->rebal.p, m->d_dir, m->arena.base);
+      const auto launch_retry = [&](uint32_t* in, uint32_t* other, uint32_t est_nd) -> uint32_t* {
+        const dim3 rgrid(std::min<uint32_t>(blocks_for(est_nd), 16384));
+        if (m->clustered && est_nd <= m->wpo_max && m->retry_split && m->d_hints) {
+          const dim3 wgrid(std::min<uint32_t>(blocks_for((uint64_t)est_nd * (64 / SMX_WPO_OPS)), 65536));
+          switch (op) {
+            case OP_SET:  hipLaunchKernelGGL((k_apply_short<OP_SET>), rgrid, dim3(256), 0, s, m->d_ctl, m->d_dir, m->dir_size - 1, m->arena.base, 0xFFFFFFFFu, in, x, y, v, out, other, m->in_stride); break;
+            case OP_INCR: hipLaunchKernelGGL((k_apply_short<OP_INCR>), rgrid, dim3(256), 0, s, m->d_ctl, m->d_dir, m->dir_size - 1, m->arena.base, 0xFFFFFFFFu, in, x, y, v, out, other, m->in_stride); break;
+            default:      hipLaunchKernelGGL((k_apply_short<OP_DECR>), rgrid, dim3(256), 0, s, m->d_ctl, m->d_dir, m->dir_size - 1, m->arena.base, 0xFFFFFFFFu, in, x, y, v, out, other, m->in_stride); break;
+          }
+          hipLaunchKernelGGL(k_list_advance, dim3(1), dim3(64), 0, s, m->d_ctl);
+          switch (op) {
+            case OP_SET:  hipLaunchKernelGGL((k_apply_wpo<OP_SET>), wgrid, dim3(256), 0, s, m->d_ctl, m->d_dir, m->dir_size - 1, m->arena.base, 0xFFFFFFFFu, other, x, y, v, out, in, m->in_stride); break;
+            case OP_INCR: hipLaunchKernelGGL((k_apply_wpo<OP_INCR>), wgrid, dim3(256), 0, s, m->d_ctl, m->d_dir, m->dir_size - 1, m->arena.base, 0xFFFFFFFFu, other, x, y, v, out, in, m->in_stride); break;
+            default:      hipLaunchKernelGGL((k_apply_wpo<OP_DECR>), wgrid, dim3(256), 0, s, m->d_ctl, m->d_dir, m->dir_size - 1, m->arena.base, 0xFFFFFFFFu, other, x, y, v, out, in, m->in_stride); break;
+          }
+          retry_halves = true;
+          return in;
+        }
+        if (m->clustered && est_nd <= m->wpo_max) {
+          const dim3 wgrid(std::min<uint32_t>(blocks_for((uint64_t)est_nd * 64), 65536));
+          switch (op) {
+            case OP_SET:  hipLaunchKernelGGL((k_apply_wpo<OP_SET>), wgrid, dim3(256), 0, s, m->d_ctl, m->d_dir, m->dir_size - 1, m->arena.base, 0xFFFFFFFFu, in, x, y, v, out, other, m->in_stride); break;
+            case OP_INCR: hipLaunchKernelGGL((k_apply_wpo<OP_INCR>), wgrid, dim3(256), 0, s, m->d_ctl, m->d_dir, m->dir_size - 1, m->arena.base, 0xFFFFFFFFu, in, x, y, v, out, other, m->in_stride); break;
+            default:      hipLaunchKernelGGL((k_apply_wpo<OP_DECR>), wgrid, dim3(256), 0, s, m->d_ctl, m->d_dir, m->dir_size - 1, m->arena.base, 0xFFFFFFFFu, in, x, y, v, out, other, m->in_stride); break;
+          }
+          return other;
+        }
+        switch (op) {
+          case OP_SET:  hipLaunchKernelGGL((k_apply<OP_SET>), rgrid, dim3(256), 0, s, m->d_ctl, m->d_dir, m->dir_size - 1, m->arena.base, 0xFFFFFFFFu, in, x, y, v, out, other, m->in_stride); break;
+          case OP_INCR: hipLaunchKernelGGL((k_apply<OP_INCR>), rgrid, dim3(256), 0, s, m->d_ctl, m->d_dir, m->dir_size - 1, m->arena.base, 0xFFFFFFFFu, in, x, y, v, out, other, m->in_stride); break;
+          default:      hipLaunchKernelGGL((k_apply<OP_DECR>), rgrid, dim3(256), 0, s, m->d_ctl, m->d_dir, m->dir_size - 1, m->arena.base, 0xFFFFFFFFu, in, x, y, v, out, other, m->in_stride); break;
+        }
+        return other;
+      };
       const uint32_t est_nd = (uint32_t)std::min<uint64_t>(std::max<uint64_t>(2ull * m->spec_nd_prev, 1u << 16), cur_n);
-      uint32_t* dl1 = pre_pass ? m->defer[0].p : m->defer[1].p;
-      const dim3 rgrid(std::min<uint32_t>(blocks_for(est_nd), 16384));
-      if (m->clustered && est_nd <= m->wpo_max && m->retry_split && m->d_hints) {
-        uint32_t* dl0 = dl;
-        const dim3 wgrid(std::min<uint32_t>(blocks_for((uint64_t)est_nd * (64 / SMX_WPO_OPS)), 65536));
-        switch (op) {
-          case OP_SET:  hipLaunchKernelGGL((k_apply_short<OP_SET>), rgrid, dim3(256), 0, s, m->d_ctl, m->d_dir, m->dir_size - 1, m->arena.base, 0xFFFFFFFFu, dl, x, y, v, out, dl1, m->in_stride); break;
-          case OP_INCR: hipLaunchKernelGGL((k_apply_short<OP_INCR>), rgrid, dim3(256), 0, s, m->d_ctl, m->d_dir, m->dir_size - 1, m->arena.base, 0xFFFFFFFFu, dl, x, y, v, out, dl1, m->in_stride); break;
-          default:      hipLaunchKernelGGL((k_apply_short<OP_DECR>), rgrid, dim3(256), 0, s, m->d_ctl, m->d_dir, m->dir_size - 1, m->arena.base, 0xFFFFFFFFu, dl, x, y, v, out, dl1, m->in_stride); break;
-        }
-        hipLaunchKernelGGL(k_list_advance, dim3(1), dim3(64), 0, s, m->d_ctl);
-        switch (op) {
-          case OP_SET:  hipLaunchKernelGGL((k_apply_wpo<OP_SET>), wgrid, dim3(256), 0, s, m->d_ctl, m->d_dir, m->dir_size - 1, m->arena.base, 0xFFFFFFFFu, dl1, x, y, v, out, dl0, m->in_stride); break;
-          case OP_INCR: hipLaunchKernelGGL((k_apply_wpo<OP_INCR>), wgrid, dim3(256), 0, s, m->d_ctl, m->d_dir, m->dir_size - 1, m->arena.base, 0xFFFFFFFFu, dl1, x, y, v, out, dl0, m->in_stride); break;
-          default:      hipLaunchKernelGGL((k_apply_wpo<OP_DECR>), wgrid, dim3(256), 0, s, m->d_ctl, m->d_dir, m->dir_size - 1, m->arena.base, 0xFFFFFFFFu, dl1, x, y, v, out, dl0, m->in_stride); break;
-        }
-        dl1 = dl0;
-        retry_halves = true;
-      } else if (m->clustered && est_nd <= m->wpo_max) {
-        const dim3 wgrid(std::min<uint32_t>(blocks_for((uint64_t)est_nd * 64), 65536));
-        switch (op) {
-          case OP_SET:  hipLaunchKernelGGL((k_apply_wpo<OP_SET>), wgrid, dim3(256), 0, s, m->d_ctl, m->d_dir, m->dir_size - 1, m->arena.base, 0xFFFFFFFFu, dl, x, y, v, out, dl1, m->in_stride); break;
-          case OP_INCR: hipLaunchKernelGGL((k_apply_wpo<OP_INCR>), wgrid, dim3(256), 0, s, m->d_ctl, m->d_dir, m->dir_size - 1, m->arena.base, 0xFFFFFFFFu, dl, x, y, v, out, dl1, m->in_stride); break;
-          default:      hipLaunchKernelGGL((k_apply_wpo<OP_DECR>), wgrid, dim3(256), 0, s, m->d_ctl, m->d_dir, m->dir_size - 1, m->arena.base, 0xFFFFFFFFu, dl, x, y, v, out, dl1, m->in_stride); break;
-        }
-      } else
-      switch (op) {
-        case OP_SET:  hipLaunchKernelGGL((k_apply<OP_SET>), rgrid, dim3(256), 0, s, m->d_ctl, m->d_dir, m->dir_size - 1, m->arena.base, 0xFFFFFFFFu, dl, x, y, v, out, dl1, m->in_stride); break;
-        case OP_INCR: hipLaunchKernelGGL((k_apply<OP_INCR>), rgrid, dim3(256), 0, s, m->d_ctl, m->d_dir, m->dir_size - 1, m->arena.base, 0xFFFFFFFFu, dl, x, y, v, out, dl1, m->in_stride); break;
-        default:      hipLaunchKernelGGL((k_apply<OP_DECR>), rgrid, dim3(256), 0, s, m->d_ctl, m->d_dir, m->dir_size - 1, m->arena.base, 0xFFFFFFFFu, dl, x, y, v, out, dl1, m->in_stride); break;
+      uint32_t* dl1 = launch_retry(dl, pre_pass ? m->defer[0].p : m->defer[1].p, est_nd);
+      if (chained2) {
+        launch_prep(dl1);
+        HIP_OK(hipGetLastError());
+        const uint32_t est_nk2[4] = {std::max<uint32_t>(2 * m->spec2_nk_prev[0], 4096), std::max<uint32_t>(2 * m->spec2_nk_prev[1], 1024),
+                                     std::max<uint32_t>(2 * m->spec2_nk_prev[2], 256), std::max<uint32_t>(2 * m->spec2_nk_prev[3], 64)};
+        grow_rows(m, s, est_nt2, est_gu2, est_nk2, true, prep_pend, 1);
+        m->arena_next = host_next;
+        hipLaunchKernelGGL(k_round_advance2, dim3(1), dim3(64), 0, s, m->d_ctl, m->rebal.p, m->d_dir, m->arena.base);
+        const uint32_t est_nd2 = (uint32_t)std::min<uint64_t>(std::max<uint64_t>(2ull * m->spec2_nd_prev, 1u << 16), cur_n);
+        dl1 = launch_retry(dl1, dl1 == m->defer[0].p ? m->defer[1].p : m->defer[0].p, est_nd2);
       }
       launch_prep(dl1);
       HIP_OK(hipGetLastError());
@@ -1544,6 +1579,16 @@
         m->spec_nd_prev = nd_chain0; m->spec_nt_prev = c.spec_nt0; m->spec_gu_prev = c.spec_gu0;
         for (int k = 0; k < 4; k++) m->spec_nk_prev[k] = c.spec_nkind0[k];
       }
+      if (chained2 && nd_chain0 && c.spec_nd1) {
+        m->st.rounds++;
+        rounds_this_batch++;
+        m->st.deferred_ops += c.spec_nd1;
+        m->st.rows_grown += c.spec_nt1;
+        m->st.rows_rebalanced += c.spec_nrebal1;
+        m->spec2_nd_prev = c.spec_nd1; m->spec2_nt_prev = c.spec_nt1; m->spec2_gu_prev = c.spec_gu1;
+        for (int k = 0; k < 4; k++) m->spec2_nk_prev[k] = c.spec_nkind1[k];
+        if (c.n_defer == 0) m->st.spec_chains2++;
+      }
       if (c.spec_failed) {
         m->st.spec_refused++;
         const uint32_t zero = 0;
@@ -1561,12 +1606,17 @@
         fprintf(stderr, "[smatrix] batch %llu chain: ops=%u (the pass in front of prep took %u) deferred=%u grow=%u (%llu units) rebal=%u refused=%u | after the retry: deferred=%u grow=%u rows=%u | long probes %u%s\n",
                 (unsigned long long)m->st.batches, cur_n, far_joined ? c.far_nd : 0u, nd_chain0, c.spec_nt0, (unsigned long long)c.spec_gu0, c.spec_nrebal0,
                 c.spec_failed, c.n_defer, c.n_tasks, c.dir_used, c.n_long_ops, m->clustered ? " (clustered)" : "");
+      if (m->trace_rounds && chained2)
+        fprintf(stderr, "[smatrix]   long chain: the first retry left deferred=%u grow=%u (%llu units) rebal=%u -- second growth round and retry enqueued behind it\n",
+                c.spec_nd1, c.spec_nt1, (unsigned long long)c.spec_gu1, c.spec_nrebal1);
       if (!m->clustered_forced && m->clustered) {
         m->clustered_quiet = (uint64_t)c.n_long_ops * (m->d_hints ? 4096 : 256) < n ? m->clustered_quiet + 1 : 0;
         if (m->clustered_quiet >= 8) { m->clustered = false; clustered_sync(m, s); }
       }
       if (nd_chain0 == 0) { structure_stable = true; break; }
-      cur_n = nd_chain0;
+      cur_n = chained2 && c.spec_nd1 ? c.spec_nd1 : nd_chain0;
+      if (chained2) round = dl == m->defer[0].p ? 2 : 1;
+      else
       round = (pre_pass ? 2 : 1) + (retry_halves ? 1 : 0);
     } else if (pre_pass) {
       if (far_joined) { m->far_rows_seen = m->h_ctl->n_big; m->far_units_seen = m->h_ctl->n_units; m->far_nd_seen = m->h_ctl->far_nd; }
@@ -1588,6 +1638,10 @@
       t_prev = now;
     }
     if (m->h_ctl->arena_oom) smx_die("internal: arena reservation too small");
+    if (!chained2 && rounds_this_batch == 2) {
+      m->spec2_nd_prev = m->h_ctl->n_defer; m->spec2_nt_prev = m->h_ctl->n_tasks; m->spec2_gu_prev = m->h_ctl->grow_units;
+      for (int k = 0; k < 4; k++) m->spec2_nk_prev[k] = m->h_ctl->n_kind[k];
+    }
     const uint32_t nd = m->h_ctl->n_defer;
     if (round == 0) m->expect_bulk = (uint64_t)nd * 8 >= n;
     if (round == 0 && !chained && !m->in_cache_sync) m->last_nd0 = nd;
@@ -1623,6 +1677,7 @@
     if (pre_pass && !chained) round++;
   }
   m->spec_ready = rounds_this_batch <= 4;
+  m->spec2_ready = plain_rounds && rounds_this_batch == 3;
   for (void* q : m->put_aside) (void)dev_free(q);
   m->put_aside.clear();
   if (m->spec_ready || !cold_tried) {
@@ -1748,6 +1803,11 @@
   const uint64_t k_gu = m->spec_gu_prev;
   uint32_t k_nk[4];
   memcpy(k_nk, m->spec_nk_prev, sizeof k_nk);
+  const bool k_ready2 = m->spec2_ready;
+  const uint32_t k_nd2 = m->spec2_nd_prev, k_nt2 = m->spec2_nt_prev;
+  const uint64_t k_gu2 = m->spec2_gu_prev;
+  uint32_t k_nk2[4];
+  memcpy(k_nk2, m->spec2_nk_prev, sizeof k_nk2);
   m->in_cache_sync = true;
   run_write(m, OP_SET, (uint32_t)k, m->sx.p, m->sy.p, m->sv.p, m->so.p, s);
   m->in_cache_sync = false;
@@ -1755,6 +1815,8 @@
   clustered_sync(m, s);
   m->spec_nd_prev = k_nd; m->spec_nt_prev = k_nt; m->clustered_quiet = k_quiet; m->spec_gu_prev = k_gu;
   memcpy(m->spec_nk_prev, k_nk, sizeof k_nk);
+  m->spec2_ready = k_ready2; m->spec2_nd_prev = k_nd2; m->spec2_nt_prev = k_nt2; m->spec2_gu_prev = k_gu2;
+  memcpy(m->spec2_nk_prev, k_nk2, sizeof k_nk2);
   m->st.batches = batches;
   m->in_stride = keep;
   m->cache.flushes++;
@@ -2056,7 +2118,7 @@
     "SMATRIX_FLUSH_MS", "SMATRIX_FLUSH_SNAPSHOT_MB", "SMATRIX_FLUSH_SNAPSHOT_REFUSE", "SMATRIX_FSYNC", "SMATRIX_HINT_LG", "SMATRIX_HIP_LIB", "SMATRIX_HOST_CHUNK_LG",
     "SMATRIX_IO_THREADS", "SMATRIX_IO_WINDOW_MB", "SMATRIX_NO_VMM", "SMATRIX_PEND", "SMATRIX_RCCL_LIB", "SMATRIX_REST_LDS", "SMATRIX_REST_SLICE", "SMATRIX_SCALAR_CACHE",
     "SMATRIX_SCALAR_CACHE_CAP", "SMATRIX_SCRATCH_POOL", "SMATRIX_SET_LOCATE", "SMATRIX_SHARD_FORCE_RCCL", "SMATRIX_SHARD_PLACE", "SMATRIX_SHARD_SHM_MB",
-    "SMATRIX_SHARD_TRANSPORT", "SMATRIX_SPEC", "SMATRIX_SPEC_TINY", "SMATRIX_TRACE_ROUNDS",
+    "SMATRIX_SHARD_TRANSPORT", "SMATRIX_SPEC", "SMATRIX_SPEC2", "SMATRIX_SPEC_TINY", "SMATRIX_TRACE_ROUNDS",
     "SMATRIX_SHARD_HOST_STAGED",
 #ifdef SMX_MEASURE
     "SMATRIX_DBG_AFTER", "SMATRIX_REST_DBG", "SMATRIX_REST_DBG_FROM",
@@ -2111,6 +2173,8 @@
     HIP_OK(hipStreamCreateWithFlags(&m->helper, hipStreamNonBlocking));
     HIP_OK(hipEventCreateWithFlags(&m->ev_fork, hipEventDisableTiming));
     HIP_OK(hipEventCreateWithFlags(&m->ev_join, hipEventDisableTiming));
+    HIP_OK(hipEventCreateWithFlags(&m->ev_fork2, hipEventDisableTiming));
+    HIP_OK(hipEventCreateWithFlags(&m->ev_join2, hipEventDisableTiming));
   }
   m->dir_size = 65536;
   dev_malloc(&m->d_dir, (size_t)m->dir_size * sizeof(DirSlot));
@@ -2153,6 +2217,7 @@
   m->io_threads = std::min(16u, std::max(1u, std::thread::hardware_concurrency()));
   if (const char* a = getenv("SMATRIX_BULK")) m->bulk_enabled = *a != '0';
   if (const char* a = getenv("SMATRIX_SPEC")) m->spec_enabled = *a != '0';
+  if (const char* a = getenv("SMATRIX_SPEC2")) m->spec2_enabled = *a != '0';
   if (const char* a = getenv("SMATRIX_COLD_MIN")) m->cold_min = (uint32_t)strtoul(a, nullptr, 10);
   if (const char* a = getenv("SMATRIX_COLD_SHARE")) m->cold_share = std::max(1u, (uint32_t)strtoul(a, nullptr, 10));
   if (const char* a = getenv("SMATRIX_CLUSTERED")) { m->clustered = *a != '0'; m->clustered_forced = true; }
@@ -2258,6 +2323,8 @@
       if (m->ev1) (void)hipEventDestroy(m->ev1);
       if (m->ev_fork) (void)hipEventDestroy(m->ev_fork);
       if (m->ev_join) (void)hipEventDestroy(m->ev_join);
+      if (m->ev_fork2) (void)hipEventDestroy(m->ev_fork2);
+      if (m->ev_join2) (void)hipEventDestroy(m->ev_join2);
       if (m->helper) (void)hipStreamDestroy(m->helper);
       if (m->flush_stream) (void)hipStreamDestroy(m->flush_stream);
       if (m->stream) (void)hipStreamDestroy(m->stream);
```
